# MingruiYuan/SpoofSV

Measured on AMD Instinct MI355X. Metric: mel-frames/sec (Text2Mel+SSRN train), higher is better.
Workload: dtype f32 (conv GEMMs: fp32 operands scaled by a power of two and split into fp16 hi+lo = 22 significand bits, three exact fp16 MFMAs per product, fp32 accumulate: ~2^-22 per product, gradients within 3e-6 of float64 = the exact-fp32 path's level); 1 GPU; train_text2mel + train_ssrn (train/ordinary.py step: fwd, l1+bin-div+guided-att losses, bwd, Adam), batch 32 utterances/GPU, N=186, T=325, 80 mel -> 513x1300 linear, hidden 256, random-init; global_batch=32, parallelism=dp1, launch=hipGraph replay, ddp=none

## Files before the change

include/ssv_hip.h:

```cpp
#ifndef SSV_HIP_H
#define SSV_HIP_H
#include <stddef.h>
#include <stdint.h>
#ifdef __cplusplus
extern "C" {
#endif

typedef void* ssv_stream_t;

int ssv_version(void);
const char* ssv_arch(void);
const char* ssv_last_error(void);
int ssv_set_precision(int mode);
int ssv_get_precision(void);
int ssv_amax_rows(int L);
int ssv_absmax(const float* x, long x_bs, int B, long n, float* amax, int namax, ssv_stream_t stream);
int ssv_shift_right_amax(const float* x, long x_bs, float* y, int B, int C, int T, float* amax, int namax, ssv_stream_t stream);
int ssv_deinterleave2_amax(const float* x, long x_bs, float* out, int B, long n, float* amax, int namax, ssv_stream_t stream);
int ssv_deinterleave2_rows_amax(const float* x, long x_bs, float* out, int B, int rows, int L, float* amax, int namax, ssv_stream_t stream);

size_t ssv_conv1d_fwd_workspace(int Cin, int Cout, int k);
int ssv_conv1d_fwd(const float* x, long x_bs, const float* x_amax, int x_namax, const float* w, const void* w_packed, const float* bias,
                   const float* bias_b, float* y, long y_bs, float* y_colstats,
                   int B, int Cin, int Cout, int L, int k, int dilation, int causal,
                   void* ws, size_t ws_bytes, ssv_stream_t stream);
size_t ssv_conv1d_bwd_data_workspace(int Cin, int Cout, int k);
int ssv_conv1d_bwd_data(const float* dy, long dy_bs, const float* dy_amax, int dy_namax, const float* w, const void* w_packed,
                        const float* dx_add, float* dx, long dx_bs,
                        int B, int Cin, int Cout, int L, int k, int dilation, int causal,
                        void* ws, size_t ws_bytes, ssv_stream_t stream);
size_t ssv_conv1d_bwd_weight_workspace(int B, int Cin, int Cout, int L, int k);
int ssv_conv1d_bwd_weight(const float* dy, long dy_bs, const float* dy_amax, int dy_namax, const float* x, long x_bs, const float* x_amax, int x_namax,
                          float* dw, int B, int Cin, int Cout, int L, int k, int dilation, int causal,
                          void* ws, size_t ws_bytes, ssv_stream_t stream);
int ssv_rowsum(const float* x, long x_bs, float* out, int B, int C, int L, ssv_stream_t stream);
int ssv_bias_grad(const float* x, long x_bs, float* out, int B, int C, int L, ssv_stream_t stream);
int ssv_sum_slabs(const float* slabs, float* out, long n, int Z, long stride, ssv_stream_t stream);
int ssv_copy_rows(const float* src, long src_bs, float* dst, long dst_bs, int B, long n, ssv_stream_t stream);

size_t ssv_channel_ln_act_fwd_workspace(int B, int C, int L);
int ssv_channel_ln_act_fwd(const float* x, long x_bs, const float* gamma, const float* beta,
                           float* y, long y_bs, float* y_amax, float* stats, int B, int C, int L, int act,
                           void* ws, size_t ws_bytes, ssv_stream_t stream);
size_t ssv_pointwise_conv_ln_act_fwd_workspace(int Cin, int Cout);
int ssv_pointwise_conv_ln_act_fwd(const float* x, long x_bs, const float* x_amax, int x_namax, const float* w, const void* w_packed, const float* bias,
                                  const float* s, const float* gamma, const float* beta, float* pre, float* stats, float* y, long y_bs, float* y_amax,
                                  int B, int Cin, int Cout, int L, int act, void* ws, size_t ws_bytes, ssv_stream_t stream);
size_t ssv_channel_ln_act_bwd_workspace(int B, int C, int L);
int ssv_channel_ln_act_bwd(const float* dy, long dy_bs, const float* x, long x_bs, const float* stats,
                           const float* gamma, const float* beta, float* dx, long dx_bs, float* pgrads,
                           int B, int C, int L, int act, void* ws, size_t ws_bytes, ssv_stream_t stream);

size_t ssv_pointwise_conv_ln_act_bwd_workspace(int B, int Cin, int Cout, int L);
int ssv_pointwise_conv_ln_act_bwd(const float* dy, long dy_bs, const float* x, long x_bs, const float* x_amax, int x_namax,
                                  const float* w, const void* w_packed,
                                  const float* gamma, const float* beta, const float* pre, const float* stats,
                                  float* dx, long dx_bs, float* dw, float* pgrads, float* ds,
                                  int B, int Cin, int Cout, int L, int act, void* ws, size_t ws_bytes, ssv_stream_t stream);

typedef struct {
  const float* dy; const float* x; float* dw; const float* part; float* pgrads;
  int shift[3]; int pad_;
  const float* dy_amax; const float* x_amax;
  int dy_namax, x_namax;
} ssv_wgrad_job;
int ssv_conv_shifts(int k, int dilation, int causal, int* shift3);
int ssv_conv1d_bwd_weight_multi_ok(int B, int Cin, int Cout, int L, int k);
int ssv_conv1d_bwd_weight_multi_splits(int njobs, int B, int Cin, int Cout, int L, int k);
size_t ssv_conv1d_bwd_weight_multi_workspace(int njobs, int B, int Cin, int Cout, int L, int k);
int ssv_conv1d_bwd_weight_multi(const ssv_wgrad_job* jobs_dev, int njobs, long dy_bs, long x_bs, int B, int Cin, int Cout, int L, int k, int max_shift,
                                int n2, int nblk, void* ws, size_t ws_bytes, ssv_stream_t stream);
int ssv_ln_partial_rows(int B, int L);
int ssv_ln_bwd_partial_rows(int gate, int B, int C, int L, int with_amax);
size_t ssv_highway_conv1d_bwd_data_workspace(int B, int C, int L, int k);
int ssv_highway_conv1d_bwd_data(const float* dy, long dy_bs, const float* x, long x_bs, const float* w, const void* w_packed,
                                const float* g1, const float* b1, const float* g2, const float* b2, const float* h, const float* stats,
                                float* dx, long dx_bs, float* dh, float* dh_amax, float* part, int B, int C, int L, int k, int dilation, int causal,
                                void* ws, size_t ws_bytes, ssv_stream_t stream);
size_t ssv_pointwise_conv_ln_act_bwd_data_workspace(int B, int Cin, int Cout, int L);
int ssv_pointwise_conv_ln_act_bwd_data(const float* dy, long dy_bs, const float* w, const void* w_packed, const float* gamma, const float* beta,
                                       const float* pre, const float* stats, float* dx, long dx_bs, float* ds, float* dpre, float* dpre_amax,
                                       float* part, int B, int Cin, int Cout, int L, int act, void* ws, size_t ws_bytes, ssv_stream_t stream);

size_t ssv_highway_conv1d_fwd_workspace(int B, int C, int L, int k);
int ssv_highway_conv1d_fwd(const float* x, long x_bs, const float* x_amax, int x_namax, const float* w, const void* w_packed, const float* bias,
                           const float* g1, const float* b1, const float* g2, const float* b2,
                           float* h, float* stats, float* y, long y_bs, float* y_amax,
                           int B, int C, int L, int k, int dilation, int causal,
                           void* ws, size_t ws_bytes, ssv_stream_t stream);
size_t ssv_highway_conv1d_bwd_workspace(int B, int C, int L, int k);
int ssv_highway_conv1d_bwd(const float* dy, long dy_bs, const float* x, long x_bs, const float* x_amax, int x_namax, const float* w, const void* w_packed,
                           const float* g1, const float* b1, const float* g2, const float* b2,
                           const float* h, const float* stats, float* dx, long dx_bs, float* dw, float* pgrads,
                           int B, int C, int L, int k, int dilation, int causal,
                           void* ws, size_t ws_bytes, ssv_stream_t stream);

size_t ssv_highway_gate_bwd_workspace(int B, int C, int L);
int ssv_highway_gate_bwd(const float* dy, long dy_bs, const float* x, long x_bs,
                         const float* g1, const float* b1, const float* g2, const float* b2,
                         const float* h, const float* stats, float* dh, float* dxres, long dx_bs, float* pgrads,
                         int B, int C, int L, void* ws, size_t ws_bytes, ssv_stream_t stream);

int ssv_text_embed_fwd(const int64_t* ids, const float* w, const float* bias, float* y,
                       int B, int N, int E, int vocab, ssv_stream_t stream);
int ssv_text_embed_bwd(const int64_t* ids, const float* dy, float* dw, float* dbias,
                       int B, int N, int E, int vocab, ssv_stream_t stream);

int ssv_attention_train_fwd(const float* k, const float* v, long kv_bs, const float* q, long q_bs,
                            float* a, float* r, long r_bs, int B, int d, int N, int T, ssv_stream_t stream);
int ssv_attention_train_fwd_rq(const float* k, const float* v, long kv_bs, const float* q, long q_bs, float* a, float* rq, long rq_bs,
                               int B, int d, int N, int T, ssv_stream_t stream);
size_t ssv_attention_train_bwd_workspace(int B, int d, int N, int T);
int ssv_attention_train_bwd(const float* dr, long dr_bs, const float* da_ext, const float* dq_add, long dq_add_bs,
                            const float* k, const float* v, long kv_bs, const float* q, long q_bs, const float* a,
                            float* dk, float* dv, long dkv_bs, float* dq, long dq_bs,
                            int B, int d, int N, int T, void* ws, size_t ws_bytes, ssv_stream_t stream);

int ssv_attention_step(const float* k, long kv_bs, const float* q_last, long q_bs, long q_cs,
                       const int64_t* pma_in, float* a, int a_T, int col, const int* col_dev, int64_t* pma_out,
                       int B, int d, int N, ssv_stream_t stream);
int ssv_synth_advance(const float* y, float* mel_in, int* col_dev, int B, int F, int T, ssv_stream_t stream);
int ssv_attention_apply(const float* v, long kv_bs, const float* a, int a_T, float* r, long r_bs,
                        int B, int d, int N, int T, ssv_stream_t stream);

size_t ssv_deconv1d_k2s2_fwd_workspace(int Cin, int Cout);
int ssv_deconv1d_k2s2_fwd(const float* x, long x_bs, const float* x_amax, int x_namax, const float* w, const void* w_packed, const float* bias,
                          float* y, long y_bs, float* y_amax, int y_namax, int B, int Cin, int Cout, int L, void* ws, size_t ws_bytes, ssv_stream_t stream);
size_t ssv_deconv1d_k2s2_bwd_workspace(int B, int Cin, int Cout);
int ssv_deconv1d_k2s2_bwd(const float* dy, long dy_bs, const float* dy_amax, int dy_namax, const float* x, long x_bs, const float* w,
                          float* dx, long dx_bs, float* dw, float* dbias,
                          int B, int Cin, int Cout, int L, void* ws, size_t ws_bytes, ssv_stream_t stream);

size_t ssv_spec_losses_workspace(long n);
int ssv_spec_losses_fwd(const float* y, const float* gt, long n, float* out, void* ws, size_t ws_bytes, ssv_stream_t stream);
int ssv_spec_losses_bwd(const float* y, const float* gt, long n, const float* gscale, float* dy, ssv_stream_t stream);
int ssv_spec_losses_fwd_bwd(const float* y, const float* gt, long n, const float* gscale, float* out, float* dy, void* ws, size_t ws_bytes,
                            ssv_stream_t stream);
size_t ssv_guided_att_loss_workspace(int B, int N, int T);
int ssv_guided_att_loss_fwd(const float* a, const float* gaw, int gaw_T, float* out, int B, int N, int T,
                            void* ws, size_t ws_bytes, ssv_stream_t stream);
int ssv_guided_att_loss_bwd(const float* gaw, int gaw_T, const float* gscale, float* da, int B, int N, int T,
                            ssv_stream_t stream);

int ssv_mask_cols(float* x, long x_bs, int B, int C, int L, const int* live, int mult, ssv_stream_t stream);
int ssv_attention_train_fwd_rq_len(const float* k, const float* v, long kv_bs, const float* q, long q_bs, float* a, float* rq, long rq_bs,
                                   int B, int d, int N, int T, const int* live, ssv_stream_t stream);
int ssv_spec_losses_len(const float* y, const float* gt, int B, int C, int L, const int* live, int mult, const float* gscale,
                        float* out, float* dy, void* ws, size_t ws_bytes, ssv_stream_t stream);
int ssv_guided_att_loss_fwd_len(const float* a, const float* gaw, int gaw_T, float* out, int B, int N, int T, const int* live,
                                void* ws, size_t ws_bytes, ssv_stream_t stream);
int ssv_guided_att_loss_bwd_len(const float* gaw, int gaw_T, const float* gscale, float* da, int B, int N, int T, const int* live,
                                ssv_stream_t stream);

typedef struct { const float* w; void* planes; int M, K, Kpad, KT; long sm, sk; int first_block, pad_; float* inv_out; } ssv_pack_job;
size_t ssv_conv_pack_bytes(int Cout, int Cin, int k);
int ssv_conv_pack_plan(int n, const float* const* w, void* const* planes, const int* Cout, const int* Cin, const int* k,
                       ssv_pack_job* jobs_host);
size_t ssv_conv_pack_multi_workspace(int njobs);
int ssv_conv_pack_multi(const ssv_pack_job* jobs_dev, int njobs, int nblocks, void* ws, size_t ws_bytes, ssv_stream_t stream);

typedef struct { float* p; const float* g; float* m; float* v; long n; } ssv_adam_chunk;
int ssv_adam_multi(const ssv_adam_chunk* chunks, int nchunks, float lr, float beta1, float beta2, float eps,
                   int step, int* step_dev, ssv_stream_t stream);

size_t ssv_lstm_fwd_workspace(int Bn, int T, int F, int H, int layers);
int ssv_lstm_fwd(const float* x, const float* const* w_ih, const float* const* w_hh,
                 const float* const* b_ih, const float* const* b_hh, float* h_last,
                 int Bn, int T, int F, int H, int layers, void* ws, size_t ws_bytes, ssv_stream_t stream);
int ssv_lstm_fwd_cached(const float* x, const float* const* w_ih, const float* const* w_hh,
                        const float* const* b_ih, const float* const* b_hh, float* h_last,
                        int Bn, int T, int F, int H, int layers, void* ws, size_t ws_bytes, int weights_packed, ssv_stream_t stream);
size_t ssv_proj_l2norm_fwd_workspace(int Bn, int P);
int ssv_proj_l2norm_fwd(const float* h, const float* w, const float* bias, float* e, float* norms, int Bn, int H, int P,
                        void* ws, size_t ws_bytes, ssv_stream_t stream);
size_t ssv_proj_l2norm_bwd_workspace(int Bn, int P);
int ssv_proj_l2norm_bwd(const float* de, const float* e, const float* norms, const float* h, const float* w,
                        float* dh, float* dw, float* dbias, int Bn, int H, int P, void* ws, size_t ws_bytes, ssv_stream_t stream);
size_t ssv_lstm_saved_bytes(int Bn, int T, int F, int H, int layers);
size_t ssv_lstm_train_fwd_workspace(int Bn, int T, int F, int H, int layers);
int ssv_lstm_train_fwd(const float* x, const float* const* w_ih, const float* const* w_hh,
                       const float* const* b_ih, const float* const* b_hh, float* h_last, void* saved,
                       int Bn, int T, int F, int H, int layers, void* ws, size_t ws_bytes, ssv_stream_t stream);
size_t ssv_lstm_bwd_workspace(int Bn, int T, int F, int H, int layers);
int ssv_lstm_bwd(const float* dh_last, const void* saved, const float* const* w_ih, const float* const* w_hh,
                 float* const* dw_ih, float* const* dw_hh, float* const* db_ih, float* const* db_hh,
                 int Bn, int T, int F, int H, int layers, void* ws, size_t ws_bytes, ssv_stream_t stream);
size_t ssv_ge2e_loss_fwd_workspace(int N, int M, int D);
int ssv_ge2e_loss_fwd(const float* emb, const float* w, const float* b, float* loss, float* per,
                      int N, int M, int D, void* ws, size_t ws_bytes, ssv_stream_t stream);

size_t ssv_ge2e_loss_bwd_workspace(int N, int M, int D);
int ssv_ge2e_loss_bwd(const float* emb, const float* w, const float* b, const float* dloss, float* demb, float* dw, float* db,
                      int N, int M, int D, void* ws, size_t ws_bytes, ssv_stream_t stream);

int ssv_tisv_batch_gather(const float* corpus, long U_total, const int* rows, float* out, int Bn, int nmels, int frames, ssv_stream_t stream);
#define SSV_CLIP_SGD_MAX_GROUPS 8
typedef struct { float* p; const float* g; long n; int group; int pad_; } ssv_clip_sgd_chunk;
long ssv_clip_sgd_workspace(int nchunks);
int ssv_clip_sgd_multi(const ssv_clip_sgd_chunk* chunks, int nchunks, const float* max_norm, int ngroups, float lr, float* norms,
                       const float* loss, float* loss_hist, int hist_len, int* step_dev, void* ws, size_t ws_bytes, ssv_stream_t stream);

int ssv_sv_trial_scores(const float* enr, const float* ver, float* sim, float* cent, int N, int E, int V, int ver_stride, int D, ssv_stream_t stream);
int ssv_sv_eer_sweep(const float* sim, int N, int V, const float* thr, int nthr, int head, int tail, double den, double pos, double hden,
                     double hpos, int* counts, double* hist, int hist_len, int* step_dev, ssv_stream_t stream);
int ssv_sv_accept_rate(const float* sim_stack, int nmat, int N, int V, int tail, float thres, float* rates, ssv_stream_t stream);
int ssv_sv_score_curve(const float* sim_stack, int nmat, int N, int V, int head, int tail, const float* thr, int nthr, int* counts, ssv_stream_t stream);
int ssv_score_list_curve_f32(const float* scores, const unsigned char* cls, long n, int nclass, const float* thr, int nthr, int* counts, ssv_stream_t stream);
int ssv_score_list_curve_f64(const double* scores, const unsigned char* cls, long n, int nclass, const double* thr, int nthr, int* counts, ssv_stream_t stream);
int ssv_sv_curve_tile(void);

long ssv_ivec_features_workspace(long G, int Cc, int delta_order);
int ssv_ivec_features(const float* mel, const long* utt_off, const float* dct, float* out, long G, int M, int U, int Cc, int delta_window,
                      int delta_order, int cmn_window, void* ws, size_t ws_bytes, ssv_stream_t stream);
int ssv_gmm_frame_tile(int D, int C);
int ssv_gmm_diag_gselect(const float* X, const float* A, const float* B, const float* g, int* idx, float* post, float* loglik, long F, int D, int C,
                         int nsel, float min_post, ssv_stream_t stream);
int ssv_gmm_diag_stats(const float* X, const int* idx, const float* post, const long* seg_off, const long* seg_off_host, float* slab, long F, int D,
                       int C, int nsel, int S, int order, ssv_stream_t stream);
int ssv_gmm_stats_reduce(const float* slab, double* out, int S, long n, ssv_stream_t stream);
int ssv_gmm_diag_update(const double* stats, double* w, double* mu, double* var, float* A, float* B, float* g, int C, int D, double var_floor,
                        double min_count, double min_weight, ssv_stream_t stream);
int ssv_gmm_diag_planes(const double* w, const double* mu, const double* var, float* A, float* B, float* g, int C, int D, ssv_stream_t stream);

int ssv_gl_project(const float* mag, const float* reb, const float* tprev, float alpha, float* proj,
                   int B, int F, int T, ssv_stream_t stream);
int ssv_complex_abs(const float* spec, float* mag, int B, int F, int T, ssv_stream_t stream);
int ssv_ola_frames(const float* fr, const float* inv_env, float* out, int B, int N, int T, int hop, ssv_stream_t stream);
int ssv_ola_signal(const float* fr, const float* inv_env, float* y, int B, int N, int T, int hop, ssv_stream_t stream);
int ssv_frame_signal(const float* y, float* fr, int B, int n, int N, int T, int hop, ssv_stream_t stream);
int ssv_rowmax(const float* x, float* out, int B, long n, ssv_stream_t stream);
int ssv_scale_pow(const float* x, const float* rowmax, float* y, float p, float s, int B, long n, ssv_stream_t stream);
int ssv_deemphasis(const float* x, float* y, double a, int B, int n, ssv_stream_t stream);
int ssv_preemphasis(const float* x, float* y, float a, int B, int n, ssv_stream_t stream);
int ssv_exp_affine(const float* x, float* y, float a, float b, long n, ssv_stream_t stream);
int ssv_log_norm(const float* x, float* y, float ref_db, float max_db, long n, ssv_stream_t stream);

size_t ssv_fft_tables_floats(int n_fft);
int ssv_fft_tables_host(float* out, int n_fft);
int ssv_fft_frame_tile(int n_fft);
int ssv_stft_fft(const float* y, const float* tab, float* spec, int B, int n, int n_fft, int hop, int T, ssv_stream_t stream);
int ssv_istft_frames_fft(const float* spec, const float* tab, float* fr, int B, int n_fft, int T, ssv_stream_t stream);
int ssv_ola_signal_fm(const float* fr, const float* inv_env, float* y, int B, int N, int T, int hop, ssv_stream_t stream);
int ssv_gl_step_fft(const float* fr, const float* inv_env, const float* tab, const float* mag, const float* tprev, float alpha,
                    float* reb, float* proj, int B, int n_fft, int T, int hop, ssv_stream_t stream);

int ssv_resample_sinc(const float* x, const int* n_in, const float* bank, float* y, int* n_out, int B, int n_max, int m_max,
// ... 92 lines not shown
```

spoofsv_amd/_lib.py:

```python
import ctypes
import os
import re

_PKG = os.path.dirname(os.path.abspath(__file__))
_ROOT = os.path.dirname(_PKG)
HEADER = os.path.join(_ROOT, "include", "ssv_hip.h")
LIBPATH = os.environ.get("SSV_HIP_LIB") or os.path.join(_PKG, "libssv_hip.so")


class AdamChunk(ctypes.Structure):
    _fields_ = [("p", ctypes.c_void_p), ("g", ctypes.c_void_p), ("m", ctypes.c_void_p),
                ("v", ctypes.c_void_p), ("n", ctypes.c_long)]


class AdamExChunk(ctypes.Structure):
    _fields_ = [("p", ctypes.c_void_p), ("g", ctypes.c_void_p), ("m", ctypes.c_void_p), ("v", ctypes.c_void_p),
                ("vmax", ctypes.c_void_p), ("n", ctypes.c_long)]


class ClipSgdChunk(ctypes.Structure):
    _fields_ = [("p", ctypes.c_void_p), ("g", ctypes.c_void_p), ("n", ctypes.c_long), ("group", ctypes.c_int), ("pad_", ctypes.c_int)]


class PackJob(ctypes.Structure):
    _fields_ = [("w", ctypes.c_void_p), ("planes", ctypes.c_void_p), ("M", ctypes.c_int), ("K", ctypes.c_int),
                ("Kpad", ctypes.c_int), ("KT", ctypes.c_int), ("sm", ctypes.c_long), ("sk", ctypes.c_long),
                ("first_block", ctypes.c_int), ("pad_", ctypes.c_int), ("inv_out", ctypes.c_void_p)]


class WgradJob(ctypes.Structure):
    _fields_ = [("dy", ctypes.c_void_p), ("x", ctypes.c_void_p), ("dw", ctypes.c_void_p), ("part", ctypes.c_void_p),
                ("pgrads", ctypes.c_void_p), ("shift", ctypes.c_int * 3), ("pad_", ctypes.c_int),
                ("dy_amax", ctypes.c_void_p), ("x_amax", ctypes.c_void_p), ("dy_namax", ctypes.c_int), ("x_namax", ctypes.c_int)]


def _ctype(decl):
    d = decl.strip()
    if "*" in d:
        return ctypes.c_char_p if d.replace(" ", "") == "constchar*" else ctypes.c_void_p
    base = d.split()[0] if d.split() else d
    if base == "unsigned":
        return ctypes.c_uint
    return {"int": ctypes.c_int, "long": ctypes.c_long, "float": ctypes.c_float, "double": ctypes.c_double, "size_t": ctypes.c_size_t,
            "ssv_stream_t": ctypes.c_void_p, "void": None}[base]


def parse_header(path=HEADER):
    src = open(path).read()
    src = re.sub(r"/\*.*?\*/", "", src, flags=re.S)
    src = re.sub(r"typedef\s+struct\s*\{.*?\}\s*\w+\s*;", "", src, flags=re.S)
    protos = {}
    for m in re.finditer(r"(?:^|\n)\s*((?:const\s+)?[\w]+\s*\*?)\s*(ssv_\w+)\s*\(([^;{]*?)\)\s*;", src, flags=re.S):
        ret, name, args = m.group(1), m.group(2), m.group(3)
        argtypes, argnames = [], []
        if args.strip() not in ("", "void"):
            for a in args.split(","):
                a = " ".join(a.split())
                mm = re.match(r"(.*?)(\w+)$", a)
                argtypes.append(_ctype(mm.group(1)))
                argnames.append(mm.group(2))
        protos[name] = (_ctype(ret), argtypes, argnames)
    return protos


_lib = None
_protos = None


def lib():
    global _lib, _protos
    if _lib is not None:
        return _lib
    if not os.path.exists(LIBPATH):
        raise RuntimeError(
            "libssv_hip.so not found at %s -- build it with `python -c 'import __graft_entry__ as g; g.build()'` "
            "(or `make -C spoofsv_amd/csrc`).  There is no CPU/torch fallback for the HIP hot path." % LIBPATH)
    import torch
    e = os.environ.get("SSV_PRECISION")
    if e and e not in ("fp32", "0", "bf16x3", "1", "f16x2", "2"):
        raise RuntimeError("SSV_PRECISION=%r is not one of fp32|0, bf16x3|1, f16x2|2" % e)
    L = ctypes.CDLL(LIBPATH)
    _protos = parse_header()
    missing = [n for n in _protos if not hasattr(L, n)]
    if missing:
        raise RuntimeError("libssv_hip.so lacks symbols declared in include/ssv_hip.h: %s" % ", ".join(missing))
    for name, (ret, argtypes, _) in _protos.items():
        fn = getattr(L, name)
        fn.restype = ret
        fn.argtypes = argtypes
    _lib = L
    return L


def precision():
    return lib().ssv_get_precision()


def call(name, *args):
    rc = getattr(lib(), name)(*args)
    if rc != 0:
        raise RuntimeError("%s failed (%d): %s" % (name, rc, lib().ssv_last_error().decode()))


def query(name, *args):
    return int(getattr(lib(), name)(*args))
```

spoofsv_amd/csrc/api.hip:

```cpp
#include <stdarg.h>
#include <stdio.h>
#include <stdlib.h>
#include <string.h>
#include "ssv_common.h"

static thread_local char g_err[512] = "";
int ssv_fail(int code, const char* fmt, ...) {
  va_list ap;
  va_start(ap, fmt);
  vsnprintf(g_err, sizeof(g_err), fmt, ap);
  va_end(ap);
  return code;
}
int ssv_check_launch(const char* what) {
  hipError_t e = hipGetLastError();
  if (e == hipSuccess) return 0;
  ssv_fail(0, "%s: launch failed: %s", what, hipGetErrorString(e));
  return -(int)e;
}
static int g_precision = -1;
static int precision_from_env() {
  const char* e = getenv("SSV_PRECISION");
  if (!e || !*e || !strcmp(e, "f16x2") || !strcmp(e, "2")) return 2;
  if (!strcmp(e, "fp32") || !strcmp(e, "0")) return 0;
  if (!strcmp(e, "bf16x3") || !strcmp(e, "1")) return 1;
  return -1;
}
int ssv_precision() {
  if (g_precision < 0) {
    g_precision = precision_from_env();
    if (g_precision < 0) {
      fprintf(stderr, "libssv_hip: SSV_PRECISION=%s is not one of fp32|0, bf16x3|1, f16x2|2 (call ssv_set_precision to choose a mode)\n", getenv("SSV_PRECISION"));
      abort();
    }
  }
  return g_precision;
}
static const char* const g_knob_names[SSV_T_COUNT] = {"SSV_NT_FORCE", "SSV_NNB_FORCE", "SSV_LN_GROUPS", "SSV_LN_PERSIST", "SSV_LSTM_MERGE", "SSV_PWLN_BWD"};
static char g_knob_val[SSV_T_COUNT][512];
static const char* g_knob[SSV_T_COUNT];
static int g_knobs_loaded = 0;
static void load_knobs() {
  for (int i = 0; i < SSV_T_COUNT; ++i) {
    const char* e = getenv(g_knob_names[i]);
    if (e) { strncpy(g_knob_val[i], e, sizeof g_knob_val[i] - 1); g_knob_val[i][sizeof g_knob_val[i] - 1] = 0; g_knob[i] = g_knob_val[i]; }
    else g_knob[i] = nullptr;
  }
  __atomic_store_n(&g_knobs_loaded, 1, __ATOMIC_RELEASE);
}
const char* ssv_tuning(int knob) {
  if (!__atomic_load_n(&g_knobs_loaded, __ATOMIC_ACQUIRE)) load_knobs();
  return g_knob[knob];
}
extern "C" void ssv_reload_tuning(void) { load_knobs(); }
#include <mutex>
#include <string>
#include <map>
static int g_shape_log = -1;
static std::string g_shape_path;
static std::mutex g_shape_mu;
static std::map<std::string, long>* g_shape_seen = nullptr;
static void shape_log_flush() {
  std::lock_guard<std::mutex> lk(g_shape_mu);
  if (!g_shape_seen) return;
  if (g_shape_path.empty()) return;
  if (FILE* f = fopen(g_shape_path.c_str(), "w")) {
    for (const auto& kv : *g_shape_seen) fprintf(f, "%s\t%ld\n", kv.first.c_str(), kv.second);
    fclose(f);
  }
}
bool ssv_shape_log_on() {
  if (g_shape_log < 0) { const char* e = getenv("SSV_SHAPE_LOG"); g_shape_log = (e && *e) ? 1 : 0; if (g_shape_log) { g_shape_path = e; atexit(shape_log_flush); } }
  return g_shape_log == 1;
}
void ssv_shape_log(const char* kernel, dim3 grid, dim3 block, double flops, double bytes, const char* note) {
  if (!ssv_shape_log_on()) return;
  char line[768];
  snprintf(line, sizeof line, "%s\t%ux%ux%u\t%.6g\t%.6g\t%s", kernel, grid.x * block.x, grid.y * block.y, grid.z * block.z, flops, bytes, note ? note : "");
  std::lock_guard<std::mutex> lk(g_shape_mu);
  if (!g_shape_seen) g_shape_seen = new std::map<std::string, long>();
  ++(*g_shape_seen)[line];
}
extern "C" int ssv_set_precision(int mode) {
  int prev = g_precision >= 0 ? g_precision : precision_from_env();
  if (prev < 0) prev = ssv_fail(SSV_UNSUPPORTED, "SSV_PRECISION=%s is not one of fp32|0, bf16x3|1, f16x2|2; mode %d set explicitly", getenv("SSV_PRECISION"), mode);
  g_precision = mode <= 0 ? 0 : (mode == 1 ? 1 : 2);
  return prev;
}
extern "C" int ssv_get_precision(void) {
  if (g_precision < 0 && precision_from_env() < 0)
    return ssv_fail(SSV_UNSUPPORTED, "SSV_PRECISION=%s is not one of fp32|0, bf16x3|1, f16x2|2", getenv("SSV_PRECISION"));
  return ssv_precision();
}
extern "C" int ssv_version(void) { return 7; }
extern "C" const char* ssv_arch(void) { return "gfx950"; }
extern "C" const char* ssv_last_error(void) { return g_err; }
```

spoofsv_amd/csrc/api_conv.hip:

```cpp
#include "ssv_host.h"

int conv_shifts(int k, int dilation, int causal, int* shift) {
  SSV_CHECK(k == 1 || k == 3, SSV_UNSUPPORTED, "conv1d: kernel_size %d not supported (1 or 3)", k);
  SSV_CHECK(dilation >= 1 && dilation * (k - 1) <= 54, SSV_UNSUPPORTED, "conv1d: dilation %d not supported (k=%d)", dilation, k);
  const int j0 = causal ? k - 1 : (k - 1) / 2;
  for (int j = 0; j < 3; ++j) shift[j] = j < k ? (j - j0) * dilation : 0;
  return 0;
}
extern "C" int ssv_conv_shifts(int k, int dilation, int causal, int* shift3) { return conv_shifts(k, dilation, causal, shift3); }

int amax_of(const float* x, long x_bs, int B, long n_item, const float* given, int ngiven, float* fb, AmaxList* out, hipStream_t st) {
  if (given) {
    SSV_CHECK(ngiven > 0, SSV_BAD_SHAPE, "operand scale list given with %d entries per item", ngiven);
    out->p = given; out->n = ngiven;
    return 0;
  }
  SSV_CHECK(fb, SSV_BAD_SHAPE, "split-fp16: no operand scales given and no workspace to compute them in");
  SSV_CHECK(B <= SSV_AMAX_FB_FLOATS, SSV_UNSUPPORTED, "split-fp16: batch %d needs caller-provided operand scales (ssv_absmax)", B);
  int npb = SSV_AMAX_FB_FLOATS / B;
  if (npb > 64) npb = 64;
  const long pieces = (n_item + 4095) / 4096;
  if (npb > pieces) npb = (int)(pieces > 0 ? pieces : 1);
  SSV_TRY(ssv_launch_absmax(x, x_bs, B, n_item, fb, npb, st));
  out->p = fb; out->n = npb;
// ... 51 lines not shown
    return ssv_launch_linear_len1_fwd(x, x_bs, w, bias, bias_b, M, y, y_bs, B, K, M, st);
  GemmNN g;
  for (int j = 0; j < 3; ++j) g.shift[j] = shift[j];
  const float* a = w;
  if (w_sk != k) {
    SSV_TRY(ssv_launch_pack_wt(w, ws_f32(ws, l.main), K, M, k, st));
    a = ws_f32(ws, l.main);
  }
  g.A = a; g.sam = (long)K * k; g.sac = k; g.saj = 1;
  g.X = x; g.sxb = x_bs; g.sxc = L; g.Lx = L;
  g.C = y; g.scb = y_bs; g.scm = L;
  g.bias = bias; g.bias_b = bias_b; g.sbb = M;
  if (r) { g.R = r; g.srb = r_bs; g.srm = L; }
  g.M = M; g.N = L; g.Kc = K; g.KT = k; g.B = B;
  return ssv_launch_gemm_nn(g, st);
}

extern "C" size_t ssv_conv1d_fwd_workspace(int Cin, int Cout, int k) { return conv_fwd_ws(Cin, Cout, k).total; }
extern "C" int ssv_conv1d_fwd(const float* x, long x_bs, const float* x_amax, int x_namax, const float* w, const void* w_packed, const float* bias,
                              const float* bias_b, float* y, long y_bs, float* y_colstats,
                              int B, int Cin, int Cout, int L, int k, int dilation, int causal, void* ws, size_t ws_bytes,
                              ssv_stream_t stream) {
  SSV_CHECK(x && w && y && B > 0 && Cin > 0 && Cout > 0 && L > 0, SSV_BAD_SHAPE, "conv1d_fwd: bad argument B=%d Cin=%d Cout=%d L=%d", B, Cin, Cout, L);
  SSV_CHECK(x_bs >= (long)Cin * L && y_bs >= (long)Cout * L, SSV_BAD_SHAPE, "conv1d_fwd: batch stride smaller than C*L");
  int shift[3];
  SSV_TRY(conv_shifts(k, dilation, causal, shift));
  const bool bf3 = use_bf3(B, L, Cin, Cout);
  const ConvWs l = conv_fwd_ws(Cin, Cout, k);
  if (bf3 && (!w_packed || (use_f16() && !x_amax)))
    SSV_CHECK(ws && ws_bytes >= l.total, SSV_BAD_SHAPE, "conv1d_fwd: workspace too small");
  SSV_CHECK(!y_colstats || (bf3 && Cout % 64 == 0 && y_bs == (long)Cout * L), SSV_UNSUPPORTED,
            "conv1d_fwd: column statistics need a split-MFMA mode, Cout %% 64 == 0 and a dense output (Cout=%d)", Cout);
  return conv_nn(x, x_bs, w, packed_planes(w_packed, Cout, Cin, k).fwd, (long)Cin * k, k, bias, bias_b, nullptr, 0, y, y_bs, B, Cin, Cout, L, k, shift, bf3,
                 ws, l, (hipStream_t)stream, x_amax, x_namax, y_colstats);
}

extern "C" size_t ssv_conv1d_bwd_data_workspace(int Cin, int Cout, int k) { return conv_bwd_data_ws(Cin, Cout, k).total; }
extern "C" int ssv_conv1d_bwd_data(const float* dy, long dy_bs, const float* dy_amax, int dy_namax, const float* w, const void* w_packed,
                                   const float* dx_add, float* dx, long dx_bs,
                                   int B, int Cin, int Cout, int L, int k, int dilation, int causal,
                                   void* ws, size_t ws_bytes, ssv_stream_t stream) {
  SSV_CHECK(dy && w && dx && B > 0 && Cin > 0 && Cout > 0 && L > 0, SSV_BAD_SHAPE, "conv1d_bwd_data: bad argument");
  const ConvWs l = conv_bwd_data_ws(Cin, Cout, k);
  SSV_CHECK((w_packed && !(use_f16() && !dy_amax)) || (ws && ws_bytes >= l.total), SSV_BAD_SHAPE, "conv1d_bwd_data: workspace too small");
  int shift[3];
  SSV_TRY(conv_shifts(k, dilation, causal, shift));
  for (int j = 0; j < 3; ++j) shift[j] = -shift[j];
  return conv_nn(dy, dy_bs, w, packed_planes(w_packed, Cout, Cin, k).tr, k, (long)Cin * k, nullptr, nullptr, dx_add, dx_bs, dx, dx_bs, B, Cout, Cin, L, k, shift,
                 use_bf3(B, L, Cout, Cin), ws, l, (hipStream_t)stream, dy_amax, dy_namax);
}

extern "C" size_t ssv_conv_pack_bytes(int Cout, int Cin, int k) { return packed_planes(nullptr, Cout, Cin, k).bytes; }
extern "C" int ssv_conv_pack_plan(int n, const float* const* w, void* const* planes, const int* Cout, const int* Cin, const int* k,
                                  ssv_pack_job* jobs) {
  SSV_CHECK(n > 0 && w && planes && Cout && Cin && k && jobs, SSV_BAD_SHAPE, "conv_pack_plan: bad argument");
  long blocks = 0;
  for (int i = 0; i < n; ++i) {
    SSV_CHECK(w[i] && planes[i] && Cout[i] > 0 && Cin[i] > 0 && (k[i] == 1 || k[i] == 3), SSV_BAD_SHAPE, "conv_pack_plan: weight %d: bad shape", i);
    const PackedPlanes pp = packed_planes(planes[i], Cout[i], Cin[i], k[i]);
    for (int tr = 0; tr < 2; ++tr) {
      ssv_pack_job& j = jobs[2 * i + tr];
      const SplitPlanes& pl = tr ? pp.tr : pp.fwd;
      const int M = tr ? Cin[i] : Cout[i], K = tr ? Cout[i] : Cin[i];
      j.w = w[i];
      j.planes = pl.hi;
      j.M = M; j.K = K; j.Kpad = pad32(K); j.KT = k[i];
      j.sm = tr ? k[i] : (long)Cin[i] * k[i];
      j.sk = tr ? (long)Cin[i] * k[i] : k[i];
      j.first_block = (int)blocks; j.pad_ = 0;
      j.inv_out = pl.inv;
      blocks += ssv_pack_job_blocks(j);
      SSV_CHECK(blocks < (1L << 30), SSV_UNSUPPORTED, "conv_pack_plan: too many elements");
    }
  }
  return (int)blocks;
}
extern "C" size_t ssv_conv_pack_multi_workspace(int njobs) { return align256((size_t)(njobs / 2) * SSV_PACK_AMAX_PER_WEIGHT * sizeof(float)); }
extern "C" int ssv_conv_pack_multi(const ssv_pack_job* jobs_dev, int njobs, int nblocks, void* ws, size_t ws_bytes, ssv_stream_t stream) {
  SSV_CHECK(jobs_dev && njobs > 0 && njobs % 2 == 0 && nblocks > 0, SSV_BAD_SHAPE, "conv_pack_multi: bad argument");
  const bool f16 = use_f16();
  SSV_CHECK(!f16 || (ws && ws_bytes >= ssv_conv_pack_multi_workspace(njobs)), SSV_BAD_SHAPE, "conv_pack_multi: workspace too small");
  return ssv_launch_pack_multi(jobs_dev, njobs, nblocks, f16 ? (float*)ws : nullptr, (hipStream_t)stream);
}

static int nt_slabs(long tiles_all, int njobs, int B, int L, int kt, int M, int Nc) {
  int wm, ntc;
  ssv_nt_bf3_tile(kt, M, Nc, &wm, &ntc);
  const int per_cu = ssv_nt_bf3_wg_per_cu(kt, wm, ntc);
  const long slots = 256L * per_cu;
  const double t_item = 2.0 * 64 * wm * 16 * ntc * kt * L / (0.55e12 * 2.0 / per_cu);
  const double t_slab = 8.0 * (double)M * Nc * kt / 4e12 * njobs;
  int best = 1;
  double best_t = 1e30;
  for (int z = 1; z <= B && z <= 64; ++z) {
    const long rounds = (tiles_all * z + slots - 1) / slots;
    const double t = (double)rounds * ssv_cdiv(B, z) * t_item + (z > 1 ? z * t_slab : 0.0);
    if (t < best_t * 0.98) { best_t = t; best = z; }
  }
  return best;
}
static int xrow_slabs(long tiles_all, int B, int L) {
  const long chunks = (long)B * ssv_cdiv(L, 64);
  long z = 512 / (tiles_all > 0 ? tiles_all : 1);
  if (z > chunks) z = chunks;
  if (z > 64) z = 64;
  return (int)(z < 1 ? 1 : z);
}
static bool wgrad_bf3_runs(int B, int M, int Nc, int L, long dy_bs, long x_bs) {
  if (ssv_precision() < 1 || (long)B * L < 256 || Nc < SSV_MIN_SPLIT_CHANNELS || M < SSV_MIN_SPLIT_CHANNELS) return false;
  GemmNT g;
  g.sab = dy_bs; g.sam = L; g.La = L; g.sxb = x_bs; g.sxc = L; g.Lx = L;
  g.M = M; g.Nc = Nc; g.B = B;
  return ssv_nt_bf3_fits(g);
}
static bool wgrad_bf3_runs_dense(int B, int M, int Nc, int L) { return wgrad_bf3_runs(B, M, Nc, L, (long)M * L, (long)Nc * L); }
static int nt_force(int z, int M, int Nc, int k) {
  if (const char* e = ssv_tuning(SSV_T_NT_FORCE)) {
    char key[48];
    snprintf(key, sizeof key, "%d:%d:%d=", M, Nc, k);
    const char* hit = strstr(e, key);
    if (hit && (hit == e || hit[-1] == ';')) { const int v = atoi(hit + strlen(key)); if (v > 0) z = v; }
  }
  return z;
}
int dw_splits(int B, int M, int Nc, int k, int L) {
  const int tiles = ssv_nt_bf3_tiles(k == 3 ? 3 : 1, M, Nc);
  if (k != 3 && ssv_nt_bf3_xrow(1, M, Nc) && wgrad_bf3_runs_dense(B, M, Nc, L)) {
    int z = nt_force(xrow_slabs(tiles, B, L), M, Nc, k);
    const long chunks = (long)B * ssv_cdiv(L, 64);
    if (z > chunks) z = (int)chunks;
    return z < 1 ? 1 : z;
  }
  int z = nt_force(nt_slabs(tiles, 1, B, L, k == 3 ? 3 : 1, M, Nc), M, Nc, k);
  if (z > B) z = B;
  if (z < 1) z = 1;
  return z;
}
struct WgradWs { int Z; size_t slabs, fb_dy, fb_x, total; };
static WgradWs wgrad_ws(int B, int Cin, int Cout, int L, int k) {
  WsTake t;
  WgradWs l;
  l.Z = dw_splits(B, Cout, Cin, k, L);
  l.slabs = t.take((size_t)l.Z * Cout * Cin * k * sizeof(float));
  l.fb_dy = t.take(AMAX_FB_BYTES);
  l.fb_x = t.take(AMAX_FB_BYTES);
  l.total = t.off;
  return l;
}
extern "C" size_t ssv_conv1d_bwd_weight_workspace(int B, int Cin, int Cout, int L, int k) { return wgrad_ws(B, Cin, Cout, L, k).total; }
int conv1d_bwd_weight_impl(const float* dy, long dy_bs, const float* x, long x_bs, float* dw, int B, int Cin, int Cout, int L, int k, int dilation,
                           int causal, void* ws, size_t ws_bytes, ssv_stream_t stream, const float* part, float* pgrads, int n2, int nblk,
                           const float* dy_amax, int dy_namax, const float* x_amax, int x_namax) {
  SSV_CHECK(dy && x && dw && B > 0 && Cin > 0 && Cout > 0 && L > 0, SSV_BAD_SHAPE, "conv1d_bwd_weight: bad argument");
  const WgradWs l = wgrad_ws(B, Cin, Cout, L, k);
  SSV_CHECK(ws && ws_bytes >= l.total, SSV_BAD_SHAPE, "conv1d_bwd_weight: workspace too small");
  hipStream_t st = (hipStream_t)stream;
  GemmNT g;
  SSV_TRY(conv_shifts(k, dilation, causal, g.shift));
  int Z = l.Z;
  const float* slabs = ws_f32(ws, l.slabs);
  const long n = (long)Cout * Cin * k;
  g.A = dy; g.sab = dy_bs; g.sam = L; g.La = L;
  g.X = x; g.sxb = x_bs; g.sxc = L; g.Lx = L;
  g.M = Cout; g.Nc = Cin; g.KT = k; g.B = B;
  const bool bf3 = wgrad_bf3_runs(B, Cout, Cin, L, dy_bs, x_bs);
  if (!bf3 && Z > B) Z = B;
  if (Z == 1) { g.C = dw; g.scz = n; g.scm = (long)Cin * k; g.scc = k; g.scj = 1; }
  else { g.C = ws_f32(ws, l.slabs); g.scz = n; g.scm = (long)Cin * k; g.scc = 1; g.scj = Cin; }
  g.Z = Z; g.bstep = Z;
  if (bf3) {
    if (k != 3 && ssv_nt_bf3_xrow(1, Cout, Cin)) g.bstep = 0;
    if (use_f16()) {
      AmaxList la, lx;
      SSV_TRY(amax_of(dy, dy_bs, B, (long)Cout * L, dy_amax, dy_namax, ws_f32(ws, l.fb_dy), &la, st));
      SSV_TRY(amax_of(x, x_bs, B, (long)Cin * L, x_amax, x_namax, ws_f32(ws, l.fb_x), &lx, st));
      g.f16 = 1; g.a_amax = la.p; g.a_namax = la.n * B; g.x_amax = lx.p; g.x_namax = lx.n * B;
    }
    SSV_TRY(ssv_launch_gemm_nt_bf3(g, st));
  } else if (L == 1 && k == 1) {
    SSV_TRY(ssv_launch_linear_len1_wgrad(dy, dy_bs, x, x_bs, dw, B, Cin, Cout, st));
    if (part) SSV_TRY(ssv_reduce_partial_rows(part, pgrads, n2, nblk, st));
    return 0;
  } else SSV_TRY(ssv_launch_gemm_nt(g, st));
  if (part) {
    if (Z > 1 && nblk <= 768) return ssv_launch_reduce_pair(slabs, dw, Cout, Cin, k, Z, part, pgrads, n2, nblk, st);
    SSV_TRY(ssv_reduce_partial_rows(part, pgrads, n2, nblk, st));
  }
  if (Z > 1) SSV_TRY(ssv_launch_reduce_slabs_perm(slabs, dw, Cout, Cin, k, Z, st));
  return 0;
}
extern "C" int ssv_conv1d_bwd_weight(const float* dy, long dy_bs, const float* dy_amax, int dy_namax, const float* x, long x_bs, const float* x_amax, int x_namax,
                                     float* dw, int B, int Cin, int Cout, int L, int k, int dilation, int causal,
                                     void* ws, size_t ws_bytes, ssv_stream_t stream) {
  return conv1d_bwd_weight_impl(dy, dy_bs, x, x_bs, dw, B, Cin, Cout, L, k, dilation, causal, ws, ws_bytes, stream, nullptr, nullptr, 0, 0,
                                dy_amax, dy_namax, x_amax, x_namax);
}

extern "C" int ssv_conv1d_bwd_weight_multi_ok(int B, int Cin, int Cout, int L, int k) {
  return (k == 1 || k == 3) && L >= 8 && wgrad_bf3_runs_dense(B, Cout, Cin, L) ? 1 : 0;
}
extern "C" int ssv_conv1d_bwd_weight_multi_splits(int njobs, int B, int Cin, int Cout, int L, int k) {
  const int kt = k == 3 ? 3 : 1;
  if (njobs < 1) njobs = 1;
  const long tiles = (long)ssv_nt_bf3_tiles(kt, Cout, Cin) * njobs;
  if (kt == 1 && ssv_nt_bf3_xrow(1, Cout, Cin)) return xrow_slabs(tiles, B, L);
  int z = nt_slabs(tiles, njobs, B, L, kt, Cout, Cin);
  if (z > B) z = B;
  if (z < 1) z = 1;
  return z;
}
extern "C" size_t ssv_conv1d_bwd_weight_multi_workspace(int njobs, int B, int Cin, int Cout, int L, int k) {
  return align256((size_t)njobs * ssv_conv1d_bwd_weight_multi_splits(njobs, B, Cin, Cout, L, k) * Cout * Cin * k * sizeof(float));
}
extern "C" int ssv_conv1d_bwd_weight_multi(const ssv_wgrad_job* jobs_dev, int njobs, long dy_bs, long x_bs, int B, int Cin, int Cout, int L, int k, int max_shift,
                                           int n2, int nblk, void* ws, size_t ws_bytes, ssv_stream_t stream) {
  SSV_CHECK(jobs_dev && njobs > 0 && B > 0 && Cin > 0 && Cout > 0 && L > 0, SSV_BAD_SHAPE, "conv1d_bwd_weight_multi: bad argument");
  SSV_CHECK(ssv_conv1d_bwd_weight_multi_ok(B, Cin, Cout, L, k), SSV_UNSUPPORTED, "conv1d_bwd_weight_multi: shape or arithmetic mode not supported");
  SSV_CHECK(n2 == 0 || nblk <= 768, SSV_UNSUPPORTED, "conv1d_bwd_weight_multi: %d partial rows (max 768)", nblk);
  SSV_CHECK(ws && ws_bytes >= ssv_conv1d_bwd_weight_multi_workspace(njobs, B, Cin, Cout, L, k), SSV_BAD_SHAPE, "conv1d_bwd_weight_multi: workspace too small");
  hipStream_t st = (hipStream_t)stream;
  const int Z = ssv_conv1d_bwd_weight_multi_splits(njobs, B, Cin, Cout, L, k);
  const long n = (long)Cout * Cin * k;
  GemmNT g;
  g.sab = dy_bs; g.sam = L; g.La = L;
  g.sxb = x_bs; g.sxc = L; g.Lx = L;
  g.C = (float*)ws; g.scz = n; g.scm = (long)Cin * k; g.scc = 1; g.scj = Cin;
  g.M = Cout; g.Nc = Cin; g.KT = k; g.B = B; g.Z = Z; g.bstep = (k != 3 && ssv_nt_bf3_xrow(1, Cout, Cin)) ? 0 : Z;
  g.jobs = jobs_dev; g.njobs = njobs; g.max_shift = max_shift;
  g.f16 = use_f16() ? 1 : 0;
  SSV_TRY(ssv_launch_gemm_nt_bf3(g, st));
  return ssv_launch_reduce_pair_multi(jobs_dev, njobs, (const float*)ws, Cout, Cin, k, Z, n2, nblk, st);
}

static ConvWs deconv_fwd_ws(int Cin, int Cout) { return conv_ws(2 * split_bytes(Cout, Cin, 2)); }
extern "C" size_t ssv_deconv1d_k2s2_fwd_workspace(int Cin, int Cout) { return deconv_fwd_ws(Cin, Cout).total; }
extern "C" int ssv_deconv1d_k2s2_fwd(const float* x, long x_bs, const float* x_amax, int x_namax, const float* w, const void* w_packed, const float* bias,
                                     float* y, long y_bs, float* y_amax, int y_namax, int B, int Cin, int Cout, int L, void* ws, size_t ws_bytes, ssv_stream_t stream) {
  SSV_CHECK(x && w && y && B > 0 && Cin > 0 && Cout > 0 && L > 0, SSV_BAD_SHAPE, "deconv1d_k2s2_fwd: bad argument");
  SSV_CHECK(!y_amax || y_namax > 0, SSV_BAD_SHAPE, "deconv1d_k2s2_fwd: scale list of %d entries", y_namax);
  hipStream_t st = (hipStream_t)stream;
  if (use_bf3(B, L, Cin, Cout)) {
    const ConvWs l = deconv_fwd_ws(Cin, Cout);
    SSV_CHECK(ws && ws_bytes >= l.total, SSV_BAD_SHAPE, "deconv1d_k2s2_fwd: workspace too small");
    const int M2 = 2 * Cout, Kpad = pad32(Cin);
    const bool f16 = use_f16();
    float* aux = ws_f32(ws, l.aux);
    SplitPlanes pl = packed_planes(w_packed, Cin, M2, 1).tr;
    if (!pl.hi) {
      pl.hi = ws_u16(ws, l.main); pl.lo = ws_u16(ws, l.main + split_bytes(M2, Cin, 1));
      if (f16) { SSV_TRY(ssv_launch_pack_split_f16(w, (long)Cin * M2, pl.hi, pl.lo, M2, Cin, Kpad, 1, 1, (long)M2, 1, aux, st)); pl.inv = aux + 64; }
      else SSV_TRY(ssv_launch_pack_split(w, pl.hi, pl.lo, M2, Cin, Kpad, 1, 1, (long)M2, 1, 0, st));
    }
    GemmNNB g;
    if (f16) {
      AmaxList xa = {nullptr, 0};
      SSV_TRY(amax_of(x, x_bs, B, (long)Cin * L, x_amax, x_namax, ws_f32(ws, l.fb), &xa, st));
      g.f16 = 1; g.a_inv = pl.inv; g.x_amax = xa.p; g.x_namax = xa.n; g.x_amax_bs = xa.n;
    }
    g.Ahi = pl.hi; g.Alo = pl.lo; g.Kpad = Kpad;
    g.X = x; g.sxb = x_bs; g.sxc = L; g.Lx = L;
    g.C = y; g.scb = y_bs; g.scm = (long)2 * L; g.row_pair = 1;
    g.bias = bias;
    g.M = M2; g.N = L; g.Kc = Cin; g.B = B;
    if (y_amax && f16) { g.c_amax = y_amax; g.c_namax = y_namax; }
    const int rc = ssv_launch_gemm_nn_bf3(g, st);
    if (rc == SSV_UNSUPPORTED && g.c_amax) {
      g.c_amax = nullptr; g.c_namax = 0;
      SSV_TRY(ssv_launch_gemm_nn_bf3(g, st));
      return ssv_launch_absmax(y, y_bs, B, (long)Cout * 2 * L, y_amax, y_namax, st);
    }
    return rc;
  }
  for (int j = 0; j < 2; ++j) {
    GemmNN g;
    g.A = w + j; g.sam = 2; g.sac = (long)2 * Cout;
    g.X = x; g.sxb = x_bs; g.sxc = L; g.Lx = L;
    g.C = y + j; g.scb = y_bs; g.scm = (long)2 * L; g.scn = 2;
    g.bias = bias;
    g.M = Cout; g.N = L; g.Kc = Cin; g.B = B;
    SSV_TRY(ssv_launch_gemm_nn(g, st));
  }
  if (y_amax && use_f16()) return ssv_launch_absmax(y, y_bs, B, (long)Cout * 2 * L, y_amax, y_namax, st);
  return 0;
}
struct DeconvBwdWs { int Z; size_t slabs, rs, hi, lo, aux, fb, total; };
static DeconvBwdWs deconv_bwd_ws(int B, int Cin, int Cout) {
  WsTake t;
  DeconvBwdWs l;
  l.Z = dw_splits(B, Cin, Cout, 1, SSV_NOMINAL_L);
  l.slabs = t.take((size_t)l.Z * Cin * Cout * 2 * sizeof(float));
  l.rs = t.take((size_t)B * Cout * sizeof(float));
  l.hi = t.take(split_bytes(Cin, Cout, 2));
  l.lo = t.take(split_bytes(Cin, Cout, 2));
  l.aux = t.take(SSV_F16_AUX_BYTES);
  l.fb = t.take(AMAX_FB_BYTES);
  l.total = t.off;
  return l;
}
extern "C" size_t ssv_deconv1d_k2s2_bwd_workspace(int B, int Cin, int Cout) { return deconv_bwd_ws(B, Cin, Cout).total; }
extern "C" int ssv_deconv1d_k2s2_bwd(const float* dy, long dy_bs, const float* dy_amax, int dy_namax, const float* x, long x_bs, const float* w, float* dx, long dx_bs,
                                     float* dw, float* dbias, int B, int Cin, int Cout, int L, void* ws, size_t ws_bytes, ssv_stream_t stream) {
  SSV_CHECK(dy && x && w && dx && B > 0 && Cin > 0 && Cout > 0 && L > 0, SSV_BAD_SHAPE, "deconv1d_k2s2_bwd: bad argument");
  const DeconvBwdWs l = deconv_bwd_ws(B, Cin, Cout);
  SSV_CHECK(ws && ws_bytes >= l.total, SSV_BAD_SHAPE, "deconv1d_k2s2_bwd: workspace too small");
  hipStream_t st = (hipStream_t)stream;
  const int Z = l.Z;
  const long n = (long)Cin * Cout * 2;
  float* slabs = ws_f32(ws, l.slabs);
  float* rs = ws_f32(ws, l.rs);
  const bool bf3 = use_bf3(B, L, Cout, Cin);
  unsigned short* hi = ws_u16(ws, l.hi);
  unsigned short* lo = ws_u16(ws, l.lo);
  const int Kpad = pad32(Cout);
  const size_t tap = (size_t)((Cin + 15) / 16 * 16) * Kpad;
// ... 42 lines not shown
```

spoofsv_amd/csrc/misc.hip:

```cpp
#include "ssv_common.h"
#include "../../include/ssv_hip.h"

__global__ __launch_bounds__(256) void reduce_slabs_kernel(const float* __restrict__ s, float* __restrict__ out, long n, int Z, long stride) {
  const long i = (long)blockIdx.x * 256 + threadIdx.x;
  if (i >= n) return;
  float a[4] = {0.f, 0.f, 0.f, 0.f};
  int z = 0;
  for (; z + 3 < Z; z += 4) {
#pragma unroll
    for (int u = 0; u < 4; ++u) a[u] += s[(long)(z + u) * stride + i];
  }
  for (; z < Z; ++z) a[0] += s[(long)z * stride + i];
  out[i] = (a[0] + a[1]) + (a[2] + a[3]);
}
int ssv_launch_reduce_slabs(const float* slabs, float* out, long n, int Z, long stride, hipStream_t st) {
  hipLaunchKernelGGL(reduce_slabs_kernel, dim3(ssv_cdiv(n, 256)), dim3(256), 0, st, slabs, out, n, Z, stride);
  return ssv_check_launch("reduce_slabs");
}

__device__ __forceinline__ void reduce_perm_block(const float* __restrict__ s, float* __restrict__ out, int Nc, int KT, long n, int Z, int block,
                                                  float* __restrict__ stage ) {
  const long P = n / KT;
  const long q = (long)block * 256 + threadIdx.x;
  if (KT == 1) {
    if (q >= P) return;
    float a[8];
#pragma unroll
    for (int u = 0; u < 8; ++u) a[u] = 0.f;
    int z = 0;
    for (; z + 7 < Z; z += 8) {
#pragma unroll
      for (int u = 0; u < 8; ++u) a[u] += s[(long)(z + u) * n + q];
    }
    for (; z < Z; ++z) a[0] += s[(long)z * n + q];
    out[q] = ((a[0] + a[1]) + (a[2] + a[3])) + ((a[4] + a[5]) + (a[6] + a[7]));
    return;
  }
  if (q < P) {
    const long m = q / Nc;
    const int c = (int)(q % Nc);
    if (KT == 3) {
      const long i0 = (m * 3) * Nc + c, i1 = i0 + Nc, i2 = i1 + Nc;
      float a0 = 0.f, a1 = 0.f, b0 = 0.f, b1 = 0.f, c0 = 0.f, c1 = 0.f;
      int z = 0;
#pragma unroll 2
      for (; z + 1 < Z; z += 2) {
        const float* __restrict__ s0 = s + (long)z * n;
        const float* __restrict__ s1 = s0 + n;
        a0 += s0[i0]; a1 += s1[i0]; b0 += s0[i1]; b1 += s1[i1]; c0 += s0[i2]; c1 += s1[i2];
      }
      if (z < Z) { const float* __restrict__ s0 = s + (long)z * n; a0 += s0[i0]; b0 += s0[i1]; c0 += s0[i2]; }
      stage[threadIdx.x * 3] = a0 + a1; stage[threadIdx.x * 3 + 1] = b0 + b1; stage[threadIdx.x * 3 + 2] = c0 + c1;
    } else {
      for (int j = 0; j < KT; ++j) {
        const long i = (m * KT + j) * Nc + c;
        float a0 = 0.f, a1 = 0.f;
        int z = 0;
        for (; z + 1 < Z; z += 2) { a0 += s[(long)z * n + i]; a1 += s[(long)(z + 1) * n + i]; }
        if (z < Z) a0 += s[(long)z * n + i];
        stage[threadIdx.x * KT + j] = a0 + a1;
      }
    }
  }
  __syncthreads();
  const long o0 = (long)block * 256 * KT;
  const long cnt = (P - (long)block * 256 < 256 ? P - (long)block * 256 : 256) * KT;
  float* __restrict__ dst = out + o0;
  if ((reinterpret_cast<size_t>(dst) & 15) == 0) {
    for (long f = threadIdx.x * 4; f + 3 < cnt; f += 1024) *reinterpret_cast<float4*>(dst + f) = *reinterpret_cast<const float4*>(stage + f);
    for (long f = (cnt & ~3L) + threadIdx.x; f < cnt; f += 256) dst[f] = stage[f];
  } else {
    for (long f = threadIdx.x; f < cnt; f += 256) dst[f] = stage[f];
  }
}
__global__ __launch_bounds__(256) void reduce_slabs_perm_kernel(const float* __restrict__ s, float* __restrict__ out, int Nc, int KT, long n, int Z) {
  __shared__ __attribute__((aligned(16))) float stage[256 * 3];
  reduce_perm_block(s, out, Nc, KT, n, Z, (int)blockIdx.x, stage);
}
int ssv_launch_reduce_slabs_perm(const float* slabs, float* out, int M, int Nc, int KT, int Z, hipStream_t st) {
  const long n = (long)M * Nc * KT;
  hipLaunchKernelGGL(reduce_slabs_perm_kernel, dim3(ssv_cdiv((long)M * Nc, 256)), dim3(256), 0, st, slabs, out, Nc, KT, n, Z);
  return ssv_check_launch("reduce_slabs_perm");
}

template <typename P>
__device__ __forceinline__ float ssv_fold_rows(P part, int n2, int nblk, int i, int rg) {
  float a[16];
#pragma unroll
  for (int u = 0; u < 16; ++u) a[u] = 0.f;
  int k = rg;
  for (; k + 120 < nblk; k += 128) {
#pragma unroll
    for (int u = 0; u < 16; ++u) a[u] += part[(long)(k + 8 * u) * n2 + i];
  }
  for (; k < nblk; k += 8) a[0] += part[(long)k * n2 + i];
  return (((a[0] + a[1]) + (a[2] + a[3])) + ((a[4] + a[5]) + (a[6] + a[7]))) + (((a[8] + a[9]) + (a[10] + a[11])) + ((a[12] + a[13]) + (a[14] + a[15])));
}
__global__ __launch_bounds__(256) void reduce_pair_kernel(const float* __restrict__ s, float* __restrict__ out, int Nc, int KT, long n, int Z, int nA,
                                                          const float* __restrict__ part, float* __restrict__ pout, int n2, int nblk) {
  __shared__ float red[8][32];
  __shared__ __attribute__((aligned(16))) float stage[256 * 3];
  if ((int)blockIdx.x < nA) {
    reduce_perm_block(s, out, Nc, KT, n, Z, (int)blockIdx.x, stage);
    return;
  }
  const int li = threadIdx.x & 31, rg = threadIdx.x >> 5;
  const int i = ((int)blockIdx.x - nA) * 32 + li;
  red[rg][li] = i < n2 ? ssv_fold_rows(part, n2, nblk, i, rg) : 0.f;
  __syncthreads();
  if (rg == 0 && i < n2) {
    float t = 0.f;
#pragma unroll
    for (int r = 0; r < 8; ++r) t += red[r][li];
    pout[i] = t;
  }
}
int ssv_launch_reduce_pair(const float* slabs, float* out, int M, int Nc, int KT, int Z, const float* part, float* pout, int n2, int nblk, hipStream_t st) {
  const long n = (long)M * Nc * KT;
  const int nA = ssv_cdiv((long)M * Nc, 256), nB = ssv_cdiv(n2, 32);
  hipLaunchKernelGGL(reduce_pair_kernel, dim3(nA + nB), dim3(256), 0, st, slabs, out, Nc, KT, n, Z, nA, part, pout, n2, nblk);
  return ssv_check_launch("reduce_pair");
}

__global__ __launch_bounds__(256) void reduce_pair_multi_kernel(const ssv_wgrad_job* __restrict__ jobs, const float* __restrict__ slabs, int Nc, int KT, long n,
                                                                int Z, int nA, int n2, int nblk) {
  __shared__ float red[8][32];
  const ssv_wgrad_job jb = jobs[blockIdx.y];
  const float* __restrict__ s = slabs + (long)blockIdx.y * Z * n;
  __shared__ __attribute__((aligned(16))) float stage[256 * 3];
  if ((int)blockIdx.x < nA) {
    reduce_perm_block(s, jb.dw, Nc, KT, n, Z, (int)blockIdx.x, stage);
    return;
  }
  if (!jb.part) return;
  const __attribute__((address_space(1))) float* __restrict__ part = (const __attribute__((address_space(1))) float*)jb.part;
  const int li = threadIdx.x & 31, rg = threadIdx.x >> 5;
  const int i = ((int)blockIdx.x - nA) * 32 + li;
  red[rg][li] = i < n2 ? ssv_fold_rows(part, n2, nblk, i, rg) : 0.f;
  __syncthreads();
  if (rg == 0 && i < n2) {
    float t = 0.f;
#pragma unroll
    for (int r = 0; r < 8; ++r) t += red[r][li];
    jb.pgrads[i] = t;
  }
}
int ssv_launch_reduce_pair_multi(const ssv_wgrad_job* jobs, int njobs, const float* slabs, int M, int Nc, int KT, int Z, int n2, int nblk, hipStream_t st) {
  const long n = (long)M * Nc * KT;
  const int nA = ssv_cdiv((long)M * Nc, 256), nB = n2 > 0 ? ssv_cdiv(n2, 32) : 0;
  hipLaunchKernelGGL(reduce_pair_multi_kernel, dim3(nA + nB, njobs), dim3(256), 0, st, jobs, slabs, Nc, KT, n, Z, nA, n2, nblk);
  return ssv_check_launch("reduce_pair_multi");
}

__global__ __launch_bounds__(256) void pack_wt_kernel(const float* __restrict__ w, float* __restrict__ wt, int Cout, int Cin, int KT) {
  const long i = (long)blockIdx.x * 256 + threadIdx.x;
  const long n = (long)Cout * Cin * KT;
  if (i >= n) return;
  const int j = (int)(i % KT);
  const long r = i / KT;
  const int o = (int)(r % Cout), c = (int)(r / Cout);
  wt[i] = w[((long)o * Cin + c) * KT + j];
}
int ssv_launch_pack_wt(const float* w, float* wt, int Cout, int Cin, int KT, hipStream_t st) {
  const long n = (long)Cout * Cin * KT;
  hipLaunchKernelGGL(pack_wt_kernel, dim3(ssv_cdiv(n, 256)), dim3(256), 0, st, w, wt, Cout, Cin, KT);
  return ssv_check_launch("pack_wt");
}

__global__ __launch_bounds__(256) void linear_len1_fwd_kernel(const float* __restrict__ x, long x_bs, const float* __restrict__ w, const float* __restrict__ bias,
                                                              const float* __restrict__ bias_b, long sbb, float* __restrict__ y, long y_bs, int B, int K, int M) {
  const long t = ((long)blockIdx.x * 256 + threadIdx.x) >> 3;
  const int j = threadIdx.x & 7;
  if (t >= (long)B * M) return;
  const int m = (int)(t % M), b = (int)(t / M);
  const float* __restrict__ wr = w + (long)m * K;
  const float* __restrict__ xr = x + (long)b * x_bs;
  float a0 = 0.f, a1 = 0.f, a2 = 0.f, a3 = 0.f;
  int kdone = 0;
  if ((K & 3) == 0 && (((size_t)w | (size_t)x) & 15) == 0 && (x_bs & 3) == 0) {
    for (int k = 4 * j; k + 3 < K; k += 32) {
      const f32x4 wv = *reinterpret_cast<const f32x4*>(wr + k), xv = *reinterpret_cast<const f32x4*>(xr + k);
      a0 = __builtin_fmaf(wv[0], xv[0], a0); a1 = __builtin_fmaf(wv[1], xv[1], a1); a2 = __builtin_fmaf(wv[2], xv[2], a2); a3 = __builtin_fmaf(wv[3], xv[3], a3);
    }
    kdone = K;
  }
  for (int k = kdone + j; k < K; k += 8) a0 = __builtin_fmaf(wr[k], xr[k], a0);
  float acc = (a0 + a1) + (a2 + a3);
  acc += __shfl_xor(acc, 1);
  acc += __shfl_xor(acc, 2);
  acc += __shfl_xor(acc, 4);
  if (j == 0) {
    if (bias) acc += bias[m];
    if (bias_b) acc += bias_b[(long)b * sbb + m];
    y[(long)b * y_bs + m] = acc;
  }
}
int ssv_launch_linear_len1_fwd(const float* x, long x_bs, const float* w, const float* bias, const float* bias_b, long sbb, float* y, long y_bs,
                               int B, int K, int M, hipStream_t st) {
  hipLaunchKernelGGL(linear_len1_fwd_kernel, dim3(ssv_cdiv((long)B * M * 8, 256)), dim3(256), 0, st, x, x_bs, w, bias, bias_b, sbb, y, y_bs, B, K, M);
  return ssv_check_launch("linear_len1_fwd");
}
__global__ __launch_bounds__(256) void linear_len1_wgrad_kernel(const float* __restrict__ dy, long dy_bs, const float* __restrict__ x, long x_bs,
                                                                float* __restrict__ dw, int B, int K, int M) {
  const long i = (long)blockIdx.x * 256 + threadIdx.x;
  if (i >= (long)M * K) return;
  const int m = (int)(i / K), c = (int)(i % K);
  float acc = 0.f;
  int b = 0;
  for (; b + 3 < B; b += 4) {
    const float d0 = dy[(long)b * dy_bs + m], d1 = dy[(long)(b + 1) * dy_bs + m], d2 = dy[(long)(b + 2) * dy_bs + m], d3 = dy[(long)(b + 3) * dy_bs + m];
    const float x0 = x[(long)b * x_bs + c], x1 = x[(long)(b + 1) * x_bs + c], x2 = x[(long)(b + 2) * x_bs + c], x3 = x[(long)(b + 3) * x_bs + c];
    acc = __builtin_fmaf(d0, x0, acc); acc = __builtin_fmaf(d1, x1, acc); acc = __builtin_fmaf(d2, x2, acc); acc = __builtin_fmaf(d3, x3, acc);
  }
  for (; b < B; ++b) acc = __builtin_fmaf(dy[(long)b * dy_bs + m], x[(long)b * x_bs + c], acc);
  dw[i] = acc;
}
int ssv_launch_linear_len1_wgrad(const float* dy, long dy_bs, const float* x, long x_bs, float* dw, int B, int K, int M, hipStream_t st) {
  hipLaunchKernelGGL(linear_len1_wgrad_kernel, dim3(ssv_cdiv((long)M * K, 256)), dim3(256), 0, st, dy, dy_bs, x, x_bs, dw, B, K, M);
  return ssv_check_launch("linear_len1_wgrad");
}

__global__ __launch_bounds__(256) void fill_kernel(float* p, float v, long n) {
  const long i = (long)blockIdx.x * 256 + threadIdx.x;
  if (i < n) p[i] = v;
}
int ssv_launch_fill(float* p, float v, long n, hipStream_t st) {
  hipLaunchKernelGGL(fill_kernel, dim3(ssv_cdiv(n, 256)), dim3(256), 0, st, p, v, n);
  return ssv_check_launch("fill");
}

__global__ __launch_bounds__(256) void rowsum_kernel(const float* __restrict__ x, long x_bs, float* __restrict__ out, int B, int C, int L) {
  const int row = blockIdx.x * 4 + (threadIdx.x >> 6), lane = threadIdx.x & 63;
  if (row >= B * C) return;
  const int b = row / C, c = row % C;
// ... 372 lines not shown
  const float w1 = dy ? gscale[0] * inv : 0.f, w2 = dy ? gscale[1] * inv : 0.f;
  float s1 = 0.f, s2 = 0.f;
  for (long i = (long)blockIdx.x * 256 + threadIdx.x; i < n; i += (long)gridDim.x * 256) {
    const int t = (int)(i % L);
    float d = 0.f;
    if (t < lv) {
      const float a = y[i], g = gt[i];
      s1 += fabsf(g - a);
      s2 += -g * logf(a + 1e-8f) - (1.f - g) * logf(1.f - a + 1e-8f);
      const float df = a - g;
      const float sgn = df > 0.f ? 1.f : (df < 0.f ? -1.f : 0.f);
      d = w1 * sgn + w2 * (-g / (a + 1e-8f) + (1.f - g) / (1.f - a + 1e-8f));
    }
    if (dy) dy[i] = d;
  }
  s1 = block_sum256(s1, red);
  s2 = block_sum256(s2, red);
  if (threadIdx.x == 0) { part[blockIdx.x] = s1; part[gridDim.x + blockIdx.x] = s2; }
}
__global__ __launch_bounds__(256) void finish_sums_len_kernel(const float* __restrict__ part, int nblk, int nout, long rows, const int* __restrict__ live0,
                                                              int mult, int cap0, const int* __restrict__ live1, int cap1, float* __restrict__ out) {
  __shared__ float red[4];
  const float den = (float)rows * (float)live_cols(live0, mult, cap0) * (live1 ? (float)live_cols(live1, 1, cap1) : 1.f);
  for (int k = 0; k < nout; ++k) {
    float s = 0.f;
    for (int i = threadIdx.x; i < nblk; i += 256) s += part[(long)k * nblk + i];
    s = block_sum256(s, red);
    if (threadIdx.x == 0) out[k] = den > 0.f ? s / den : 0.f;
  }
}
extern "C" int ssv_spec_losses_len(const float* y, const float* gt, int B, int C, int L, const int* live, int mult, const float* gscale,
                                   float* out, float* dy, void* ws, size_t ws_bytes, ssv_stream_t stream) {
  SSV_CHECK(y && gt && out && live && B > 0 && C > 0 && L > 0 && mult > 0 && (!dy || gscale), SSV_BAD_SHAPE,
            "spec_losses_len: bad argument (B=%d C=%d L=%d mult=%d)", B, C, L, mult);
  const long n = (long)B * C * L;
  SSV_CHECK(ws && ws_bytes >= ssv_spec_losses_workspace(n), SSV_BAD_SHAPE, "spec_losses_len: workspace too small");
  const int nblk = (int)((n + 255) / 256 < LOSS_BLOCKS ? (n + 255) / 256 : LOSS_BLOCKS);
  hipLaunchKernelGGL(spec_loss_len_kernel, dim3(nblk), dim3(256), 0, (hipStream_t)stream, y, gt, C, L, n, live, mult, gscale, dy, (float*)ws);
  SSV_TRY(ssv_check_launch("spec_loss_len"));
  hipLaunchKernelGGL(finish_sums_len_kernel, dim3(1), dim3(256), 0, (hipStream_t)stream, (const float*)ws, nblk, 2, (long)B * C, live, mult, L,
                     (const int*)nullptr, 1, out);
  return ssv_check_launch("finish_sums_len");
}
__global__ __launch_bounds__(256) void gatt_part_len_kernel(const float* __restrict__ a, const float* __restrict__ gaw, int gaw_T,
                                                            long tot, int N, int T, const int* __restrict__ live, float* __restrict__ part) {
  __shared__ float red[4];
  const int nl = live_cols(live, 1, N), tl = live_cols(live + 1, 1, T);
  float s = 0.f;
  for (long i = (long)blockIdx.x * 256 + threadIdx.x; i < tot; i += (long)gridDim.x * 256) {
    const int t = (int)(i % T), n = (int)((i / T) % N);
    if (n < nl && t < tl) s += a[i] * gaw[(long)n * gaw_T + t];
  }
  s = block_sum256(s, red);
  if (threadIdx.x == 0) part[blockIdx.x] = s;
}
__global__ __launch_bounds__(256) void gatt_bwd_len_kernel(const float* __restrict__ gaw, int gaw_T, const float* __restrict__ gscale,
                                                           float* __restrict__ da, long tot, int B, int N, int T, const int* __restrict__ live) {
  const long i = (long)blockIdx.x * 256 + threadIdx.x;
  if (i >= tot) return;
  const int nl = live_cols(live, 1, N), tl = live_cols(live + 1, 1, T);
  const int t = (int)(i % T), n = (int)((i / T) % N);
  da[i] = (n < nl && t < tl) ? gscale[0] * gaw[(long)n * gaw_T + t] / ((float)B * (float)nl * (float)tl) : 0.f;
}
extern "C" int ssv_guided_att_loss_fwd_len(const float* a, const float* gaw, int gaw_T, float* out, int B, int N, int T, const int* live,
                                           void* ws, size_t ws_bytes, ssv_stream_t stream) {
  SSV_CHECK(a && gaw && out && live && B > 0 && N > 0 && T > 0 && gaw_T >= T, SSV_BAD_SHAPE, "guided_att_loss_fwd_len: bad shape B=%d N=%d T=%d gaw_T=%d",
            B, N, T, gaw_T);
  SSV_CHECK(ws && ws_bytes >= LOSS_BLOCKS * sizeof(float), SSV_BAD_SHAPE, "guided_att_loss_fwd_len: workspace too small");
  const long tot = (long)B * N * T;
  const int nblk = (int)((tot + 255) / 256 < LOSS_BLOCKS ? (tot + 255) / 256 : LOSS_BLOCKS);
  hipLaunchKernelGGL(gatt_part_len_kernel, dim3(nblk), dim3(256), 0, (hipStream_t)stream, a, gaw, gaw_T, tot, N, T, live, (float*)ws);
  SSV_TRY(ssv_check_launch("gatt_part_len"));
  hipLaunchKernelGGL(finish_sums_len_kernel, dim3(1), dim3(256), 0, (hipStream_t)stream, (const float*)ws, nblk, 1, (long)B, live, 1, N, live + 1, T, out);
  return ssv_check_launch("finish_sums_len");
}
extern "C" int ssv_guided_att_loss_bwd_len(const float* gaw, int gaw_T, const float* gscale, float* da, int B, int N, int T, const int* live,
                                           ssv_stream_t stream) {
  SSV_CHECK(gaw && gscale && da && live && B > 0 && N > 0 && T > 0 && gaw_T >= T, SSV_BAD_SHAPE, "guided_att_loss_bwd_len: bad shape");
  const long tot = (long)B * N * T;
  hipLaunchKernelGGL(gatt_bwd_len_kernel, dim3(ssv_cdiv(tot, 256)), dim3(256), 0, (hipStream_t)stream, gaw, gaw_T, gscale, da, tot, B, N, T, live);
  return ssv_check_launch("gatt_bwd_len");
}

__global__ __launch_bounds__(256) void adam_multi_kernel(const ssv_adam_chunk* __restrict__ chunks, float lr, float b1, float b2, float eps,
                                                         int step_host, const int* __restrict__ step_dev) {
  const int step = step_dev ? step_dev[0] + 1 : step_host;
  const double bc1 = 1.0 - pow((double)b1, (double)step), bc2 = 1.0 - pow((double)b2, (double)step);
  const float step_size = (float)((double)lr / bc1), inv_sqrt_bc2 = (float)(1.0 / sqrt(bc2));
  const ssv_adam_chunk ch = chunks[blockIdx.x];
  auto upd = [&](float& p, float g, float& m, float& v) {
    m = b1 * m + (1.f - b1) * g;
    v = b2 * v + (1.f - b2) * g * g;
    p -= step_size * (m / (sqrtf(v) * inv_sqrt_bc2 + eps));
  };
  long i0 = 0;
  if ((((uintptr_t)ch.p | (uintptr_t)ch.g | (uintptr_t)ch.m | (uintptr_t)ch.v) & 15) == 0) {
    const long n4 = ch.n >> 2;
    typedef float vf4 __attribute__((ext_vector_type(4)));
    auto upd4 = [&](vf4& p, const vf4 g, vf4& m, vf4& v) {
#pragma unroll
      for (int k = 0; k < 4; ++k) {
        float pp = p[k], mm = m[k], vv = v[k];
        upd(pp, g[k], mm, vv);
        p[k] = pp; m[k] = mm; v[k] = vv;
      }
    };
    typedef __attribute__((address_space(1))) vf4 gf4;
    gf4* __restrict__ p4 = (gf4*)ch.p; const gf4* __restrict__ g4 = (const gf4*)ch.g;
    gf4* __restrict__ m4 = (gf4*)ch.m; gf4* __restrict__ v4 = (gf4*)ch.v;
    long i = threadIdx.x;
    for (; i + 256 < n4; i += 512) {
      vf4 p = p4[i], m = m4[i], v = v4[i], q = p4[i + 256], n = m4[i + 256], w = v4[i + 256];
      const vf4 g = g4[i], h = g4[i + 256];
      upd4(p, g, m, v);
      upd4(q, h, n, w);
      p4[i] = p; m4[i] = m; v4[i] = v;
      p4[i + 256] = q; m4[i + 256] = n; v4[i + 256] = w;
    }
    for (; i < n4; i += 256) {
      vf4 p = p4[i], m = m4[i], v = v4[i];
      const vf4 g = g4[i];
      upd4(p, g, m, v);
      p4[i] = p; m4[i] = m; v4[i] = v;
    }
    i0 = n4 << 2;
  }
  for (long i = i0 + threadIdx.x; i < ch.n; i += 256) {
    float p = ch.p[i], m = ch.m[i], v = ch.v[i];
    upd(p, ch.g[i], m, v);
    ch.p[i] = p; ch.m[i] = m; ch.v[i] = v;
  }
}
__global__ void step_inc_kernel(int* step_dev) { step_dev[0] += 1; }
extern "C" int ssv_adam_multi(const ssv_adam_chunk* chunks, int nchunks, float lr, float beta1, float beta2, float eps,
                              int step, int* step_dev, ssv_stream_t stream) {
  SSV_CHECK(nchunks > 0 && (step_dev || step > 0), SSV_BAD_SHAPE, "adam_multi: nchunks=%d step=%d", nchunks, step);
  hipLaunchKernelGGL(adam_multi_kernel, dim3(nchunks), dim3(256), 0, (hipStream_t)stream, chunks, lr, beta1, beta2, eps, step, (const int*)step_dev);
  SSV_TRY(ssv_check_launch("adam_multi"));
  if (step_dev) {
    hipLaunchKernelGGL(step_inc_kernel, dim3(1), dim3(1), 0, (hipStream_t)stream, step_dev);
    return ssv_check_launch("step_inc");
  }
  return 0;
}
```

spoofsv_amd/csrc/pack.hip:

```cpp
#include "bf3_common.h"

__device__ __forceinline__ float ssv_absmax4(const f32x4 q) { return fmaxf(fmaxf(fabsf(q[0]), fabsf(q[1])), fmaxf(fabsf(q[2]), fabsf(q[3]))); }
__device__ __forceinline__ float ssv_absmax_scan(const float* __restrict__ xb, const long lo, const long hi) {
  float v = 0.f;
  if ((((size_t)xb) & 15) == 0) {
    long i = lo + 4L * threadIdx.x;
    for (; i + 3 * 1024 + 3 < hi; i += 4096) {
      const f32x4 q0 = *reinterpret_cast<const f32x4*>(xb + i), q1 = *reinterpret_cast<const f32x4*>(xb + i + 1024);
      const f32x4 q2 = *reinterpret_cast<const f32x4*>(xb + i + 2048), q3 = *reinterpret_cast<const f32x4*>(xb + i + 3072);
      v = fmaxf(v, fmaxf(fmaxf(ssv_absmax4(q0), ssv_absmax4(q1)), fmaxf(ssv_absmax4(q2), ssv_absmax4(q3))));
    }
    for (; i + 3 < hi; i += 1024) v = fmaxf(v, ssv_absmax4(*reinterpret_cast<const f32x4*>(xb + i)));
    for (; i < hi; ++i) v = fmaxf(v, fabsf(xb[i]));
  } else {
    for (long i = lo + threadIdx.x; i < hi; i += 256) v = fmaxf(v, fabsf(xb[i]));
  }
  return v;
}
__global__ __launch_bounds__(256) void absmax_kernel(const float* __restrict__ x, long x_bs, long n, float* __restrict__ out, int npb) {
  __shared__ float sm[4];
  const float* __restrict__ xb = x + (long)blockIdx.y * x_bs;
  const long piece = (((n + npb - 1) / npb) + 3) & ~3L;
  const long lo = (long)blockIdx.x * piece, hi = min(lo + piece, n);
  float v = ssv_absmax_scan(xb, lo, hi);
// ... 61 lines not shown
int ssv_launch_pack_split(const float* w, void* hi, void* lo, int M, int K, int Kpad, int KT, long sm, long sk, long sj, int perm_h, hipStream_t st,
                          int nch_total, int ch_off) {
  const long n = (long)KT * ((M + 15) / 16 * 16) * Kpad;
  if (nch_total <= 0) { nch_total = Kpad / 32; ch_off = 0; }
  hipLaunchKernelGGL(pack_split_kernel, dim3(ssv_cdiv(n, 256)), dim3(256), 0, st, w, (__bf16*)hi, (__bf16*)lo, M, K, Kpad, KT, sm, sk, sj, perm_h,
                     nch_total, ch_off);
  return ssv_check_launch("pack_split");
}

#define PACK_PER_BLOCK 256
__global__ __launch_bounds__(256) void pack_amax_multi_kernel(const ssv_pack_job* __restrict__ jobs, float* __restrict__ amax) {
  __shared__ float sm[4];
  const ssv_pack_job j = jobs[2 * blockIdx.y];
  const long n = (long)j.M * j.K * j.KT;
  const long piece = (((n + gridDim.x - 1) / gridDim.x) + 3) & ~3L;
  const long lo = (long)blockIdx.x * piece, hi = min(lo + piece, n);
  float v = ssv_absmax_scan(j.w, lo, hi);
  v = ssv_wg_max<4>(v, sm);
  if (threadIdx.x == 0) amax[(long)blockIdx.y * gridDim.x + blockIdx.x] = v;
}
template <int F16, int KT>
__device__ __forceinline__ void pack_slot(const ssv_pack_job& j, const long slot, const float sc) {
  typedef __attribute__((address_space(1))) const float gfloat;
  typedef unsigned vu4 __attribute__((ext_vector_type(4)));
  typedef __attribute__((address_space(1))) vu4 guint4;
  const int MB = (j.M + 15) >> 4, NCH = j.Kpad >> 5;
  const int r16 = (int)(slot & 15), kg = (int)((slot >> 4) & 3);
  const long blk = slot >> 6;
  const int ch = (int)(blk % NCH), mb = (int)(blk / NCH);
  const int m = mb * 16 + r16, k0 = ch * 32 + kg * 8;
  const long n = (long)KT * MB * NCH * 512;
  guint4* hip = (guint4*)j.planes;
  guint4* lop = (guint4*)((char*)j.planes + (((size_t)n * 2 + 255) & ~(size_t)255));
  gfloat* w = (gfloat*)j.w + (long)m * j.sm + (long)k0 * j.sk;
  float v[8][KT];
  if (m < j.M && k0 + 8 <= j.K) {
    if (j.sk == KT) {
      float flat[8 * KT];
#pragma unroll
      for (int q = 0; q < 8 * KT; ++q) flat[q] = w[q];
#pragma unroll
      for (int e = 0; e < 8; ++e)
#pragma unroll
        for (int t = 0; t < KT; ++t) v[e][t] = flat[e * KT + t];
    } else {
#pragma unroll
      for (int e = 0; e < 8; ++e)
#pragma unroll
        for (int t = 0; t < KT; ++t) v[e][t] = w[(long)e * j.sk + t];
    }
  } else {
#pragma unroll
    for (int e = 0; e < 8; ++e)
#pragma unroll
      for (int t = 0; t < KT; ++t) v[e][t] = (m < j.M && k0 + e < j.K) ? w[(long)e * j.sk + t] : 0.f;
  }
#pragma unroll
  for (int t = 0; t < KT; ++t) {
    unsigned hw[4], lw[4];
#pragma unroll
    for (int q = 0; q < 4; ++q) {
      unsigned short hb[2], lb[2];
#pragma unroll
      for (int u = 0; u < 2; ++u) {
        const float x = v[2 * q + u][t];
        if constexpr (F16) {
          const _Float16 h = (_Float16)(x * sc);
          const _Float16 l = (_Float16)__builtin_fmaf(x, sc, -(float)h);
          hb[u] = __builtin_bit_cast(unsigned short, h); lb[u] = __builtin_bit_cast(unsigned short, l);
        } else {
          const __bf16 h = (__bf16)x;
          const __bf16 l = (__bf16)(x - (float)h);
          hb[u] = __builtin_bit_cast(unsigned short, h); lb[u] = __builtin_bit_cast(unsigned short, l);
        }
      }
      hw[q] = hb[0] | ((unsigned)hb[1] << 16); lw[q] = lb[0] | ((unsigned)lb[1] << 16);
    }
    const long o = (((long)t * MB + mb) * NCH + ch) * 64 + kg * 16 + r16;
    hip[o] = vu4{hw[0], hw[1], hw[2], hw[3]};
    lop[o] = vu4{lw[0], lw[1], lw[2], lw[3]};
  }
}
template <int F16>
__global__ __launch_bounds__(256) void pack_multi_kernel(const ssv_pack_job* __restrict__ jobs, int njobs, const float* __restrict__ amax) {
  __shared__ float smx[4];
  int lo = 0, hi = njobs - 1;
  while (lo < hi) {
    const int mid = (lo + hi + 1) >> 1;
    if (jobs[mid].first_block <= (int)blockIdx.x) lo = mid; else hi = mid - 1;
  }
  const ssv_pack_job j = jobs[lo];
  float sc = 1.f, inv = 1.f;
  if constexpr (F16) {
    ssv_pow2_scale(ssv_list_max<4>(amax + (long)(lo >> 1) * SSV_PACK_AMAX_PER_WEIGHT, SSV_PACK_AMAX_PER_WEIGHT, smx), sc, inv);
    if ((int)blockIdx.x == j.first_block && threadIdx.x == 0 && j.inv_out) *j.inv_out = inv;
  }
  const long slots = (long)((j.M + 15) >> 4) * (j.Kpad >> 5) * 64;
  const long slot = (long)((int)blockIdx.x - j.first_block) * PACK_PER_BLOCK + threadIdx.x;
  if (slot >= slots) return;
  if (j.KT == 3) pack_slot<F16, 3>(j, slot, sc);
  else if (j.KT == 1) pack_slot<F16, 1>(j, slot, sc);
  else if (j.KT == 2) pack_slot<F16, 2>(j, slot, sc);
}
int ssv_pack_job_blocks(const ssv_pack_job& j) {
  const long slots = (long)((j.M + 15) / 16) * (j.Kpad / 32) * 64;
  return (int)((slots + PACK_PER_BLOCK - 1) / PACK_PER_BLOCK);
}
int ssv_launch_pack_multi(const ssv_pack_job* jobs_dev, int njobs, int nblocks, float* amax_ws, hipStream_t st) {
  if (amax_ws) {
    hipLaunchKernelGGL(pack_amax_multi_kernel, dim3(SSV_PACK_AMAX_PER_WEIGHT, njobs / 2), dim3(256), 0, st, jobs_dev, amax_ws);
    SSV_TRY(ssv_check_launch("pack_amax_multi"));
    hipLaunchKernelGGL(pack_multi_kernel<1>, dim3(nblocks), dim3(256), 0, st, jobs_dev, njobs, (const float*)amax_ws);
  } else {
    hipLaunchKernelGGL(pack_multi_kernel<0>, dim3(nblocks), dim3(256), 0, st, jobs_dev, njobs, (const float*)nullptr);
  }
  return ssv_check_launch("pack_multi");
}
```

spoofsv_amd/csrc/ssv_common.h:

```cpp
#pragma once
#include <hip/hip_runtime.h>
#include <stdint.h>
#include <stddef.h>
#include "../../include/ssv_hip.h"

int ssv_fail(int code, const char* fmt, ...);
#define SSV_BAD_SHAPE (-1)
#define SSV_UNSUPPORTED (-2)
#define SSV_CHECK(cond, code, ...) do { if (!(cond)) return ssv_fail((code), __VA_ARGS__); } while (0)
#define SSV_TRY(expr) do { int _e = (expr); if (_e) return _e; } while (0)
int ssv_check_launch(const char* what);

typedef __attribute__((ext_vector_type(4))) float f32x4;

struct GemmNN {
  const float* A = nullptr; long sab = 0, sam = 0, sac = 0, saj = 0;
  const float* X = nullptr; long sxb = 0, sxc = 0, sxn = 1; int Lx = 0;
  float* C = nullptr; long scb = 0, scm = 0, scn = 1;
  const float* bias = nullptr;
  const float* bias_b = nullptr; long sbb = 0;
  const float* R = nullptr; long srb = 0, srm = 0, srn = 1;
  int M = 0, N = 0, Kc = 0, KT = 1, B = 1;
  int shift[3] = {0, 0, 0};
  float alpha = 1.f;
};
int ssv_launch_gemm_nn(const GemmNN& g, hipStream_t st);

struct GemmNT {
  const float* A = nullptr; long sab = 0, sam = 0, sat = 1; int La = 0;
  const float* X = nullptr; long sxb = 0, sxc = 0, sxn = 1; int Lx = 0;
  float* C = nullptr; long scz = 0, scm = 0, scc = 1, scj = 0;
  int M = 0, Nc = 0, KT = 1, B = 1, Z = 1, bstep = 1;
  int shift[3] = {0, 0, 0};
  const ssv_wgrad_job* jobs = nullptr; int njobs = 0;
  int max_shift = -1;
  int f16 = 0; const float* a_amax = nullptr; int a_namax = 0; const float* x_amax = nullptr; int x_namax = 0;
};
int ssv_launch_gemm_nt(const GemmNT& g, hipStream_t st);

struct GemmNNB {
  const unsigned short* Ahi = nullptr; const unsigned short* Alo = nullptr; int Kpad = 0;
  const float* X = nullptr; long sxb = 0, sxc = 0; int Lx = 0;
  float* C = nullptr; long scb = 0, scm = 0;
  const float* bias = nullptr;
  const float* bias_b = nullptr; long sbb = 0;
  const float* R = nullptr; long srb = 0, srm = 0;
  int M = 0, N = 0, Kc = 0, KT = 1, B = 1;
  int shift[3] = {0, 0, 0};
  int sxn = 1, scn = 1;
  int row_pair = 0; float* c_amax = nullptr; int c_namax = 0;
  unsigned short* hs_planes = nullptr; long hs_plane_bytes = 0; int hs_npad = 0;
  int hs_keep_h = 1;
  int ksplit = 1; long scz = 0; int skip_rows = 0;
  const unsigned short* x0_planes = nullptr; const float* x0_amax = nullptr; int xsplit0 = 0;
  int perm_h = 0, epi = 0, first = 0;
  float* cstate = nullptr;
  float* lstm_out = nullptr; int lstm_s = 0, lstm_lo = 0, lstm_D = 0, xsplit = 0; long sab = 0;
  const unsigned short* A0hi = nullptr; const unsigned short* A0lo = nullptr;
  float* gates_out = nullptr;
  int f16 = 0; const float* a_inv = nullptr; const float* x_amax = nullptr; int x_namax = 0; long x_amax_bs = 0;
  float* colstats = nullptr;
  const float* xrow_w = nullptr; long xrow_sk = 0;
};
int ssv_launch_gemm_nn_bf3(const GemmNNB& g, hipStream_t st);
int ssv_launch_gemm_pwln(const GemmNNB& g, const float* gamma, const float* beta, float* y, long ybs, float* stats, float* y_amax, int namax, int act,
                         hipStream_t st);
int ssv_launch_gemm_nt_bf3(const GemmNT& g, hipStream_t st);
int ssv_launch_gemm_nt3r(const GemmNT& g, dim3 grid, int mtiles, int tchunks, int ring_ms, hipStream_t st);
struct PwLnBw {
  const float* dy; long dy_bs; const float* pre; const float* stats; const float* gamma; const float* beta;
  float* dpre; float* part; int part_rows; int part_q; float* amax; int namax;
  const unsigned short* Ahi; const unsigned short* Alo; const float* a_inv;
  float* dx; long dx_bs; const float* xrow_w; long xrow_sk;
  int M, Cin, L, act;
};
bool ssv_pwln_bwd_fused_ok(int B, int Cin, int Cout, int L);
int ssv_launch_pwln_bwd(const PwLnBw& q, int B, int f16, hipStream_t st);
bool ssv_nt_bf3_xrow(int KT, int M, int Nc);
bool ssv_nt_bf3_fits(const GemmNT& g);
int ssv_launch_pack_split(const float* w, void* hi, void* lo, int M, int K, int Kpad, int KT, long sm, long sk, long sj, int perm_h, hipStream_t st,
                          int nch_total = 0, int ch_off = 0);
int ssv_launch_pack_split_f16(const float* w, long w_elems, void* hi, void* lo, int M, int K, int Kpad, int KT, long sm, long sk, long sj, float* aux, hipStream_t st);
int ssv_launch_pack_split_f16_list(const float* w, void* hi, void* lo, int M, int K, int Kpad, int KT, long sm, long sk, long sj, int perm_h,
                                   const float* list, int nlist, float* inv_out, hipStream_t st, int nch_total = 0, int ch_off = 0);
#define SSV_F16_AUX_FLOATS 128
#define SSV_AMAX_FALLBACK 64
int ssv_launch_absmax(const float* x, long x_bs, int B, long n, float* out, int npb, hipStream_t st);
int ssv_nt_bf3_tiles(int KT, int M, int Nc);
void ssv_nt_bf3_tile(int KT, int M, int Nc, int* wm, int* ntc);
int ssv_nt_bf3_wg_per_cu(int KT, int wm, int ntc);
int ssv_precision();
enum { SSV_T_NT_FORCE, SSV_T_NNB_FORCE, SSV_T_LN_GROUPS, SSV_T_LN_PERSIST, SSV_T_LSTM_MERGE, SSV_T_PWLN_BWD, SSV_T_COUNT };
const char* ssv_tuning(int knob);
int ssv_pack_job_blocks(const ssv_pack_job& j);
int ssv_launch_pack_multi(const ssv_pack_job* jobs_dev, int njobs, int nblocks, float* amax_ws, hipStream_t st);
#define SSV_PACK_AMAX_PER_WEIGHT 32

int ssv_launch_reduce_slabs(const float* slabs, float* out, long n, int Z, long slab_stride, hipStream_t st);
int ssv_launch_reduce_slabs_perm(const float* slabs, float* out, int M, int Nc, int KT, int Z, hipStream_t st);
int ssv_launch_reduce_pair(const float* slabs, float* out, int M, int Nc, int KT, int Z, const float* part, float* pout, int n2, int nblk, hipStream_t st);
int ssv_launch_reduce_pair_multi(const ssv_wgrad_job* jobs, int njobs, const float* slabs, int M, int Nc, int KT, int Z, int n2, int nblk, hipStream_t st);
int ssv_launch_pack_wt(const float* w, float* wt, int Cout, int Cin, int KT, hipStream_t st);
int ssv_launch_fill(float* p, float v, long n, hipStream_t st);
int ssv_launch_linear_len1_fwd(const float* x, long x_bs, const float* w, const float* bias, const float* bias_b, long sbb, float* y, long y_bs,
                               int B, int K, int M, hipStream_t st);
int ssv_launch_linear_len1_wgrad(const float* dy, long dy_bs, const float* x, long x_bs, float* dw, int B, int K, int M, hipStream_t st);

static inline int ssv_cdiv(long a, long b) { return (int)((a + b - 1) / b); }
bool ssv_shape_log_on();
void ssv_shape_log(const char* kernel, dim3 grid, dim3 block, double flops, double bytes, const char* note);
__host__ __device__ static inline int ssv_amax_rows_(int L) { return 4 * ((L + 63) / 64); }

__device__ __forceinline__ unsigned ssv_xcd_order(unsigned lin, unsigned total) {
  const unsigned xcd = lin & 7u, idx = lin >> 3, q = total >> 3, r = total & 7u;
  return xcd * q + (xcd < r ? xcd : r) + idx;
}

__device__ __forceinline__ void ssv_pow2_scale(float amax, float& scale, float& inv) {
  int E = (int)((__float_as_uint(amax) >> 23) & 0xffu);
  E = min(max(E, 15), 254);
  scale = __uint_as_float((unsigned)(268 - E) << 23);
  inv = __uint_as_float((unsigned)(E - 14) << 23);
}
typedef unsigned ssv_u32x4g __attribute__((vector_size(16)));
__device__ __forceinline__ __amdgpu_buffer_rsrc_t ssv_buf(const void* base) {
  return __builtin_amdgcn_make_buffer_rsrc(const_cast<void*>(base), 0, -1, 0x00020000);
}
__device__ __forceinline__ float ssv_buf_f32(__amdgpu_buffer_rsrc_t r, unsigned voff, unsigned soff) {
  return __builtin_bit_cast(float, __builtin_amdgcn_raw_buffer_load_b32(r, (int)voff, (int)soff, 0));
}
__device__ __forceinline__ uint4 ssv_buf_u4(__amdgpu_buffer_rsrc_t r, unsigned voff, unsigned soff) {
  return __builtin_bit_cast(uint4, __builtin_amdgcn_raw_buffer_load_b128(r, (int)voff, (int)soff, 0));
}
template <class T> __device__ __forceinline__ T* ssv_global(T* p) {
  return (T*)(__attribute__((address_space(1))) T*)p;
}
__device__ __forceinline__ float ssv_uniform(float v) { return __builtin_bit_cast(float, __builtin_amdgcn_readfirstlane(__builtin_bit_cast(int, v))); }
template <int NW>
__device__ __forceinline__ float ssv_wg_max(float v, float* sm) {
#pragma unroll
  for (int o = 1; o < 64; o <<= 1) v = fmaxf(v, __shfl_xor(v, o));
  if ((threadIdx.x & 63) == 0) sm[threadIdx.x >> 6] = v;
  __syncthreads();
  float r = sm[0];
#pragma unroll
  for (int i = 1; i < NW; ++i) r = fmaxf(r, sm[i]);
  return r;
}
template <int CTRL> __device__ __forceinline__ float ssv_dpp_mov(float v);
template <int CTRL>
__device__ __forceinline__ float ssv_dpp_max(float v) { return fmaxf(v, ssv_dpp_mov<CTRL>(v)); }
__device__ __forceinline__ float ssv_wave_list_max(const float* __restrict__ p, int n) {
  float v = 0.f;
  for (int i = threadIdx.x & 63; i < n; i += 64) v = fmaxf(v, p[i]);
  v = ssv_dpp_max<0xB1>(v);
  v = ssv_dpp_max<0x4E>(v);
  v = ssv_dpp_max<0x141>(v);
  v = ssv_dpp_max<0x140>(v);
  const int b = __builtin_bit_cast(int, v);
  const float r0 = __builtin_bit_cast(float, __builtin_amdgcn_readlane(b, 0)), r1 = __builtin_bit_cast(float, __builtin_amdgcn_readlane(b, 16));
  const float r2 = __builtin_bit_cast(float, __builtin_amdgcn_readlane(b, 32)), r3 = __builtin_bit_cast(float, __builtin_amdgcn_readlane(b, 48));
  return fmaxf(fmaxf(r0, r1), fmaxf(r2, r3));
}
template <int NW>
__device__ __forceinline__ float ssv_list_max(const float* __restrict__ p, int n, float* sm) {
  float v = 0.f;
  for (int i = threadIdx.x; i < n; i += 64 * NW) v = fmaxf(v, p[i]);
  return ssv_wg_max<NW>(v, sm);
}

template <int CTRL>
__device__ __forceinline__ float ssv_dpp_mov(float v) {
  return __builtin_bit_cast(float, __builtin_amdgcn_update_dpp(0, __builtin_bit_cast(int, v), CTRL, 0xf, 0xf, true));
}
__device__ __forceinline__ float ssv_row16_sum(float v) {
  v += ssv_dpp_mov<0xB1>(v);
  v += ssv_dpp_mov<0x4E>(v);
  v += ssv_dpp_mov<0x141>(v);
  v += ssv_dpp_mov<0x140>(v);
  return v;
}
__device__ __forceinline__ float ssv_wave_sum(float v) {
  v = ssv_row16_sum(v);
  v += __shfl_xor(v, 16);
// ... 4 lines not shown
```

spoofsv_amd/csrc/ssv_host.h:

```cpp
#pragma once
#include <math.h>
#include <stdio.h>
#include <stdlib.h>
#include <string.h>
#include "ssv_common.h"
#include <type_traits>
static_assert(std::is_trivially_copyable<GemmNN>::value && std::is_trivially_copyable<GemmNT>::value && std::is_trivially_copyable<GemmNNB>::value,
              "the GEMM argument structs are kernel arguments");
#define SSV_HIP(expr) do { hipError_t _he = (expr); if (_he != hipSuccess) { ssv_fail(0, "%s: %s", #expr, hipGetErrorString(_he)); return -(int)_he; } } while (0)

static inline size_t align256(size_t n) { return (n + 255) & ~(size_t)255; }
static inline size_t zmax(size_t a, size_t b) { return a > b ? a : b; }
static inline int pad32(int n) { return (n + 31) & ~31; }

struct WsTake {
  size_t off = 0;
  size_t take(size_t bytes) { const size_t at = off; off += align256(bytes); return at; }
};
static inline float* ws_f32(void* ws, size_t off) { return (float*)((char*)ws + off); }
static inline const float* ws_f32(const void* ws, size_t off) { return (const float*)((const char*)ws + off); }
static inline unsigned short* ws_u16(void* ws, size_t off) { return (unsigned short*)((char*)ws + off); }

#define SSV_MIN_SPLIT_CHANNELS 32
static inline bool use_bf3(int B, int L, int Cin, int Cout) {
  return ssv_precision() >= 1 && (long)B * L >= 128 && Cin >= SSV_MIN_SPLIT_CHANNELS && Cout >= SSV_MIN_SPLIT_CHANNELS;
}
static inline bool use_f16() { return ssv_precision() == 2; }

static inline size_t split_bytes(int rows, int K, int k) { return align256((size_t)k * ((rows + 15) / 16 * 16) * pad32(K) * sizeof(unsigned short)); }
struct SplitPlanes { unsigned short* hi; unsigned short* lo; float* inv; };
struct PackedPlanes { SplitPlanes fwd, tr; size_t bytes; };
static inline PackedPlanes packed_planes(const void* w_packed, int Cout, int Cin, int k) {
  const size_t f = split_bytes(Cout, Cin, k), t = split_bytes(Cin, Cout, k);
  PackedPlanes p = {{nullptr, nullptr, nullptr}, {nullptr, nullptr, nullptr}, 2 * f + 2 * t + 256};
  if (char* b = (char*)w_packed) {
    p.fwd = {(unsigned short*)b, (unsigned short*)(b + f), (float*)(b + 2 * f + 2 * t)};
    p.tr = {(unsigned short*)(b + 2 * f), (unsigned short*)(b + 2 * f + t), (float*)(b + 2 * f + 2 * t + 128)};
  }
  return p;
}

#pragma GCC visibility push(hidden)
#define SSV_AMAX_FB_FLOATS 4096
#define SSV_F16_AUX_BYTES (SSV_F16_AUX_FLOATS * sizeof(float))
static const size_t AMAX_FB_BYTES = SSV_AMAX_FB_FLOATS * sizeof(float);
struct AmaxList { const float* p; int n; };
int amax_of(const float* x, long x_bs, int B, long n_item, const float* given, int ngiven, float* fb, AmaxList* out, hipStream_t st);

int conv_shifts(int k, int dilation, int causal, int* shift);
struct ConvWs { size_t main, aux, fb, total; };
ConvWs conv_ws(size_t main_bytes);
ConvWs conv_fwd_ws(int Cin, int Cout, int k);
ConvWs conv_bwd_data_ws(int Cin, int Cout, int k);
struct PwLnArgs { const float* gamma; const float* beta; float* y; long ybs; float* stats; float* y_amax; int namax; int act; };
int conv_nn(const float* x, long x_bs, const float* w, SplitPlanes packed, long w_sm, long w_sk, const float* bias, const float* bias_b,
            const float* r, long r_bs, float* y, long y_bs, int B, int K, int M, int L, int k, const int* shift,
            bool bf3, void* ws, const ConvWs& l, hipStream_t st, const float* xa_given = nullptr, int xa_n = 0,
            float* colstats = nullptr, const PwLnArgs* pw = nullptr);
#define SSV_NOMINAL_L 325
int dw_splits(int B, int M, int Nc, int k, int L);
int conv1d_bwd_weight_impl(const float* dy, long dy_bs, const float* x, long x_bs, float* dw, int B, int Cin, int Cout, int L, int k, int dilation,
                           int causal, void* ws, size_t ws_bytes, ssv_stream_t stream, const float* part, float* pgrads, int n2, int nblk,
                           const float* dy_amax, int dy_namax, const float* x_amax, int x_namax);

struct LstmWave { size_t xt, xp, out, c, bias, ih0, hh0, comb, comb_stride, aux, hp, hp_plane, l0c, x0p, total; int npad, xsplit0; };
LstmWave lstm_wave_ws(int Bn, int T, int F, int H, int layers);
int lstm_fwd_wave(const float* x, const float* const* w_ih, const float* const* w_hh, const float* const* b_ih,
                  const float* const* b_hh, float* h_last, int Bn, int T, int F, int H, int layers, char* base, hipStream_t st,
                  float* keep_xt = nullptr, float* keep_hs = nullptr, float* keep_cs = nullptr, float* keep_gates = nullptr, bool packed = false);
int lstm_gemm_f32(const float* A, const float* X, long sxb, float* C, long scb, const float* bias, const float* bias_b,
                  const float* R, int M, int K, int Bn, int nb, hipStream_t st);

#pragma GCC visibility pop

int ssv_launch_ln_gate_fwd(const float* H, long h_bs, const float* X, long x_bs, const float* g1, const float* b1, const float* g2, const float* b2,
                           float* Y, long y_bs, float* stats, int B, int C, int L, hipStream_t st, float* amax = nullptr);
int ssv_launch_ln_gate_fwd_stream(const float* H, const float* X, long x_bs, const float* colstats, const float* g1, const float* b1, const float* g2, const float* b2,
                                  float* Y, long y_bs, float* stats, float* amax, int B, int C, int L, hipStream_t st);
int ssv_launch_ln_gate_bwd(const float* dY, long dy_bs, const float* H, const float* X, long x_bs, const float* stats, const float* g1, const float* b1,
                           const float* g2, const float* b2, float* dH, float* dXres, long dx_bs, float* part, float* pgrads ,
                           int B, int C, int L, hipStream_t st, float* amax = nullptr);
int ssv_launch_ln_act_fwd(const float* X, long x_bs, const float* gam, const float* bet, float* Y, long y_bs, float* stats,
                          int B, int C, int L, int act, hipStream_t st, float* amax = nullptr);
int ssv_launch_ln_act_bwd(const float* dY, long dy_bs, const float* X, long x_bs, const float* stats, const float* gam, const float* bet,
                          float* dX, long dx_bs, float* part, float* pgrads , int B, int C, int L, int act, hipStream_t st, float* amax = nullptr);
int ssv_launch_ln_bwd2(const float* V, long v_bs, const float* GN, long gn_bs, const float* X, long x_bs, const float* stats, const float* gam,
                       float* dGN, long dgn_bs, float* dX, long dx_bs, float* part, float* dgamma, int B, int C, int L, hipStream_t st);
int ssv_launch_ln_gate_bwd2(const float* VH, const float* VX, long vx_bs, const float* GY, long gy_bs, const float* H, const float* X, long x_bs,
                            const float* stats, const float* g1, const float* b1, const float* g2, const float* b2, float* dGY, long dgy_bs,
                            float* dH, float* dX, long dx_bs, float* part, float* pgrads , int B, int C, int L, hipStream_t st);
int ssv_ln_gate_bwd_nblk(int B, int L);
int ssv_ln_gate_bwd_rows(int B, int C, int L, bool has_amax);
int ssv_ln_act_bwd_rows(int B, int C, int L, bool has_amax);
int ssv_ln_act_bwd_vec(int C, int L, bool has_amax);
int ssv_reduce_partial_rows(const float* part, float* out, int n, int nblk, hipStream_t st);

int ssv_launch_softmax_cols(float* s, int B, int N, int T, hipStream_t st);
int ssv_launch_softmax_cols_bwd(const float* a, float* da, const float* da_ext, float scale, int B, int N, int T, hipStream_t st);
int ssv_launch_softmax_cols_len(float* s, int B, int N, int T, const int* live, hipStream_t st);
bool ssv_attn_fused_ok(int B, int d, int N, int T);
int ssv_launch_attn_fwd_fused(const float* k, const float* v, long kv_bs, const float* q, long q_bs, float* a, float* rq, long rq_bs, int copy_q,
                              int B, int d, int N, int T, hipStream_t st);
int ssv_launch_attn_bwd_fused(const float* dr, long dr_bs, const float* da_ext, const float* dq_add, long dq_add_bs, const float* k, const float* v, long kv_bs,
                              const float* a, float* ds, float* dq, long dq_bs, int B, int d, int N, int T, hipStream_t st);

int ssv_launch_lstm_in_transpose(const float* x, float* xt, int Bn, int T, int F, hipStream_t st);
int ssv_launch_lstm_x_planes(const float* x, const float* amax, void* planes, long plane_bytes, int Bn, int T, int F, int kgroups, int npad, hipStream_t st);
int ssv_launch_lstm_cell(const float* g, float* c, float* h, int H, int Bn, int first, hipStream_t st);
int ssv_launch_lstm_cell_train(const float* pre, float* act, const float* cprev, float* c, float* h, int H, int Bn, hipStream_t st);
int ssv_launch_lstm_cell_bwd(const float* gates, const float* cs, const float* dxa, long zstride, int nz, const float* dh_top, float* dgates, float* dcarry,
                             float* dbp, float* amax, int H, int Bn, int T, int layers, int s, int lo, int nl, hipStream_t st);
int ssv_launch_transpose_out(const float* src, float* dst, int R, int Bn, hipStream_t st);
int ssv_launch_l2norm_rows(const float* y, float* e, float* norms, int P, int Bn, hipStream_t st);
int ssv_launch_l2norm_bwd(const float* de, const float* e, const float* norms, float* dy, int P, int Bn, hipStream_t st);
int ssv_launch_colsum(const float* x, float* out, int P, int Bn, hipStream_t st);
```

spoofsv_amd/ops.py:

```python
import collections
import contextlib
import ctypes

import torch

from . import _lib, gradarena, resident

_F32 = torch.float32


def _stream():
    return ctypes.c_void_p(torch.cuda.current_stream().cuda_stream)


def _p(t):
    return None if t is None else ctypes.c_void_p(t.data_ptr())


def _dev(t, what="tensor"):
    if not t.is_cuda:
        raise RuntimeError("spoofsv_amd: %s is on %s; the HIP hot path needs a ROCm device tensor "
                           "(no CPU fallback exists)" % (what, t.device))
    return t

# ... 35 lines not shown

class Live:
    __slots__ = ("lens", "index", "mult")

    def __init__(self, lens, index=0, mult=1):
        if lens.dtype != torch.int32 or not lens.is_cuda or lens.dim() != 1 or not 0 <= index < lens.numel():
            raise RuntimeError("Live: lens must be a 1-D int32 device tensor with an entry %d" % index)
        self.lens, self.index, self.mult = lens, int(index), int(mult)

    def ptr(self):
        return ctypes.c_void_p(self.lens.data_ptr() + 4 * self.index)


def _mask_cols(t, bs, live):
    if live is None:
        return
    B, C, L = t.shape
    _lib.call("ssv_mask_cols", _p(t), bs, B, C, L, live.ptr(), live.mult, _stream())


_AMAX_PIECES = 8


def _f16():
    return _lib.precision() == 2


_AMAX_ROWS = {}


def _amax_out(B, L, device):
    n = _AMAX_ROWS.get(L)
    if n is None:
        n = _AMAX_ROWS[L] = int(_lib.lib().ssv_amax_rows(L))
    return torch.empty((B, n), dtype=_F32, device=device)


def _tag(y, amax):
    y._ssv_amax = (amax, y._version)
    return y


def amax_of(x):
    h = getattr(x, "_ssv_amax", None)
    if h is not None and h[1] == x._version and h[0].shape[0] == x.shape[0] and h[0].device == x.device:
        return h[0]
    xd, xbs = _act3(x.detach(), "operand")
    B, C, L = xd.shape
    out = torch.empty((B, _AMAX_PIECES), dtype=_F32, device=xd.device)
    _lib.call("ssv_absmax", _p(xd), xbs, B, C * L, _p(out), _AMAX_PIECES, _stream())
    return out


def shift_right(mel):
    x, xbs = _act3(mel.detach(), "shift_right input")
    B, C, T = x.shape
    y = torch.empty((B, C, T), dtype=_F32, device=x.device)
    npb = min(C, 40)
    amax = torch.empty((B, npb), dtype=_F32, device=x.device)
    _lib.call("ssv_shift_right_amax", _p(x), xbs, _p(y), B, C, T, _p(amax), npb, _stream())
    return _tag(y, amax)


def _an(a):
    return (None, 0) if a is None else (_p(a), a.shape[1])


def _needs_grad(ctx):
    return any(ctx.needs_input_grad)


class _WgradSlot:
    __slots__ = ("pinned", "eager", "copied", "upload_pending", "captured", "captured_in_use")

    def __init__(self, cap, dev):
        self.pinned = torch.empty(cap, dtype=torch.uint8).pin_memory()
        self.eager = torch.empty(cap, dtype=torch.uint8, device=dev)
        self.copied = None
        self.upload_pending = False
        self.captured = torch.empty(cap, dtype=torch.uint8, device=dev)
        self.captured_in_use = False


_WgradJob = collections.namedtuple("_WgradJob", "dy x part dw_ptr pg_ptr storages shift dy_amax x_amax")


class DeferredWgrad:

    def __init__(self):
        self.jobs = {}
        self.slots = []
        self.cursor = 0
        self.pending = set()
        self._side = None

    def __enter__(self):
        global _DEFER
        self._prev, _DEFER = _DEFER, self
        return self

    def __exit__(self, *exc):
        global _DEFER
        _DEFER = self._prev
        return False

    def begin_step(self):
        self.cursor = 0

    def finish_uploads(self):
        if self._side is not None:
            self._side.synchronize()
        for slot in self.slots:
            slot.upload_pending = False

    def release_capture(self):
        if self._side is not None:
            self._side.synchronize()
        for slot in self.slots:
            slot.upload_pending = False
            slot.captured_in_use = False
        self.jobs = {}
        self.pending.clear()

    @staticmethod
    def accepts(B, Cin, Cout, L, k, nblk, params=()):
        if torch.is_grad_enabled() or any(p is not None and p.grad is not None for p in params):
            return False
        ok = nblk <= 768 and bool(_lib.lib().ssv_conv1d_bwd_weight_multi_ok(B, Cin, Cout, L, k))
        if _DEFER is not None:
            owners = [resident.param_of(p) for p in params if p is not None]
            if any(q in _DEFER.pending for q in owners):
                raise RuntimeError("DeferredWgrad: a parameter is used by two operators of one backward pass; deferred (batched) "
                                   "weight gradients cannot be summed by autograd -- build the step with defer_wgrad=False")
            if ok:
                _DEFER.pending.update(owners)
        return ok

    def add(self, dy, dy_bs, x, x_bs, dw, part, pg, k, dilation, causal, n2, nblk, dy_amax=None, x_amax=None):
        B, Cin, L = x.shape
        key = (B, Cin, dy.shape[1], L, k, dy_bs, x_bs, n2, nblk, x.device)
        sh = (ctypes.c_int * 3)()
        _lib.call("ssv_conv_shifts", k, dilation, int(causal), sh)
        self.jobs.setdefault(key, []).append(_WgradJob(dy, x, part, dw.data_ptr(), pg.data_ptr(), (dw.untyped_storage(), pg.untyped_storage()),
                                                       tuple(sh), dy_amax, x_amax))

    def _slot(self, nbytes, dev):
        capturing = torch.cuda.is_current_stream_capturing()
        if self.cursor == len(self.slots):
            if capturing:
                raise RuntimeError("DeferredWgrad: run one eager iteration before capturing (job tables are pinned buffers, "
                                   "which cannot be allocated during a hipGraph capture)")
            cap = max(4096, nbytes)
            self.slots.append(_WgradSlot(cap, dev))
        slot = self.slots[self.cursor]
        if slot.pinned.numel() < nbytes or slot.eager.device != dev:
            raise RuntimeError("DeferredWgrad: the sequence of weight-gradient launches changed between iterations")
        if capturing:
            if slot.upload_pending:
                raise RuntimeError("DeferredWgrad: call finish_uploads() after a capture before capturing again")
            slot.upload_pending = True
        elif slot.copied is not None:
            slot.copied.synchronize()
        self.cursor += 1
        return slot

    def flush(self):
        for key, jobs in self.jobs.items():
            B, Cin, Cout, L, k, dy_bs, x_bs, n2, nblk, dev = key
            n = len(jobs)
            table = (_lib.WgradJob * n)()
            f16 = _f16()
            for t, j in zip(table, jobs):
                t.dy, t.x, t.dw, t.part, t.pgrads = j.dy.data_ptr(), j.x.data_ptr(), j.dw_ptr, j.part.data_ptr(), j.pg_ptr
                t.shift[0], t.shift[1], t.shift[2] = j.shift
                if f16:
                    if j.dy_amax is None or j.x_amax is None:
                        raise RuntimeError("DeferredWgrad: a job was queued without operand scales in the split-fp16 mode")
                    t.dy_amax, t.x_amax, t.dy_namax, t.x_namax = j.dy_amax.data_ptr(), j.x_amax.data_ptr(), j.dy_amax.numel(), j.x_amax.numel()
            raw = bytes(table)
            slot = self._slot(len(raw), dev)
            slot.pinned[:len(raw)].copy_(torch.frombuffer(bytearray(raw), dtype=torch.uint8))
            if torch.cuda.is_current_stream_capturing():
                if slot.captured_in_use:
                    raise RuntimeError("DeferredWgrad: this instance already serves a captured step (its frozen job tables are in use); "
                                       "build a new step object for another capture")
                slot.captured_in_use = True
                dtable = slot.captured
                if self._side is None:
                    self._side = torch.cuda.Stream(device=dev)
                with torch.cuda.stream(self._side):
                    dtable.copy_(slot.pinned, non_blocking=True)
                    slot.copied = torch.cuda.Event()
                    slot.copied.record()
            else:
                dtable = slot.eager
                dtable.copy_(slot.pinned, non_blocking=True)
                slot.copied = torch.cuda.Event()
                slot.copied.record()
            nb = _lib.query("ssv_conv1d_bwd_weight_multi_workspace", n, B, Cin, Cout, L, k)
            ws = _ws(nb, dev)
            max_shift = max(abs(v) for j in jobs for v in j.shift)
            _lib.call("ssv_conv1d_bwd_weight_multi", _p(dtable), n, dy_bs, x_bs, B, Cin, Cout, L, k, max_shift, n2, nblk, _p(ws), nb, _stream())
        self.jobs = {}
        self.pending.clear()


_DEFER = None


class HighwayConvFn(torch.autograd.Function):

    @staticmethod
    def forward(ctx, x, w, bias, g1, b1, g2, b2, k, dilation, causal, x_amax=None, y_amax=None, live=None):
        x, xbs = _act3(x, "highwayConv input")
        B, C, L = x.shape
        w, bias, g1, b1, g2, b2 = map(_c, (w, bias, g1, b1, g2, b2))
        if tuple(w.shape) != (2 * C, C, k):
            raise RuntimeError("highwayConv: weight %s does not match input channels %d" % (tuple(w.shape), C))
        train = _needs_grad(ctx)
        y = torch.empty((B, C, L), dtype=_F32, device=x.device)
        h = torch.empty((B, 2 * C, L), dtype=_F32, device=x.device)
        stats = torch.empty((B, 4, L), dtype=_F32, device=x.device) if train else None
        nb = _lib.query("ssv_highway_conv1d_fwd_workspace", B, C, L, k)
        ws = _ws(nb, x.device)
        _lib.call("ssv_highway_conv1d_fwd", _p(x), xbs, *_an(x_amax), _p(w), resident.lookup(w), _p(bias), _p(g1), _p(b1), _p(g2), _p(b2),
                  _p(h), _p(stats), _p(y), C * L, _p(y_amax), B, C, L, k, dilation, int(causal), _p(ws), nb, _stream())
        _mask_cols(y, C * L, live)
        if train:
            ctx.save_for_backward(x, w, g1, b1, g2, b2, h, stats)
            ctx.x_amax = x_amax
            ctx.live = live
            ctx.cfg = (k, dilation, int(causal))
            ctx.bias_ref = bias
        return y

    @staticmethod
    def backward(ctx, dy):
        x, w, g1, b1, g2, b2, h, stats = ctx.saved_tensors
        k, dilation, causal = ctx.cfg
        x, xbs = _act3(x)
        dy, dybs = _act3(dy, "highwayConv grad")
        _mask_cols(dy, dybs, ctx.live)
        B, C, L = x.shape
        dx = torch.empty((B, C, L), dtype=_F32, device=x.device)
        dw = gradarena.grad_like(w)
        bias = ctx.bias_ref
        pg = gradarena.grad_block((g1, b1, g2, b2, bias), 6, C, x.device) if bias is not None else torch.empty((6, C), dtype=_F32, device=x.device)
        nblk = _lib.query("ssv_ln_partial_rows", B, L)
        if _DEFER is not None and _DEFER.accepts(B, C, 2 * C, L, k, nblk, (w, g1, b1, g2, b2, bias)):
            dh = torch.empty((B, 2 * C, L), dtype=_F32, device=x.device)
            part = torch.empty((nblk, 6 * C), dtype=_F32, device=x.device)
            f16 = _f16()
            dh_amax = _amax_out(B, L, x.device) if f16 else None
            x_amax = (ctx.x_amax if ctx.x_amax is not None else amax_of(x)) if f16 else None
            rows = _lib.query("ssv_ln_bwd_partial_rows", 1, B, C, L, int(f16))
            nb = _lib.query("ssv_highway_conv1d_bwd_data_workspace", B, C, L, k)
            ws = _ws(nb, x.device)
            _lib.call("ssv_highway_conv1d_bwd_data", _p(dy), dybs, _p(x), xbs, _p(w), resident.lookup(w), _p(g1), _p(b1), _p(g2), _p(b2),
                      _p(h), _p(stats), _p(dx), C * L, _p(dh), _p(dh_amax), _p(part), B, C, L, k, dilation, causal, _p(ws), nb, _stream())
            _DEFER.add(dh, 2 * C * L, x, xbs, dw, part, pg, k, dilation, causal, 6 * C, rows, dh_amax, x_amax)
            return (dx, dw, pg[4:6].reshape(2 * C), pg[0], pg[1], pg[2], pg[3]) + (None,) * 6
        nb = _lib.query("ssv_highway_conv1d_bwd_workspace", B, C, L, k)
        ws = _ws(nb, x.device)
        _lib.call("ssv_highway_conv1d_bwd", _p(dy), dybs, _p(x), xbs, *_an(ctx.x_amax), _p(w), resident.lookup(w), _p(g1), _p(b1), _p(g2), _p(b2),
                  _p(h), _p(stats), _p(dx), C * L, _p(dw), _p(pg), B, C, L, k, dilation, causal,
                  _p(ws), nb, _stream())
        return (dx, dw, pg[4:6].reshape(2 * C), pg[0], pg[1], pg[2], pg[3]) + (None,) * 6


def _conv_fwd(x, xbs, w, bias, bias_b, y, ybs, k, dilation, causal, x_amax=None):
    B, Cin, L = x.shape
    nb = _lib.query("ssv_conv1d_fwd_workspace", Cin, w.shape[0], k)
    ws = _ws(nb, x.device)
    _lib.call("ssv_conv1d_fwd", _p(x), xbs, *_an(x_amax), _p(w), resident.lookup(w), _p(bias), _p(bias_b), _p(y), ybs, None, B, Cin, w.shape[0], L,
              k, dilation, int(causal), _p(ws), nb, _stream())


def _conv_bwd_data(dy, dybs, w, Cin, L, k=1, dilation=1, causal=0, dy_amax=None):
    B, Cout = dy.shape[0], w.shape[0]
    dx = torch.empty((B, Cin, L), dtype=_F32, device=dy.device)
    nb = _lib.query("ssv_conv1d_bwd_data_workspace", Cin, Cout, k)
    ws = _ws(nb, dy.device)
    _lib.call("ssv_conv1d_bwd_data", _p(dy), dybs, *_an(dy_amax), _p(w), resident.lookup(w), None, _p(dx), Cin * L, B, Cin, Cout, L, k, dilation,
              int(causal), _p(ws), nb, _stream())
    return dx


def _conv_bwd_weight(dy, dybs, x, xbs, wshape, k=1, dilation=1, causal=0, out=None, dy_amax=None, x_amax=None):
    B, Cin, L = x.shape
    Cout = wshape[0]
    dw = out if out is not None else torch.empty(wshape, dtype=_F32, device=x.device)
    nb = _lib.query("ssv_conv1d_bwd_weight_workspace", B, Cin, Cout, L, k)
    ws = _ws(nb, x.device)
    _lib.call("ssv_conv1d_bwd_weight", _p(dy), dybs, *_an(dy_amax), _p(x), xbs, *_an(x_amax), _p(dw), B, Cin, Cout, L, k, dilation, int(causal),
              _p(ws), nb, _stream())
    return dw


def _sum_over_batch(rows, B, n, out=None):
    if out is None:
        out = torch.empty((n,), dtype=_F32, device=rows.device)
    _lib.call("ssv_sum_slabs", _p(rows), _p(out), n, B, n, _stream())
    return out


class PointwiseConvLnActFn(torch.autograd.Function):

    @staticmethod
    def forward(ctx, x, w, bias, gamma, beta, s, act, x_amax=None, y_amax=None, live=None):
        x, xbs = _act3(x, "conv input")
        B, Cin, L = x.shape
        w, bias, gamma, beta = map(_c, (w, bias, gamma, beta))
        Cout = w.shape[0]
        if w.shape[1] != Cin or w.shape[2] != 1:
            raise RuntimeError("pointwise conv: weight %s does not match input channels %d" % (tuple(w.shape), Cin))
        sb = None
        if s is not None:
            sb = _c(s.reshape(B, Cout))
        train = _needs_grad(ctx)
        pre = torch.empty((B, Cout, L), dtype=_F32, device=x.device)
        y = torch.empty((B, Cout, L), dtype=_F32, device=x.device)
        stats = torch.empty((B, 2, L), dtype=_F32, device=x.device) if train else None
        nb = _lib.query("ssv_pointwise_conv_ln_act_fwd_workspace", Cin, Cout)
        ws = _ws(nb, x.device)
        _lib.call("ssv_pointwise_conv_ln_act_fwd", _p(x), xbs, *_an(x_amax), _p(w), resident.lookup(w), _p(bias), _p(sb), _p(gamma), _p(beta),
                  _p(pre), _p(stats), _p(y), Cout * L, _p(y_amax), B, Cin, Cout, L, act, _p(ws), nb, _stream())
        _mask_cols(y, Cout * L, live)
        if train:
            ctx.save_for_backward(x, w, gamma, beta, pre, stats)
            ctx.x_amax = x_amax
            ctx.live = live
            ctx.act = act
            ctx.bias_ref = bias
            ctx.has_s = s is not None
            ctx.need_dx = ctx.needs_input_grad[0]
        return y

    @staticmethod
    def backward(ctx, dy):
        x, w, gamma, beta, pre, stats = ctx.saved_tensors
        x, xbs = _act3(x)
        dy, dybs = _act3(dy, "grad")
        _mask_cols(dy, dybs, ctx.live)
        B, Cin, L = x.shape
        Cout = w.shape[0]
        pg = gradarena.grad_block((gamma, beta, ctx.bias_ref), 3, Cout, x.device)
        dx = torch.empty((B, Cin, L), dtype=_F32, device=x.device) if ctx.need_dx else None
        dw = gradarena.grad_like(w)
        ds = torch.empty((B, Cout, 1), dtype=_F32, device=x.device) if ctx.has_s else None
        nblk = _lib.query("ssv_ln_partial_rows", B, L)
        if _DEFER is not None and _DEFER.accepts(B, Cin, Cout, L, 1, nblk, (w, gamma, beta, ctx.bias_ref)):
            dpre = torch.empty((B, Cout, L), dtype=_F32, device=x.device)
            part = torch.empty((nblk, 3 * Cout), dtype=_F32, device=x.device)
            f16 = _f16()
            dpre_amax = _amax_out(B, L, x.device) if f16 else None
            x_amax = (ctx.x_amax if ctx.x_amax is not None else amax_of(x)) if f16 else None
            rows = _lib.query("ssv_ln_bwd_partial_rows", 0, B, Cout, L, int(f16))
            nb = _lib.query("ssv_pointwise_conv_ln_act_bwd_data_workspace", B, Cin, Cout, L)
            ws = _ws(nb, x.device)
            _lib.call("ssv_pointwise_conv_ln_act_bwd_data", _p(dy), dybs, _p(w), resident.lookup(w), _p(gamma), _p(beta), _p(pre), _p(stats),
                      _p(dx), Cin * L, _p(ds), _p(dpre), _p(dpre_amax), _p(part), B, Cin, Cout, L, ctx.act, _p(ws), nb, _stream())
            _DEFER.add(dpre, Cout * L, x, xbs, dw, part, pg, 1, 1, 0, 3 * Cout, rows, dpre_amax, x_amax)
            return dx, dw, pg[2], pg[0], pg[1], ds, None, None, None, None
        nb = _lib.query("ssv_pointwise_conv_ln_act_bwd_workspace", B, Cin, Cout, L)
        ws = _ws(nb, x.device)
        _lib.call("ssv_pointwise_conv_ln_act_bwd", _p(dy), dybs, _p(x), xbs, *_an(ctx.x_amax), _p(w), resident.lookup(w), _p(gamma), _p(beta), _p(pre), _p(stats),
                  _p(dx), Cin * L, _p(dw), _p(pg), _p(ds), B, Cin, Cout, L, ctx.act, _p(ws), nb, _stream())
        return dx, dw, pg[2], pg[0], pg[1], ds, None, None, None, None


class Conv1dFn(torch.autograd.Function):

    @staticmethod
    def forward(ctx, x, w, bias, k, dilation, causal, x_amax=None):
        x, xbs = _act3(x, "conv input")
        B, Cin, L = x.shape
        w = _c(w)
        bias = _c(bias) if bias is not None else None
        Cout = w.shape[0]
        y = torch.empty((B, Cout, L), dtype=_F32, device=x.device)
        _conv_fwd(x, xbs, w, bias, None, y, Cout * L, k, dilation, causal, x_amax)
        if _needs_grad(ctx):
            ctx.save_for_backward(x, w)
            ctx.x_amax = x_amax
            ctx.cfg = (k, dilation, int(causal), ctx.needs_input_grad[0], bias is not None)
            ctx.bias_ref = bias
        return y

    @staticmethod
    def backward(ctx, dy):
        x, w = ctx.saved_tensors
        k, dilation, causal, need_dx, has_bias = ctx.cfg
        x, xbs = _act3(x)
        dy, dybs = _act3(dy, "grad")
        B, Cin, L = x.shape
        Cout = w.shape[0]
        dy_amax = amax_of(dy) if (_f16() and _bf3_shape(dy)) else None
        dx = _conv_bwd_data(dy, dybs, w, Cin, L, k, dilation, causal, dy_amax) if need_dx else None
        dw = _conv_bwd_weight(dy, dybs, x, xbs, tuple(w.shape), k, dilation, causal, out=gradarena.view(w), dy_amax=dy_amax, x_amax=ctx.x_amax)
        db = None
        if has_bias:
            db = gradarena.view(ctx.bias_ref)
            if db is None:
                db = torch.empty((Cout,), dtype=_F32, device=x.device)
            _lib.call("ssv_bias_grad", _p(dy), dybs, _p(db), B, Cout, L, _stream())
        return dx, dw, db, None, None, None, None


def _tiny_conv(cin, cout):
    return min(int(cin), int(cout)) < 32


def _dd_amax(t, cin=None, cout=None):
    if t is None or not (_f16() and _bf3_shape(t)) or (cin is not None and _tiny_conv(cin, cout)):
        return None
    return amax_of(t)


_INPUT_ONLY = None


def _skip_param_grads(*params):
    if _INPUT_ONLY is None:
        return False
    return all(p is not None and resident.param_of(p) in _INPUT_ONLY for p in params)


@contextlib.contextmanager
def input_grads_only(module):
    global _INPUT_ONLY
    prev, _INPUT_ONLY = _INPUT_ONLY, frozenset(module.parameters())
    try:
        yield
    finally:
        _INPUT_ONLY = prev


class ConvFwdDD(torch.autograd.Function):

    @staticmethod
    def forward(ctx, x, w, bias, k, dilation, causal, x_amax=None):
        x, xbs = _act3(x, "conv input")
        w = _c(w)
        bias = _c(bias) if bias is not None else None
        B, Cin, L = x.shape
        y = torch.empty((B, w.shape[0], L), dtype=_F32, device=x.device)
        _conv_fwd(x, xbs, w, bias, None, y, w.shape[0] * L, k, dilation, causal, x_amax)
        ctx.save_for_backward(x, w)
        ctx.x_amax = x_amax
        ctx.cfg = (k, dilation, causal, bias is not None)
        return y

    @staticmethod
    def backward(ctx, dy):
        x, w = ctx.saved_tensors
        k, dilation, causal, has_bias = ctx.cfg
        dya = _dd_amax(dy, x.shape[1], w.shape[0])
        dx = ConvBwdDataDD.apply(dy, w, x.shape[1], k, dilation, causal, dya) if ctx.needs_input_grad[0] else None
        if _skip_param_grads(w):
            return dx, None, None, None, None, None, None
        dw = ConvBwdWeightDD.apply(dy, x, k, dilation, causal, dya, ctx.x_amax) if ctx.needs_input_grad[1] else None
        db = BiasGradFn.apply(dy) if (has_bias and ctx.needs_input_grad[2]) else None
        return dx, dw, db, None, None, None, None


class BiasGradFn(torch.autograd.Function):

    @staticmethod
    def forward(ctx, dy):
        dy, dybs = _act3(dy, "grad")
        B, C, L = dy.shape
        rows = torch.empty((B, C), dtype=_F32, device=dy.device)
        _lib.call("ssv_rowsum", _p(dy), dybs, _p(rows), B, C, L, _stream())
        ctx.dims = (B, C, L)
        return _sum_over_batch(rows, B, C)

    @staticmethod
    def backward(ctx, g):
        B, C, L = ctx.dims
        return g.view(1, C, 1).expand(B, C, L)


# ... 462 lines not shown
    kv, kvbs = _act3(kv, "K|V")
    q, qbs = _act3(q, "Q")
    B, d2, N = kv.shape
    d, T = q.shape[1], q.shape[2]
    pma = pma.long().contiguous()
    out = torch.empty((B,), dtype=torch.int64, device=q.device)
    q_last = ctypes.c_void_p(q.data_ptr() + 4 * (T - 1))
    _lib.call("ssv_attention_step", ctypes.c_void_p(kv.data_ptr()), kvbs, q_last, qbs, T, _p(pma), _p(a_buf),
              a_buf.shape[2], col, None, _p(out), B, d, N, _stream())
    return out


def attention_step_dev(kv, q, pma, a_buf, col_dev):
    kv, kvbs = _act3(kv, "K|V")
    q, qbs = _act3(q, "Q")
    B, d2, N = kv.shape
    d, T = q.shape[1], q.shape[2]
    _lib.call("ssv_attention_step", ctypes.c_void_p(kv.data_ptr()), kvbs, _p(q), qbs, T, _p(pma), _p(a_buf),
              a_buf.shape[2], 0, _p(col_dev), _p(pma), B, d, N, _stream())


def synth_advance(y, mel_in, col_dev):
    B, F, T = y.shape
    _lib.call("ssv_synth_advance", _p(y), _p(mel_in), _p(col_dev), B, F, T, _stream())


def attention_apply(kv, a_buf, q, T):
    kv, kvbs = _act3(kv, "K|V")
    q, qbs = _act3(q, "Q")
    B, d2, N = kv.shape
    d = q.shape[1]
    rq = torch.empty((B, 2 * d, T), dtype=_F32, device=q.device)
    _lib.call("ssv_attention_apply", ctypes.c_void_p(kv.data_ptr() + 4 * d * N), kvbs, _p(a_buf), a_buf.shape[2],
              _p(rq), 2 * d * T, B, d, N, T, _stream())
    _lib.call("ssv_copy_rows", _p(q), qbs, ctypes.c_void_p(rq.data_ptr() + 4 * d * T), 2 * d * T, B, d * T, _stream())
    return rq


class DeconvK2S2Fn(torch.autograd.Function):

    @staticmethod
    def forward(ctx, x, w, bias, x_amax=None, y_amax=None, live=None):
        x, xbs = _act3(x, "deconv input")
        B, Cin, L = x.shape
        w, bias = _c(w), _c(bias)
        Cout = w.shape[1]
        if w.shape[0] != Cin or w.shape[2] != 2:
            raise RuntimeError("deconv: weight %s does not match input channels %d / kernel 2" % (tuple(w.shape), Cin))
        y = torch.empty((B, Cout, 2 * L), dtype=_F32, device=x.device)
        nb = _lib.query("ssv_deconv1d_k2s2_fwd_workspace", Cin, Cout)
        ws = _ws(nb, x.device)
        _lib.call("ssv_deconv1d_k2s2_fwd", _p(x), xbs, *_an(x_amax), _p(w), resident.lookup(w.view(Cin, 2 * Cout, 1)), _p(bias), _p(y), Cout * 2 * L,
                  _p(y_amax), 64, B, Cin, Cout, L, _p(ws), nb, _stream())
        _mask_cols(y, Cout * 2 * L, live)
        if _needs_grad(ctx):
            ctx.live = live
            ctx.save_for_backward(x, w)
            ctx.bias_ref = bias
            ctx.x_amax = x_amax
        return y

    @staticmethod
    def backward(ctx, dy):
        x, w = ctx.saved_tensors
        x, xbs = _act3(x)
        dy, dybs = _act3(dy, "grad")
        _mask_cols(dy, dybs, ctx.live)
        B, Cin, L = x.shape
        Cout = w.shape[1]
        dx = torch.empty((B, Cin, L), dtype=_F32, device=x.device)
        dw = gradarena.grad_like(w)
        db = gradarena.grad_like(ctx.bias_ref)
        nb = _lib.query("ssv_deconv1d_k2s2_bwd_workspace", B, Cin, Cout)
        ws = _ws(nb, x.device)
        split = _lib.precision() >= 1 and B * L >= 256 and L >= 8 and dybs == Cout * 2 * L
        if split:
            f16 = _f16()
            du = torch.empty((B, 2 * Cout, L), dtype=_F32, device=x.device)
            du_am = torch.empty((B, 64), dtype=_F32, device=x.device) if f16 else None
            _lib.call("ssv_deinterleave2_rows_amax", _p(dy), dybs, _p(du), B, Cout, L, _p(du_am), 64, _stream())
            w2 = w.view(Cin, 2 * Cout, 1)
            _conv_fwd(du, 2 * Cout * L, w2, None, None, dx, Cin * L, 1, 1, 0, du_am)
            x_am = (ctx.x_amax if ctx.x_amax is not None else amax_of(x)) if f16 else None
            _conv_bwd_weight(x, xbs, du, 2 * Cout * L, (Cin, 2 * Cout, 1), 1, 1, 0, dw.view(Cin, 2 * Cout, 1), x_am, du_am)
            _lib.call("ssv_bias_grad", _p(dy), dybs, _p(db), B, Cout, 2 * L, _stream())
            return dx, dw, db, None, None, None
        _lib.call("ssv_deconv1d_k2s2_bwd", _p(dy), dybs, None, 0, _p(x), xbs, _p(w), _p(dx), Cin * L, _p(dw), _p(db),
                  B, Cin, Cout, L, _p(ws), nb, _stream())
        return dx, dw, db, None, None, None


class SpecLossFn(torch.autograd.Function):

    @staticmethod
    def forward(ctx, y, gt, seed=None, live=None):
        y, gt = _c(y), _c(gt)
        if y.shape != gt.shape:
            raise RuntimeError("spec loss: prediction %s vs target %s" % (tuple(y.shape), tuple(gt.shape)))
        n = y.numel()
        out = torch.empty((2,), dtype=_F32, device=y.device)
        nb = _lib.query("ssv_spec_losses_workspace", n)
        ws = _ws(nb, y.device)
        ctx.fused = None
        ctx.live = live
        if live is not None and y.dim() != 3:
            raise RuntimeError("spec loss: a length-masked loss needs (B, C, L) tensors, got %s" % (tuple(y.shape),))
        if seed is not None and ctx.needs_input_grad[0]:
            if seed.dtype != _F32 or seed.numel() != 2 or seed.device != y.device or not seed.is_contiguous():
                raise RuntimeError("spec loss: the promised gradient seed must be a contiguous float32 2-vector on the prediction's device")
            dy = torch.empty_like(y)
            if live is None:
                _lib.call("ssv_spec_losses_fwd_bwd", _p(y), _p(gt), n, _p(seed), _p(out), _p(dy), _p(ws), nb, _stream())
            else:
                _lib.call("ssv_spec_losses_len", _p(y), _p(gt), *y.shape, live.ptr(), live.mult, _p(seed), _p(out), _p(dy), _p(ws), nb, _stream())
            ctx.fused = (dy, seed, seed._version)
        elif live is None:
            _lib.call("ssv_spec_losses_fwd", _p(y), _p(gt), n, _p(out), _p(ws), nb, _stream())
        else:
            _lib.call("ssv_spec_losses_len", _p(y), _p(gt), *y.shape, live.ptr(), live.mult, None, _p(out), None, _p(ws), nb, _stream())
        ctx.save_for_backward(y, gt)
        return out

    @staticmethod
    def backward(ctx, gout):
        y, gt = ctx.saved_tensors
        f = ctx.fused
        if f is not None and gout is f[1] and gout._version == f[2]:
            return f[0], None, None, None
        ctx.fused = None
        gout = _c(gout)
        dy = torch.empty_like(y)
        live = ctx.live
        if live is None:
            _lib.call("ssv_spec_losses_bwd", _p(y), _p(gt), y.numel(), _p(gout), _p(dy), _stream())
        else:
            nb = _lib.query("ssv_spec_losses_workspace", y.numel())
            scratch = torch.empty((2,), dtype=_F32, device=y.device)
            _lib.call("ssv_spec_losses_len", _p(y), _p(gt), *y.shape, live.ptr(), live.mult, _p(gout), _p(scratch), _p(dy),
                      _p(_ws(nb, y.device)), nb, _stream())
        return dy, None, None, None


class GuidedAttLossFn(torch.autograd.Function):

    @staticmethod
    def forward(ctx, a, gaw, live=None):
        a, gaw = _c(a), _c(gaw)
        B, N, T = a.shape
        if gaw.shape[0] < N or gaw.shape[1] < T:
            raise RuntimeError("guided attention: weight %s smaller than attention %s" % (tuple(gaw.shape), tuple(a.shape)))
        out = torch.empty((1,), dtype=_F32, device=a.device)
        nb = _lib.query("ssv_guided_att_loss_workspace", B, N, T)
        ws = _ws(nb, a.device)
        if live is None:
            _lib.call("ssv_guided_att_loss_fwd", _p(a), _p(gaw), gaw.shape[1], _p(out), B, N, T, _p(ws), nb, _stream())
        else:
            _lib.call("ssv_guided_att_loss_fwd_len", _p(a), _p(gaw), gaw.shape[1], _p(out), B, N, T, live.ptr(), _p(ws), nb, _stream())
        ctx.live = live
        ctx.save_for_backward(gaw)
        ctx.dims = (B, N, T)
        return out

    @staticmethod
    def backward(ctx, gout):
        (gaw,) = ctx.saved_tensors
        B, N, T = ctx.dims
        gout = _c(gout)
# ... 71 lines not shown
```

spoofsv_amd/resident.py:

```python
import ctypes
import weakref

import numpy as np
import torch

from . import _lib

_LIVE = weakref.WeakSet()
_INFER = weakref.WeakKeyDictionary()


class _Entry:
    __slots__ = ("planes", "shape", "version", "addr", "owner")

    def __reduce__(self):
        return type(None), ()


def param_of(t):
    return t if t._base is None else t._base


def lookup(w):
    p = param_of(w)
    e = getattr(p, "_ssv_planes", None)
    if (e is None or e.version != p._version or e.addr != p.data_ptr() or w.data_ptr() != e.addr or e.shape != tuple(w.shape)
            or e.owner() is None):
        return None
    return e.planes


def _owner(p):
    e = getattr(p, "_ssv_planes", None)
    return e.owner() if e is not None else None


def invalidate(params=None):
    for p in ([p for rw in _LIVE for p in rw.params] if params is None else params):
        e = getattr(p, "_ssv_planes", None)
        if e is not None:
            e.version = -1


def mark_transposed(p):
    p._ssv_transposed = True
    return p


def eligible(p):
    return (p.is_cuda and p.dtype == torch.float32 and p.dim() == 3 and p.is_contiguous()
            and p.shape[2] in ((2,) if getattr(p, "_ssv_transposed", False) else (1, 3)))


def pack_shape(p):
    return (p.shape[0], 2 * p.shape[1], 1) if getattr(p, "_ssv_transposed", False) else tuple(p.shape)


class ResidentWeights:

    def __init__(self, params):
        self.params = [p for p in params if eligible(p)]
        self._key = None
        self._jobs = None
        self._nblocks = 0
        _LIVE.add(self)

    def _build(self):
        key = tuple(p.data_ptr() for p in self.params)
        if key == self._key:
            return
        n = len(self.params)
        dev = self.params[0].device
        sizes = [int(_lib.query("ssv_conv_pack_bytes", *pack_shape(p))) for p in self.params]
        self._planes = [torch.empty(s, dtype=torch.uint8, device=dev) for s in sizes]
        vp = ctypes.c_void_p
        w = (vp * n)(*[p.data_ptr() for p in self.params])
        pl = (vp * n)(*[t.data_ptr() for t in self._planes])
        ci = lambda k: (ctypes.c_int * n)(*[pack_shape(p)[k] for p in self.params])
        jobs = (_lib.PackJob * (2 * n))()
        nblocks = _lib.lib().ssv_conv_pack_plan(n, w, pl, ci(0), ci(1), ci(2), jobs)
        if nblocks < 0:
            raise RuntimeError("ssv_conv_pack_plan: " + _lib.lib().ssv_last_error().decode())
        raw = np.frombuffer(bytes(jobs), dtype=np.uint8).copy()
        host = torch.from_numpy(raw).pin_memory()
        self._jobs = torch.empty(raw.size, dtype=torch.uint8, device=dev)
        self._jobs.copy_(host, non_blocking=False)
        self._nblocks, self._njobs = nblocks, 2 * n
        self._ws_bytes = int(_lib.query("ssv_conv_pack_multi_workspace", 2 * n))
        self._ws = torch.empty(max(self._ws_bytes, 256), dtype=torch.uint8, device=dev)
        me = weakref.ref(self)
        for p, t in zip(self.params, self._planes):
            e = p._ssv_planes = _Entry()
            e.planes, e.shape, e.version, e.addr, e.owner = ctypes.c_void_p(t.data_ptr()), pack_shape(p), -1, None, me
        self._key = key

    def refresh(self, stream):
        if not self.params:
            return
        self._build()
        _lib.call("ssv_conv_pack_multi", ctypes.c_void_p(self._jobs.data_ptr()), self._njobs, self._nblocks,
                  ctypes.c_void_p(self._ws.data_ptr()), self._ws_bytes, stream)
        for p in self.params:
            if _owner(p) is self:
                p._ssv_planes.version, p._ssv_planes.addr = p._version, p.data_ptr()


def ensure(module, stream):
    mine = [p for p in module.parameters() if eligible(p)]
    rw = _INFER.get(module)
    owners = {id(o): o for o in map(_owner, mine)}
    if owners and not any(o is None or o is rw for o in owners.values()):
        if any(lookup(p) is None for p in mine):
            for o in owners.values():
                o.refresh(stream)
        return next(iter(owners.values()))
    if rw is None or [id(p) for p in rw.params] != [id(p) for p in mine]:
        rw = _INFER[module] = ResidentWeights(mine)
    if any(lookup(p) is None for p in rw.params):
        rw.refresh(stream)
    return rw
```

spoofsv_amd/train.py:

```python
import ctypes
import os
import contextlib
import gc
import time
from types import SimpleNamespace

import numpy as np
import torch
import torch.distributed as dist

from . import _lib, ops, tts
from . import resident as _resident
from .ops import _p, _stream


def init_weights(layer):
    if hasattr(layer, "weight"):
        if len(layer.weight.shape) > 1:
            torch.nn.init.kaiming_normal_(layer.weight, nonlinearity="relu")


def guided_attention_mat(max_text_len, max_frame_num, device=None, g=0.2):
    n = torch.arange(max_text_len, dtype=torch.float64).unsqueeze(1) / max_text_len
    t = torch.arange(max_frame_num, dtype=torch.float64).unsqueeze(0) / max_frame_num
    W = (1 - torch.exp(-(t - n) ** 2 / (2 * g * g))).float()
    return W.to(device) if device is not None else W


_CHUNK = 32768



@contextlib.contextmanager
def _no_gc():
    gc.collect()
    was = gc.isenabled()
    gc.disable()
    try:
        yield
    finally:
        if was:
            gc.enable()

class FusedAdam(torch.optim.Optimizer):

    def __init__(self, params, lr=1e-3, betas=(0.9, 0.999), eps=1e-8, capturable=False, resident=True,
                 weight_decay=0, amsgrad=False, maximize=False):
        if weight_decay != 0 or amsgrad or maximize:
            raise ValueError("FusedAdam implements plain Adam as the reference uses it (train/ordinary.py:182): "
                             "weight_decay, amsgrad and maximize are not supported")
        super().__init__(params, dict(lr=lr, betas=betas, eps=eps, weight_decay=0, amsgrad=False, maximize=False,
                                      foreach=None, capturable=False, differentiable=False, fused=None,
                                      decoupled_weight_decay=False))
        self.capturable = capturable
        self._table = None
        self._upload = None
        self._key = None
        self._step_dev = None
        self._steps = 0
        self._resident = None
        self.resident = resident

    def refresh_resident_weights(self):
        if not self.resident:
            return
        if self._resident is None:
            self._resident = _resident.ResidentWeights([p for g in self.param_groups for p in g["params"]])
        self._resident.refresh(_stream())

    _CHUNK_STRUCT = _lib.AdamChunk
    _COLS = 5

    def _moments(self, p):
        st = self.state[p]
        if "exp_avg" not in st:
            st["step"] = torch.tensor(0.0)
            st["exp_avg"] = torch.zeros_like(p, memory_format=torch.contiguous_format)
            st["exp_avg_sq"] = torch.zeros_like(p, memory_format=torch.contiguous_format)
        return st["exp_avg"], st["exp_avg_sq"]

    def _check_rows(self, rows):
        pass

    def _launch(self, group, step_dev):
        b1, b2 = group["betas"]
        _lib.call("ssv_adam_multi", _p(self._table), self._nchunks, float(group["lr"]), float(b1), float(b2),
                  float(group["eps"]), self._steps, step_dev, _stream())

    def _build(self, plist):
        key = tuple((p.data_ptr(), p.grad.data_ptr()) for p in plist)
        if key == self._key:
            return
        rows = []
        for p in plist:
            moments = self._moments(p)
            if not (p.is_contiguous() and p.grad.is_contiguous() and p.dtype == torch.float32 and p.grad.dtype == torch.float32):
                raise RuntimeError("FusedAdam needs dense float32 parameters and gradients")
            n = p.numel()
            for off in range(0, n, _CHUNK):
                m = min(_CHUNK, n - off)
                rows.append((p.data_ptr() + 4 * off, p.grad.data_ptr() + 4 * off) + tuple(0 if t is None else t.data_ptr() + 4 * off for t in moments) + (m,))
        self._check_rows(rows)
        arr = np.array(rows, dtype=np.int64)
        cols = self._COLS
        assert ctypes.sizeof(self._CHUNK_STRUCT) == 8 * cols and arr.shape[1] == cols
        if self._upload is None:
            cap = sum((p.numel() + _CHUNK - 1) // _CHUNK for g in self.param_groups for p in g["params"])
            self._table = torch.empty((cap, cols), dtype=torch.int64, device=plist[0].device)
            self._upload = StagedUpload(self._table)
        self._upload.host()[:len(rows)].copy_(torch.from_numpy(arr))
        self._upload.send()
        self._nchunks = len(rows)
        self._key = key

    @torch.no_grad()
    def step(self, closure=None):
        loss = closure() if closure is not None else None
        if len(self.param_groups) != 1:
            raise RuntimeError("FusedAdam keeps one device-side step counter: use one parameter group")
        for group in self.param_groups:
            plist = [p for p in group["params"] if p.grad is not None]
            if not plist:
                continue
            ops._dev(plist[0], "parameter")
            self._build(plist)
            self._steps += 1
            step_dev = None
            if self.capturable:
                if self._step_dev is None:
                    self._step_dev = torch.full((1,), self._steps - 1, dtype=torch.int32, device=plist[0].device)
                step_dev = _p(self._step_dev)
            self._launch(group, step_dev)
        self.refresh_resident_weights()
        return loss

    def state_dict(self):
        if self._step_dev is not None:
            self._steps = int(self._step_dev.item())
        for st in self.state.values():
            if "exp_avg" in st:
                st["step"] = torch.tensor(float(self._steps))
        return super().state_dict()

    def load_state_dict(self, state_dict):
        super().load_state_dict(state_dict)
        steps = [int(st["step"]) for st in self.state.values() if "step" in st]
        self._steps = max(steps) if steps else 0
        if self._step_dev is not None:
            self._step_dev.fill_(self._steps)
        self._key = None


def check_adam_ex_rows(rows, amsgrad):
    for i, r in enumerate(rows):
        if len(r) != 6:
            raise ValueError("adam_ex chunk %d has %d fields, expected (p, g, m, v, vmax, n)" % (i, len(r)))
        if not (r[0] and r[1] and r[2] and r[3]) or int(r[5]) <= 0:
            raise ValueError("adam_ex chunk %d: null p, g, m or v, or n = %d" % (i, int(r[5])))
        if amsgrad and not r[4]:
            raise ValueError("adam_ex chunk %d: amsgrad needs max_exp_avg_sq, got a null vmax" % i)


class FusedAdamEx(FusedAdam):

    _CHUNK_STRUCT = _lib.AdamExChunk
    _COLS = 6

    def __init__(self, params, lr=1e-3, betas=(0.9, 0.999), eps=1e-8, weight_decay=0, amsgrad=False, capturable=False, resident=True):
        if weight_decay < 0:
            raise ValueError("Invalid weight_decay value: %r" % (weight_decay,))
        super().__init__(params, lr, betas, eps, capturable=capturable, resident=resident)
        self.defaults.update(weight_decay=weight_decay, amsgrad=bool(amsgrad))
        for g in self.param_groups:
            g.update(weight_decay=weight_decay, amsgrad=bool(amsgrad))

    def _moments(self, p):
        m, v = super()._moments(p)
        st = self.state[p]
        if not self.param_groups[0]["amsgrad"]:
            return m, v, None
        if "max_exp_avg_sq" not in st:
            st["max_exp_avg_sq"] = torch.zeros_like(p, memory_format=torch.contiguous_format)
        return m, v, st["max_exp_avg_sq"]

    def _check_rows(self, rows):
        check_adam_ex_rows(rows, self.param_groups[0]["amsgrad"])

    def _launch(self, group, step_dev):
        b1, b2 = group["betas"]
        _lib.call("ssv_adam_ex_multi", _p(self._table), self._nchunks, float(group["lr"]), float(b1), float(b2), float(group["eps"]),
                  float(group["weight_decay"]), int(bool(group["amsgrad"])), self._steps, step_dev, _stream())


class TrainingSnapshot:

    _MOMENTS = ("exp_avg", "exp_avg_sq", "max_exp_avg_sq")

    def __init__(self, modules, optimizers):
        self.modules, self.optimizers = list(modules), list(optimizers)

    def _tensors(self):
        return [t for m in self.modules for t in list(m.parameters()) + list(m.buffers())]

    def _sync(self):
        tensors = self._tensors()
        if tensors and tensors[0].is_cuda:
            torch.cuda.synchronize()

    def __enter__(self):
        return self.take()

    def __exit__(self, exc_type, exc, tb):
        if exc_type is None:
            self._sync()
            self.restore()

# ... 806 lines not shown
```

Baseline: 889,900 mel-frames/s.

## Batch deferred wgrad slab reductions and fuse Adam amax into resident weight repack

Weight-gradient GEMMs with split-K slabs can now skip their per-layer reduce step and queue it, so one multi-job reduce kernel folds the slabs and LN partial rows for many layers at once. The Adam kernel also gains a variant that records a per-chunk absolute max. The resident fp16 weight repack then reads these maxima, through a per-parameter chunk range table, instead of running its own amax pass, and it defers the step-counter increment. Together these aim to cut kernel launches and redundant passes over weights and gradients in the tail of the step. The cost is more bookkeeping and more paths that must stay consistent, with a legacy knob kept as a fallback.

```diff
diff --git a/include/ssv_hip.h b/include/ssv_hip.h
--- a/include/ssv_hip.h
+++ b/include/ssv_hip.h
@@ -70,6 +70,17 @@
 size_t ssv_conv1d_bwd_weight_multi_workspace(int njobs, int B, int Cin, int Cout, int L, int k);
 int ssv_conv1d_bwd_weight_multi(const ssv_wgrad_job* jobs_dev, int njobs, long dy_bs, long x_bs, int B, int Cin, int Cout, int L, int k, int max_shift,
                                 int n2, int nblk, void* ws, size_t ws_bytes, ssv_stream_t stream);
+int ssv_conv1d_bwd_weight_multi_gemm(const ssv_wgrad_job* jobs_dev, int njobs, long dy_bs, long x_bs, int B, int Cin, int Cout, int L, int k, int max_shift,
+                                     int n2, int nblk, void* ws, size_t ws_bytes, ssv_stream_t stream);
+int ssv_conv1d_bwd_weight_slabs(const float* dy, long dy_bs, const float* dy_amax, int dy_namax, const float* x, long x_bs, const float* x_amax, int x_namax,
+                                float* dw, const float* part, float* pgrads, int n2, int nblk, int B, int Cin, int Cout, int L, int k, int dilation, int causal,
+                                void* ws, size_t ws_bytes, ssv_stream_t stream);
+typedef struct {
+  const float* slabs; float* dw; const float* part; float* pgrads;
+  int M, Nc, KT, Z; int n2, nblk; int first_block, pad_;
+} ssv_reduce_job;
+int ssv_wgrad_reduce_plan(ssv_reduce_job* jobs_host, int njobs);
+int ssv_wgrad_reduce_jobs(const ssv_reduce_job* jobs_dev, int njobs, int nblocks, ssv_stream_t stream);
 int ssv_ln_partial_rows(int B, int L);
 int ssv_ln_bwd_partial_rows(int gate, int B, int C, int L, int with_amax);
 size_t ssv_highway_conv1d_bwd_data_workspace(int B, int C, int L, int k);
@@ -158,10 +169,15 @@
                        ssv_pack_job* jobs_host);
 size_t ssv_conv_pack_multi_workspace(int njobs);
 int ssv_conv_pack_multi(const ssv_pack_job* jobs_dev, int njobs, int nblocks, void* ws, size_t ws_bytes, ssv_stream_t stream);
+int ssv_conv_pack_multi_from(const ssv_pack_job* jobs_dev, int njobs, int nblocks, const float* chunk_amax, const int* ranges_dev, int* step_inc,
+                             ssv_stream_t stream);
 
 typedef struct { float* p; const float* g; float* m; float* v; long n; } ssv_adam_chunk;
 int ssv_adam_multi(const ssv_adam_chunk* chunks, int nchunks, float lr, float beta1, float beta2, float eps,
                    int step, int* step_dev, ssv_stream_t stream);
+int ssv_adam_multi_amax(const ssv_adam_chunk* chunks, int nchunks, float lr, float beta1, float beta2, float eps,
+                        int step, int* step_dev, float* chunk_amax, int defer_step_inc, ssv_stream_t stream);
+int ssv_tail_legacy(void);
 
 size_t ssv_lstm_fwd_workspace(int Bn, int T, int F, int H, int layers);
 int ssv_lstm_fwd(const float* x, const float* const* w_ih, const float* const* w_hh,
diff --git a/spoofsv_amd/_lib.py b/spoofsv_amd/_lib.py
--- a/spoofsv_amd/_lib.py
+++ b/spoofsv_amd/_lib.py
@@ -32,6 +32,16 @@
     _fields_ = [("dy", ctypes.c_void_p), ("x", ctypes.c_void_p), ("dw", ctypes.c_void_p), ("part", ctypes.c_void_p),
                 ("pgrads", ctypes.c_void_p), ("shift", ctypes.c_int * 3), ("pad_", ctypes.c_int),
                 ("dy_amax", ctypes.c_void_p), ("x_amax", ctypes.c_void_p), ("dy_namax", ctypes.c_int), ("x_namax", ctypes.c_int)]
+
+
+class ReduceJob(ctypes.Structure):
+    _fields_ = [("slabs", ctypes.c_void_p), ("dw", ctypes.c_void_p), ("part", ctypes.c_void_p), ("pgrads", ctypes.c_void_p),
+                ("M", ctypes.c_int), ("Nc", ctypes.c_int), ("KT", ctypes.c_int), ("Z", ctypes.c_int),
+                ("n2", ctypes.c_int), ("nblk", ctypes.c_int), ("first_block", ctypes.c_int), ("pad_", ctypes.c_int)]
+
+
+def tail_legacy():
+    return bool(lib().ssv_tail_legacy())
 
 
 def _ctype(decl):
diff --git a/spoofsv_amd/csrc/api.hip b/spoofsv_amd/csrc/api.hip
--- a/spoofsv_amd/csrc/api.hip
+++ b/spoofsv_amd/csrc/api.hip
@@ -36,7 +36,7 @@
   }
   return g_precision;
 }
-static const char* const g_knob_names[SSV_T_COUNT] = {"SSV_NT_FORCE", "SSV_NNB_FORCE", "SSV_LN_GROUPS", "SSV_LN_PERSIST", "SSV_LSTM_MERGE", "SSV_PWLN_BWD"};
+static const char* const g_knob_names[SSV_T_COUNT] = {"SSV_NT_FORCE", "SSV_NNB_FORCE", "SSV_LN_GROUPS", "SSV_LN_PERSIST", "SSV_LSTM_MERGE", "SSV_PWLN_BWD", "SSV_TAIL_LEGACY"};
 static char g_knob_val[SSV_T_COUNT][512];
 static const char* g_knob[SSV_T_COUNT];
 static int g_knobs_loaded = 0;
@@ -53,6 +53,7 @@
   return g_knob[knob];
 }
 extern "C" void ssv_reload_tuning(void) { load_knobs(); }
+extern "C" int ssv_tail_legacy(void) { const char* e = ssv_tuning(SSV_T_TAIL_LEGACY); return e && !strcmp(e, "1") ? 1 : 0; }
 #include <mutex>
 #include <string>
 #include <map>
diff --git a/spoofsv_amd/csrc/api_conv.hip b/spoofsv_amd/csrc/api_conv.hip
--- a/spoofsv_amd/csrc/api_conv.hip
+++ b/spoofsv_amd/csrc/api_conv.hip
@@ -157,6 +157,12 @@
   SSV_CHECK(!f16 || (ws && ws_bytes >= ssv_conv_pack_multi_workspace(njobs)), SSV_BAD_SHAPE, "conv_pack_multi: workspace too small");
   return ssv_launch_pack_multi(jobs_dev, njobs, nblocks, f16 ? (float*)ws : nullptr, (hipStream_t)stream);
 }
+extern "C" int ssv_conv_pack_multi_from(const ssv_pack_job* jobs_dev, int njobs, int nblocks, const float* chunk_amax, const int* ranges_dev, int* step_inc,
+                                        ssv_stream_t stream) {
+  SSV_CHECK(jobs_dev && njobs > 0 && njobs % 2 == 0 && nblocks > 0 && chunk_amax && ranges_dev, SSV_BAD_SHAPE, "conv_pack_multi_from: bad argument");
+  SSV_CHECK(use_f16(), SSV_UNSUPPORTED, "conv_pack_multi_from: only the split-fp16 planes take a scale (use ssv_conv_pack_multi)");
+  return ssv_launch_pack_multi_from(jobs_dev, njobs, nblocks, chunk_amax, ranges_dev, step_inc, (hipStream_t)stream);
+}
 
 static int nt_slabs(long tiles_all, int njobs, int B, int L, int kt, int M, int Nc) {
   int wm, ntc;
@@ -225,7 +231,8 @@
 extern "C" size_t ssv_conv1d_bwd_weight_workspace(int B, int Cin, int Cout, int L, int k) { return wgrad_ws(B, Cin, Cout, L, k).total; }
 int conv1d_bwd_weight_impl(const float* dy, long dy_bs, const float* x, long x_bs, float* dw, int B, int Cin, int Cout, int L, int k, int dilation,
                            int causal, void* ws, size_t ws_bytes, ssv_stream_t stream, const float* part, float* pgrads, int n2, int nblk,
-                           const float* dy_amax, int dy_namax, const float* x_amax, int x_namax) {
+                           const float* dy_amax, int dy_namax, const float* x_amax, int x_namax, int* left_z) {
+  if (left_z) *left_z = 0;
   SSV_CHECK(dy && x && dw && B > 0 && Cin > 0 && Cout > 0 && L > 0, SSV_BAD_SHAPE, "conv1d_bwd_weight: bad argument");
   const WgradWs l = wgrad_ws(B, Cin, Cout, L, k);
   SSV_CHECK(ws && ws_bytes >= l.total, SSV_BAD_SHAPE, "conv1d_bwd_weight: workspace too small");
@@ -252,6 +259,7 @@
       g.f16 = 1; g.a_amax = la.p; g.a_namax = la.n * B; g.x_amax = lx.p; g.x_namax = lx.n * B;
     }
     SSV_TRY(ssv_launch_gemm_nt_bf3(g, st));
+    if (left_z && Z > 1 && (!part || nblk <= 768)) { *left_z = Z; return 0; }
   } else if (L == 1 && k == 1) {
     SSV_TRY(ssv_launch_linear_len1_wgrad(dy, dy_bs, x, x_bs, dw, B, Cin, Cout, st));
     if (part) SSV_TRY(ssv_reduce_partial_rows(part, pgrads, n2, nblk, st));
@@ -269,6 +277,36 @@
                                      void* ws, size_t ws_bytes, ssv_stream_t stream) {
   return conv1d_bwd_weight_impl(dy, dy_bs, x, x_bs, dw, B, Cin, Cout, L, k, dilation, causal, ws, ws_bytes, stream, nullptr, nullptr, 0, 0,
                                 dy_amax, dy_namax, x_amax, x_namax);
+}
+extern "C" int ssv_conv1d_bwd_weight_slabs(const float* dy, long dy_bs, const float* dy_amax, int dy_namax, const float* x, long x_bs, const float* x_amax,
+                                           int x_namax, float* dw, const float* part, float* pgrads, int n2, int nblk, int B, int Cin, int Cout, int L, int k,
+                                           int dilation, int causal, void* ws, size_t ws_bytes, ssv_stream_t stream) {
+  SSV_CHECK(!part || (pgrads && n2 > 0 && nblk > 0), SSV_BAD_SHAPE, "conv1d_bwd_weight_slabs: partial rows without pgrads / n2 / nblk");
+  static_assert(sizeof(ssv_reduce_job) == 64, "ssv_reduce_job is mirrored by the callers");
+  int left = 0;
+  SSV_TRY(conv1d_bwd_weight_impl(dy, dy_bs, x, x_bs, dw, B, Cin, Cout, L, k, dilation, causal, ws, ws_bytes, stream, part, pgrads, part ? n2 : 0, part ? nblk : 0,
+                                 dy_amax, dy_namax, x_amax, x_namax, &left));
+  return left;
+}
+extern "C" int ssv_wgrad_reduce_plan(ssv_reduce_job* jobs, int njobs) {
+  SSV_CHECK(jobs && njobs > 0, SSV_BAD_SHAPE, "wgrad_reduce_plan: bad argument");
+  long blocks = 0;
+  for (int i = 0; i < njobs; ++i) {
+    ssv_reduce_job& j = jobs[i];
+    SSV_CHECK(j.slabs && j.dw && j.M > 0 && j.Nc > 0 && j.KT >= 1 && j.KT <= 3 && j.Z >= 1, SSV_BAD_SHAPE, "wgrad_reduce_plan: job %d: bad shape M=%d Nc=%d KT=%d Z=%d",
+              i, j.M, j.Nc, j.KT, j.Z);
+    if (j.part) SSV_CHECK(j.pgrads && j.n2 > 0 && j.nblk > 0, SSV_BAD_SHAPE, "wgrad_reduce_plan: job %d: partial rows without pgrads / n2 / nblk", i);
+    else { j.pgrads = nullptr; j.n2 = 0; j.nblk = 0; }
+    SSV_CHECK(j.nblk <= 768, SSV_UNSUPPORTED, "wgrad_reduce_plan: job %d: %d partial rows (max 768)", i, j.nblk);
+    j.first_block = (int)blocks; j.pad_ = 0;
+    blocks += ssv_reduce_job_blocks(j);
+    SSV_CHECK(blocks < (1L << 30), SSV_UNSUPPORTED, "wgrad_reduce_plan: too many elements");
+  }
+  return (int)blocks;
+}
+extern "C" int ssv_wgrad_reduce_jobs(const ssv_reduce_job* jobs_dev, int njobs, int nblocks, ssv_stream_t stream) {
+  SSV_CHECK(jobs_dev && njobs > 0 && nblocks > 0, SSV_BAD_SHAPE, "wgrad_reduce_jobs: bad argument");
+  return ssv_launch_reduce_jobs(jobs_dev, njobs, nblocks, (hipStream_t)stream);
 }
 
 extern "C" int ssv_conv1d_bwd_weight_multi_ok(int B, int Cin, int Cout, int L, int k) {
@@ -287,8 +325,8 @@
 extern "C" size_t ssv_conv1d_bwd_weight_multi_workspace(int njobs, int B, int Cin, int Cout, int L, int k) {
   return align256((size_t)njobs * ssv_conv1d_bwd_weight_multi_splits(njobs, B, Cin, Cout, L, k) * Cout * Cin * k * sizeof(float));
 }
-extern "C" int ssv_conv1d_bwd_weight_multi(const ssv_wgrad_job* jobs_dev, int njobs, long dy_bs, long x_bs, int B, int Cin, int Cout, int L, int k, int max_shift,
-                                           int n2, int nblk, void* ws, size_t ws_bytes, ssv_stream_t stream) {
+static int wgrad_multi_gemm(const ssv_wgrad_job* jobs_dev, int njobs, long dy_bs, long x_bs, int B, int Cin, int Cout, int L, int k, int max_shift,
+                            int n2, int nblk, void* ws, size_t ws_bytes, ssv_stream_t stream, int* z_out) {
   SSV_CHECK(jobs_dev && njobs > 0 && B > 0 && Cin > 0 && Cout > 0 && L > 0, SSV_BAD_SHAPE, "conv1d_bwd_weight_multi: bad argument");
   SSV_CHECK(ssv_conv1d_bwd_weight_multi_ok(B, Cin, Cout, L, k), SSV_UNSUPPORTED, "conv1d_bwd_weight_multi: shape or arithmetic mode not supported");
   SSV_CHECK(n2 == 0 || nblk <= 768, SSV_UNSUPPORTED, "conv1d_bwd_weight_multi: %d partial rows (max 768)", nblk);
@@ -303,8 +341,19 @@
   g.M = Cout; g.Nc = Cin; g.KT = k; g.B = B; g.Z = Z; g.bstep = (k != 3 && ssv_nt_bf3_xrow(1, Cout, Cin)) ? 0 : Z;
   g.jobs = jobs_dev; g.njobs = njobs; g.max_shift = max_shift;
   g.f16 = use_f16() ? 1 : 0;
-  SSV_TRY(ssv_launch_gemm_nt_bf3(g, st));
-  return ssv_launch_reduce_pair_multi(jobs_dev, njobs, (const float*)ws, Cout, Cin, k, Z, n2, nblk, st);
+  *z_out = Z;
+  return ssv_launch_gemm_nt_bf3(g, st);
+}
+extern "C" int ssv_conv1d_bwd_weight_multi(const ssv_wgrad_job* jobs_dev, int njobs, long dy_bs, long x_bs, int B, int Cin, int Cout, int L, int k, int max_shift,
+                                           int n2, int nblk, void* ws, size_t ws_bytes, ssv_stream_t stream) {
+  int Z = 0;
+  SSV_TRY(wgrad_multi_gemm(jobs_dev, njobs, dy_bs, x_bs, B, Cin, Cout, L, k, max_shift, n2, nblk, ws, ws_bytes, stream, &Z));
+  return ssv_launch_reduce_pair_multi(jobs_dev, njobs, (const float*)ws, Cout, Cin, k, Z, n2, nblk, (hipStream_t)stream);
+}
+extern "C" int ssv_conv1d_bwd_weight_multi_gemm(const ssv_wgrad_job* jobs_dev, int njobs, long dy_bs, long x_bs, int B, int Cin, int Cout, int L, int k, int max_shift,
+                                                int n2, int nblk, void* ws, size_t ws_bytes, ssv_stream_t stream) {
+  int Z = 0;
+  return wgrad_multi_gemm(jobs_dev, njobs, dy_bs, x_bs, B, Cin, Cout, L, k, max_shift, n2, nblk, ws, ws_bytes, stream, &Z);
 }
 
 static ConvWs deconv_fwd_ws(int Cin, int Cout) { return conv_ws(2 * split_bytes(Cout, Cin, 2)); }
diff --git a/spoofsv_amd/csrc/misc.hip b/spoofsv_amd/csrc/misc.hip
--- a/spoofsv_amd/csrc/misc.hip
+++ b/spoofsv_amd/csrc/misc.hip
@@ -96,6 +96,19 @@
   for (; k < nblk; k += 8) a[0] += part[(long)k * n2 + i];
   return (((a[0] + a[1]) + (a[2] + a[3])) + ((a[4] + a[5]) + (a[6] + a[7]))) + (((a[8] + a[9]) + (a[10] + a[11])) + ((a[12] + a[13]) + (a[14] + a[15])));
 }
+template <typename P>
+__device__ __forceinline__ void reduce_part_block(P part, float* __restrict__ pout, int n2, int nblk, int block, float (*red)[32] ) {
+  const int li = threadIdx.x & 31, rg = threadIdx.x >> 5;
+  const int i = block * 32 + li;
+  red[rg][li] = i < n2 ? ssv_fold_rows(part, n2, nblk, i, rg) : 0.f;
+  __syncthreads();
+  if (rg == 0 && i < n2) {
+    float t = 0.f;
+#pragma unroll
+    for (int r = 0; r < 8; ++r) t += red[r][li];
+    pout[i] = t;
+  }
+}
 __global__ __launch_bounds__(256) void reduce_pair_kernel(const float* __restrict__ s, float* __restrict__ out, int Nc, int KT, long n, int Z, int nA,
                                                           const float* __restrict__ part, float* __restrict__ pout, int n2, int nblk) {
   __shared__ float red[8][32];
@@ -104,16 +117,7 @@
     reduce_perm_block(s, out, Nc, KT, n, Z, (int)blockIdx.x, stage);
     return;
   }
-  const int li = threadIdx.x & 31, rg = threadIdx.x >> 5;
-  const int i = ((int)blockIdx.x - nA) * 32 + li;
-  red[rg][li] = i < n2 ? ssv_fold_rows(part, n2, nblk, i, rg) : 0.f;
-  __syncthreads();
-  if (rg == 0 && i < n2) {
-    float t = 0.f;
-#pragma unroll
-    for (int r = 0; r < 8; ++r) t += red[r][li];
-    pout[i] = t;
-  }
+  reduce_part_block(part, pout, n2, nblk, (int)blockIdx.x - nA, red);
 }
 int ssv_launch_reduce_pair(const float* slabs, float* out, int M, int Nc, int KT, int Z, const float* part, float* pout, int n2, int nblk, hipStream_t st) {
   const long n = (long)M * Nc * KT;
@@ -134,22 +138,39 @@
   }
   if (!jb.part) return;
   const __attribute__((address_space(1))) float* __restrict__ part = (const __attribute__((address_space(1))) float*)jb.part;
-  const int li = threadIdx.x & 31, rg = threadIdx.x >> 5;
-  const int i = ((int)blockIdx.x - nA) * 32 + li;
-  red[rg][li] = i < n2 ? ssv_fold_rows(part, n2, nblk, i, rg) : 0.f;
-  __syncthreads();
-  if (rg == 0 && i < n2) {
-    float t = 0.f;
-#pragma unroll
-    for (int r = 0; r < 8; ++r) t += red[r][li];
-    jb.pgrads[i] = t;
-  }
+  reduce_part_block(part, jb.pgrads, n2, nblk, (int)blockIdx.x - nA, red);
 }
 int ssv_launch_reduce_pair_multi(const ssv_wgrad_job* jobs, int njobs, const float* slabs, int M, int Nc, int KT, int Z, int n2, int nblk, hipStream_t st) {
   const long n = (long)M * Nc * KT;
   const int nA = ssv_cdiv((long)M * Nc, 256), nB = n2 > 0 ? ssv_cdiv(n2, 32) : 0;
   hipLaunchKernelGGL(reduce_pair_multi_kernel, dim3(nA + nB, njobs), dim3(256), 0, st, jobs, slabs, Nc, KT, n, Z, nA, n2, nblk);
   return ssv_check_launch("reduce_pair_multi");
+}
+
+__host__ __device__ static inline int reduce_job_nA(int M, int Nc) { return (int)(((long)M * Nc + 255) / 256); }
+__global__ __launch_bounds__(256) void reduce_jobs_kernel(const ssv_reduce_job* __restrict__ jobs, int njobs) {
+  __shared__ float red[8][32];
+  __shared__ __attribute__((aligned(16))) float stage[256 * 3];
+  int lo = 0, hi = njobs - 1;
+  while (lo < hi) {
+    const int mid = (lo + hi + 1) >> 1;
+    if (jobs[mid].first_block <= (int)blockIdx.x) lo = mid; else hi = mid - 1;
+  }
+  const ssv_reduce_job jb = jobs[lo];
+  const int block = (int)blockIdx.x - jb.first_block;
+  const int nA = reduce_job_nA(jb.M, jb.Nc);
+  if (block < nA) {
+    reduce_perm_block(ssv_global(jb.slabs), ssv_global(jb.dw), jb.Nc, jb.KT, (long)jb.M * jb.Nc * jb.KT, jb.Z, block, stage);
+    return;
+  }
+  if (!jb.part || (long)(block - nA) * 32 >= jb.n2) return;
+  const __attribute__((address_space(1))) float* __restrict__ part = (const __attribute__((address_space(1))) float*)jb.part;
+  reduce_part_block(part, ssv_global(jb.pgrads), jb.n2, jb.nblk, block - nA, red);
+}
+int ssv_reduce_job_blocks(const ssv_reduce_job& j) { return reduce_job_nA(j.M, j.Nc) + (j.part ? ssv_cdiv(j.n2, 32) : 0); }
+int ssv_launch_reduce_jobs(const ssv_reduce_job* jobs_dev, int njobs, int nblocks, hipStream_t st) {
+  hipLaunchKernelGGL(reduce_jobs_kernel, dim3(nblocks), dim3(256), 0, st, jobs_dev, njobs);
+  return ssv_check_launch("reduce_jobs");
 }
 
 __global__ __launch_bounds__(256) void pack_wt_kernel(const float* __restrict__ w, float* __restrict__ wt, int Cout, int Cin, int KT) {
@@ -688,16 +709,29 @@
   return ssv_check_launch("gatt_bwd_len");
 }
 
+template <int AMAX>
 __global__ __launch_bounds__(256) void adam_multi_kernel(const ssv_adam_chunk* __restrict__ chunks, float lr, float b1, float b2, float eps,
-                                                         int step_host, const int* __restrict__ step_dev) {
+                                                         int step_host, const int* __restrict__ step_dev, float* __restrict__ chunk_amax) {
+#pragma clang fp contract(off)
   const int step = step_dev ? step_dev[0] + 1 : step_host;
   const double bc1 = 1.0 - pow((double)b1, (double)step), bc2 = 1.0 - pow((double)b2, (double)step);
   const float step_size = (float)((double)lr / bc1), inv_sqrt_bc2 = (float)(1.0 / sqrt(bc2));
   const ssv_adam_chunk ch = chunks[blockIdx.x];
+  float amx = 0.f;
+  const float nb1 = 1.f - b1, nb2 = 1.f - b2;
+  auto step_p = [&](float& p, const float m, const float v) {
+    p = __builtin_fmaf(-step_size, m / __builtin_fmaf(sqrtf(v), inv_sqrt_bc2, eps), p);
+    if constexpr (AMAX) amx = fmaxf(amx, fabsf(p));
+  };
   auto upd = [&](float& p, float g, float& m, float& v) {
-    m = b1 * m + (1.f - b1) * g;
-    v = b2 * v + (1.f - b2) * g * g;
-    p -= step_size * (m / (sqrtf(v) * inv_sqrt_bc2 + eps));
+    m = __builtin_fmaf(b1, m, nb1 * g);
+    v = __builtin_fmaf(b2, v, (nb2 * g) * g);
+    step_p(p, m, v);
+  };
+  auto upd_tail = [&](float& p, float g, float& m, float& v) {
+    m = __builtin_fmaf(nb1, g, b1 * m);
+    v = b2 * v + (nb2 * g) * g;
+    step_p(p, m, v);
   };
   long i0 = 0;
   if ((((uintptr_t)ch.p | (uintptr_t)ch.g | (uintptr_t)ch.m | (uintptr_t)ch.v) & 15) == 0) {
@@ -733,19 +767,34 @@
   }
   for (long i = i0 + threadIdx.x; i < ch.n; i += 256) {
     float p = ch.p[i], m = ch.m[i], v = ch.v[i];
-    upd(p, ch.g[i], m, v);
+    upd_tail(p, ch.g[i], m, v);
     ch.p[i] = p; ch.m[i] = m; ch.v[i] = v;
   }
+  if constexpr (AMAX) {
+    __shared__ float amax_sm[4];
+    amx = ssv_wg_max<4>(amx, amax_sm);
+    if (threadIdx.x == 0) chunk_amax[blockIdx.x] = amx;
+  }
 }
 __global__ void step_inc_kernel(int* step_dev) { step_dev[0] += 1; }
+static int adam_multi_launch(const ssv_adam_chunk* chunks, int nchunks, float lr, float beta1, float beta2, float eps, int step, int* step_dev,
+                             float* chunk_amax, bool inc, hipStream_t st) {
+  if (chunk_amax) hipLaunchKernelGGL(adam_multi_kernel<1>, dim3(nchunks), dim3(256), 0, st, chunks, lr, beta1, beta2, eps, step, (const int*)step_dev, chunk_amax);
+  else hipLaunchKernelGGL(adam_multi_kernel<0>, dim3(nchunks), dim3(256), 0, st, chunks, lr, beta1, beta2, eps, step, (const int*)step_dev, (float*)nullptr);
+  SSV_TRY(ssv_check_launch("adam_multi"));
+  if (step_dev && inc) {
+    hipLaunchKernelGGL(step_inc_kernel, dim3(1), dim3(1), 0, st, step_dev);
+    return ssv_check_launch("step_inc");
+  }
+  return 0;
+}
 extern "C" int ssv_adam_multi(const ssv_adam_chunk* chunks, int nchunks, float lr, float beta1, float beta2, float eps,
                               int step, int* step_dev, ssv_stream_t stream) {
   SSV_CHECK(nchunks > 0 && (step_dev || step > 0), SSV_BAD_SHAPE, "adam_multi: nchunks=%d step=%d", nchunks, step);
-  hipLaunchKernelGGL(adam_multi_kernel, dim3(nchunks), dim3(256), 0, (hipStream_t)stream, chunks, lr, beta1, beta2, eps, step, (const int*)step_dev);
-  SSV_TRY(ssv_check_launch("adam_multi"));
-  if (step_dev) {
-    hipLaunchKernelGGL(step_inc_kernel, dim3(1), dim3(1), 0, (hipStream_t)stream, step_dev);
-    return ssv_check_launch("step_inc");
-  }
-  return 0;
-}
+  return adam_multi_launch(chunks, nchunks, lr, beta1, beta2, eps, step, step_dev, nullptr, true, (hipStream_t)stream);
+}
+extern "C" int ssv_adam_multi_amax(const ssv_adam_chunk* chunks, int nchunks, float lr, float beta1, float beta2, float eps,
+                                   int step, int* step_dev, float* chunk_amax, int defer_step_inc, ssv_stream_t stream) {
+  SSV_CHECK(nchunks > 0 && (step_dev || step > 0) && chunk_amax, SSV_BAD_SHAPE, "adam_multi_amax: nchunks=%d step=%d chunk_amax=%p", nchunks, step, (void*)chunk_amax);
+  return adam_multi_launch(chunks, nchunks, lr, beta1, beta2, eps, step, step_dev, chunk_amax, !defer_step_inc, (hipStream_t)stream);
+}
diff --git a/spoofsv_amd/csrc/pack.hip b/spoofsv_amd/csrc/pack.hip
--- a/spoofsv_amd/csrc/pack.hip
+++ b/spoofsv_amd/csrc/pack.hip
@@ -167,8 +167,10 @@
   }
 }
 template <int F16>
-__global__ __launch_bounds__(256) void pack_multi_kernel(const ssv_pack_job* __restrict__ jobs, int njobs, const float* __restrict__ amax) {
+__global__ __launch_bounds__(256) void pack_multi_kernel(const ssv_pack_job* __restrict__ jobs, int njobs, const float* __restrict__ amax,
+                                                         const int* __restrict__ ranges, int* __restrict__ step_inc) {
   __shared__ float smx[4];
+  if (step_inc && blockIdx.x == 0 && threadIdx.x == 0) step_inc[0] += 1;
   int lo = 0, hi = njobs - 1;
   while (lo < hi) {
     const int mid = (lo + hi + 1) >> 1;
@@ -177,7 +179,9 @@
   const ssv_pack_job j = jobs[lo];
   float sc = 1.f, inv = 1.f;
   if constexpr (F16) {
-    ssv_pow2_scale(ssv_list_max<4>(amax + (long)(lo >> 1) * SSV_PACK_AMAX_PER_WEIGHT, SSV_PACK_AMAX_PER_WEIGHT, smx), sc, inv);
+    const float mx = ranges ? ssv_list_max<4>(amax + ranges[2 * (lo >> 1)], ranges[2 * (lo >> 1) + 1], smx)
+                            : ssv_list_max<4>(amax + (long)(lo >> 1) * SSV_PACK_AMAX_PER_WEIGHT, SSV_PACK_AMAX_PER_WEIGHT, smx);
+    ssv_pow2_scale(mx, sc, inv);
     if ((int)blockIdx.x == j.first_block && threadIdx.x == 0 && j.inv_out) *j.inv_out = inv;
   }
   const long slots = (long)((j.M + 15) >> 4) * (j.Kpad >> 5) * 64;
@@ -195,9 +199,13 @@
   if (amax_ws) {
     hipLaunchKernelGGL(pack_amax_multi_kernel, dim3(SSV_PACK_AMAX_PER_WEIGHT, njobs / 2), dim3(256), 0, st, jobs_dev, amax_ws);
     SSV_TRY(ssv_check_launch("pack_amax_multi"));
-    hipLaunchKernelGGL(pack_multi_kernel<1>, dim3(nblocks), dim3(256), 0, st, jobs_dev, njobs, (const float*)amax_ws);
+    hipLaunchKernelGGL(pack_multi_kernel<1>, dim3(nblocks), dim3(256), 0, st, jobs_dev, njobs, (const float*)amax_ws, (const int*)nullptr, (int*)nullptr);
   } else {
-    hipLaunchKernelGGL(pack_multi_kernel<0>, dim3(nblocks), dim3(256), 0, st, jobs_dev, njobs, (const float*)nullptr);
+    hipLaunchKernelGGL(pack_multi_kernel<0>, dim3(nblocks), dim3(256), 0, st, jobs_dev, njobs, (const float*)nullptr, (const int*)nullptr, (int*)nullptr);
   }
   return ssv_check_launch("pack_multi");
 }
+int ssv_launch_pack_multi_from(const ssv_pack_job* jobs_dev, int njobs, int nblocks, const float* chunk_amax, const int* ranges_dev, int* step_inc, hipStream_t st) {
+  hipLaunchKernelGGL(pack_multi_kernel<1>, dim3(nblocks), dim3(256), 0, st, jobs_dev, njobs, chunk_amax, ranges_dev, step_inc);
+  return ssv_check_launch("pack_multi");
+}
diff --git a/spoofsv_amd/csrc/ssv_common.h b/spoofsv_amd/csrc/ssv_common.h
--- a/spoofsv_amd/csrc/ssv_common.h
+++ b/spoofsv_amd/csrc/ssv_common.h
@@ -90,16 +90,19 @@
 void ssv_nt_bf3_tile(int KT, int M, int Nc, int* wm, int* ntc);
 int ssv_nt_bf3_wg_per_cu(int KT, int wm, int ntc);
 int ssv_precision();
-enum { SSV_T_NT_FORCE, SSV_T_NNB_FORCE, SSV_T_LN_GROUPS, SSV_T_LN_PERSIST, SSV_T_LSTM_MERGE, SSV_T_PWLN_BWD, SSV_T_COUNT };
+enum { SSV_T_NT_FORCE, SSV_T_NNB_FORCE, SSV_T_LN_GROUPS, SSV_T_LN_PERSIST, SSV_T_LSTM_MERGE, SSV_T_PWLN_BWD, SSV_T_TAIL_LEGACY, SSV_T_COUNT };
 const char* ssv_tuning(int knob);
 int ssv_pack_job_blocks(const ssv_pack_job& j);
 int ssv_launch_pack_multi(const ssv_pack_job* jobs_dev, int njobs, int nblocks, float* amax_ws, hipStream_t st);
 #define SSV_PACK_AMAX_PER_WEIGHT 32
+int ssv_launch_pack_multi_from(const ssv_pack_job* jobs_dev, int njobs, int nblocks, const float* chunk_amax, const int* ranges_dev, int* step_inc, hipStream_t st);
 
 int ssv_launch_reduce_slabs(const float* slabs, float* out, long n, int Z, long slab_stride, hipStream_t st);
 int ssv_launch_reduce_slabs_perm(const float* slabs, float* out, int M, int Nc, int KT, int Z, hipStream_t st);
 int ssv_launch_reduce_pair(const float* slabs, float* out, int M, int Nc, int KT, int Z, const float* part, float* pout, int n2, int nblk, hipStream_t st);
 int ssv_launch_reduce_pair_multi(const ssv_wgrad_job* jobs, int njobs, const float* slabs, int M, int Nc, int KT, int Z, int n2, int nblk, hipStream_t st);
+int ssv_reduce_job_blocks(const ssv_reduce_job& j);
+int ssv_launch_reduce_jobs(const ssv_reduce_job* jobs_dev, int njobs, int nblocks, hipStream_t st);
 int ssv_launch_pack_wt(const float* w, float* wt, int Cout, int Cin, int KT, hipStream_t st);
 int ssv_launch_fill(float* p, float v, long n, hipStream_t st);
 int ssv_launch_linear_len1_fwd(const float* x, long x_bs, const float* w, const float* bias, const float* bias_b, long sbb, float* y, long y_bs,
diff --git a/spoofsv_amd/csrc/ssv_host.h b/spoofsv_amd/csrc/ssv_host.h
--- a/spoofsv_amd/csrc/ssv_host.h
+++ b/spoofsv_amd/csrc/ssv_host.h
@@ -61,7 +61,7 @@
 int dw_splits(int B, int M, int Nc, int k, int L);
 int conv1d_bwd_weight_impl(const float* dy, long dy_bs, const float* x, long x_bs, float* dw, int B, int Cin, int Cout, int L, int k, int dilation,
                            int causal, void* ws, size_t ws_bytes, ssv_stream_t stream, const float* part, float* pgrads, int n2, int nblk,
-                           const float* dy_amax, int dy_namax, const float* x_amax, int x_namax);
+                           const float* dy_amax, int dy_namax, const float* x_amax, int x_namax, int* left_z = nullptr);
 
 struct LstmWave { size_t xt, xp, out, c, bias, ih0, hh0, comb, comb_stride, aux, hp, hp_plane, l0c, x0p, total; int npad, xsplit0; };
 LstmWave lstm_wave_ws(int Bn, int T, int F, int H, int layers);
diff --git a/spoofsv_amd/ops.py b/spoofsv_amd/ops.py
--- a/spoofsv_amd/ops.py
+++ b/spoofsv_amd/ops.py
@@ -141,6 +141,9 @@
         self.captured_in_use = False
 
 
+_ReduceJob = collections.namedtuple("_ReduceJob", "slabs dw part pgrads M Nc KT Z n2 nblk keep")
+
+
 _WgradJob = collections.namedtuple("_WgradJob", "dy x part dw_ptr pg_ptr storages shift dy_amax x_amax")
 
 
@@ -148,6 +151,7 @@
 
     def __init__(self):
         self.jobs = {}
+        self.reduce = []
         self.slots = []
         self.cursor = 0
         self.pending = set()
@@ -179,11 +183,12 @@
             slot.upload_pending = False
             slot.captured_in_use = False
         self.jobs = {}
+        self.reduce = []
         self.pending.clear()
 
     @staticmethod
     def accepts(B, Cin, Cout, L, k, nblk, params=()):
-        if torch.is_grad_enabled() or any(p is not None and p.grad is not None for p in params):
+        if not DeferredWgrad._late_ok(params):
             return False
         ok = nblk <= 768 and bool(_lib.lib().ssv_conv1d_bwd_weight_multi_ok(B, Cin, Cout, L, k))
         if _DEFER is not None:
@@ -194,6 +199,37 @@
             if ok:
                 _DEFER.pending.update(owners)
         return ok
+
+    @staticmethod
+    def _late_ok(params):
+        return not (torch.is_grad_enabled() or any(p is not None and p.grad is not None for p in params))
+
+    @staticmethod
+    def queues(params):
+        if _DEFER is None or _lib.precision() < 1 or _lib.tail_legacy():
+            return False
+        if any(p is not None and not p.is_leaf for p in params) or not DeferredWgrad._late_ok(params):
+            return False
+        owners = [resident.param_of(p) for p in params if p is not None]
+        if any(q in _DEFER.pending for q in owners):
+            raise RuntimeError("DeferredWgrad: a parameter is used by two operators of one backward pass; deferred (batched) "
+                               "weight gradients cannot be summed by autograd -- build the step with defer_wgrad=False")
+        _DEFER.pending.update(owners)
+        return True
+
+    def queue_slabs(self, dy, dy_bs, dy_amax, x, x_bs, x_amax, dw, part, pg, n2, nblk, k, dilation, causal):
+        B, Cin, L = x.shape
+        Cout = dy.shape[1]
+        nb = _lib.query("ssv_conv1d_bwd_weight_workspace", B, Cin, Cout, L, k)
+        ws = _ws(nb, x.device)
+        z = _lib.lib().ssv_conv1d_bwd_weight_slabs(_p(dy), dy_bs, *_an(dy_amax), _p(x), x_bs, *_an(x_amax), _p(dw), _p(part), _p(pg), n2, nblk,
+                                                   B, Cin, Cout, L, k, dilation, int(causal), _p(ws), nb, _stream())
+        if z < 0:
+            raise RuntimeError("ssv_conv1d_bwd_weight_slabs failed (%d): %s" % (z, _lib.lib().ssv_last_error().decode()))
+        if z > 0:
+            keep = (ws, part, dw.untyped_storage(), None if pg is None else pg.untyped_storage())
+            self.reduce.append(_ReduceJob(ws.data_ptr(), dw.data_ptr(), 0 if part is None else part.data_ptr(), 0 if pg is None else pg.data_ptr(),
+                                          Cout, Cin, k, z, n2 if part is not None else 0, nblk if part is not None else 0, keep))
 
     def add(self, dy, dy_bs, x, x_bs, dw, part, pg, k, dilation, causal, n2, nblk, dy_amax=None, x_amax=None):
         B, Cin, L = x.shape
@@ -223,44 +259,84 @@
         self.cursor += 1
         return slot
 
-    def flush(self):
-        for key, jobs in self.jobs.items():
-            B, Cin, Cout, L, k, dy_bs, x_bs, n2, nblk, dev = key
-            n = len(jobs)
-            table = (_lib.WgradJob * n)()
-            f16 = _f16()
-            for t, j in zip(table, jobs):
-                t.dy, t.x, t.dw, t.part, t.pgrads = j.dy.data_ptr(), j.x.data_ptr(), j.dw_ptr, j.part.data_ptr(), j.pg_ptr
-                t.shift[0], t.shift[1], t.shift[2] = j.shift
-                if f16:
-                    if j.dy_amax is None or j.x_amax is None:
-                        raise RuntimeError("DeferredWgrad: a job was queued without operand scales in the split-fp16 mode")
-                    t.dy_amax, t.x_amax, t.dy_namax, t.x_namax = j.dy_amax.data_ptr(), j.x_amax.data_ptr(), j.dy_amax.numel(), j.x_amax.numel()
-            raw = bytes(table)
-            slot = self._slot(len(raw), dev)
-            slot.pinned[:len(raw)].copy_(torch.frombuffer(bytearray(raw), dtype=torch.uint8))
-            if torch.cuda.is_current_stream_capturing():
-                if slot.captured_in_use:
-                    raise RuntimeError("DeferredWgrad: this instance already serves a captured step (its frozen job tables are in use); "
-                                       "build a new step object for another capture")
-                slot.captured_in_use = True
-                dtable = slot.captured
-                if self._side is None:
-                    self._side = torch.cuda.Stream(device=dev)
-                with torch.cuda.stream(self._side):
-                    dtable.copy_(slot.pinned, non_blocking=True)
-                    slot.copied = torch.cuda.Event()
-                    slot.copied.record()
-            else:
-                dtable = slot.eager
+    def _upload(self, raw, dev):
+        slot = self._slot(len(raw), dev)
+        slot.pinned[:len(raw)].copy_(torch.frombuffer(bytearray(raw), dtype=torch.uint8))
+        if torch.cuda.is_current_stream_capturing():
+            if slot.captured_in_use:
+                raise RuntimeError("DeferredWgrad: this instance already serves a captured step (its frozen job tables are in use); "
+                                   "build a new step object for another capture")
+            slot.captured_in_use = True
+            dtable = slot.captured
+            if self._side is None:
+                self._side = torch.cuda.Stream(device=dev)
+            with torch.cuda.stream(self._side):
                 dtable.copy_(slot.pinned, non_blocking=True)
                 slot.copied = torch.cuda.Event()
                 slot.copied.record()
-            nb = _lib.query("ssv_conv1d_bwd_weight_multi_workspace", n, B, Cin, Cout, L, k)
-            ws = _ws(nb, dev)
-            max_shift = max(abs(v) for j in jobs for v in j.shift)
-            _lib.call("ssv_conv1d_bwd_weight_multi", _p(dtable), n, dy_bs, x_bs, B, Cin, Cout, L, k, max_shift, n2, nblk, _p(ws), nb, _stream())
+        else:
+            dtable = slot.eager
+            dtable.copy_(slot.pinned, non_blocking=True)
+            slot.copied = torch.cuda.Event()
+            slot.copied.record()
+        return dtable
+
+    def _wgrad_table(self, key, jobs):
+        n = len(jobs)
+        table = (_lib.WgradJob * n)()
+        f16 = _f16()
+        for t, j in zip(table, jobs):
+            t.dy, t.x, t.dw, t.part, t.pgrads = j.dy.data_ptr(), j.x.data_ptr(), j.dw_ptr, j.part.data_ptr(), j.pg_ptr
+            t.shift[0], t.shift[1], t.shift[2] = j.shift
+            if f16:
+                if j.dy_amax is None or j.x_amax is None:
+                    raise RuntimeError("DeferredWgrad: a job was queued without operand scales in the split-fp16 mode")
+                t.dy_amax, t.x_amax, t.dy_namax, t.x_namax = j.dy_amax.data_ptr(), j.x_amax.data_ptr(), j.dy_amax.numel(), j.x_amax.numel()
+        return self._upload(bytes(table), key[-1])
+
+    def flush(self):
+        if _lib.tail_legacy():
+            for key, jobs in self.jobs.items():
+                B, Cin, Cout, L, k, dy_bs, x_bs, n2, nblk, dev = key
+                n = len(jobs)
+                dtable = self._wgrad_table(key, jobs)
+                nb = _lib.query("ssv_conv1d_bwd_weight_multi_workspace", n, B, Cin, Cout, L, k)
+                ws = _ws(nb, dev)
+                max_shift = max(abs(v) for j in jobs for v in j.shift)
+                _lib.call("ssv_conv1d_bwd_weight_multi", _p(dtable), n, dy_bs, x_bs, B, Cin, Cout, L, k, max_shift, n2, nblk, _p(ws), nb, _stream())
+        elif self.jobs or self.reduce:
+            sizes = [_lib.query("ssv_conv1d_bwd_weight_multi_workspace", len(jobs), key[0], key[1], key[2], key[3], key[4]) for key, jobs in self.jobs.items()]
+            dev = next(iter(self.jobs))[-1] if self.jobs else None
+            ws = _ws(sum(sizes), dev) if self.jobs else None
+            reduce, off = list(self.reduce), 0
+            for (key, jobs), nb in zip(self.jobs.items(), sizes):
+                B, Cin, Cout, L, k, dy_bs, x_bs, n2, nblk, kdev = key
+                if kdev != dev:
+                    raise RuntimeError("DeferredWgrad: weight gradients of two devices in one flush")
+                n = len(jobs)
+                dtable = self._wgrad_table(key, jobs)
+                max_shift = max(abs(v) for j in jobs for v in j.shift)
+                base = ws.data_ptr() + off
+                _lib.call("ssv_conv1d_bwd_weight_multi_gemm", _p(dtable), n, dy_bs, x_bs, B, Cin, Cout, L, k, max_shift, n2, nblk,
+                          ctypes.c_void_p(base), nb, _stream())
+                Z = int(_lib.lib().ssv_conv1d_bwd_weight_multi_splits(n, B, Cin, Cout, L, k))
+                for i, j in enumerate(jobs):
+                    reduce.append(_ReduceJob(base + 4 * i * Z * Cout * Cin * k, j.dw_ptr, j.part.data_ptr() if n2 else 0, j.pg_ptr if n2 else 0,
+                                             Cout, Cin, k, Z, n2, nblk if n2 else 0, None))
+                off += nb
+            table = (_lib.ReduceJob * len(reduce))()
+            for t, r in zip(table, reduce):
+                t.slabs, t.dw, t.part, t.pgrads = r.slabs, r.dw, r.part or None, r.pgrads or None
+                t.M, t.Nc, t.KT, t.Z, t.n2, t.nblk = r.M, r.Nc, r.KT, r.Z, r.n2, r.nblk
+            nblocks = _lib.lib().ssv_wgrad_reduce_plan(table, len(reduce))
+            if nblocks < 0:
+                raise RuntimeError("ssv_wgrad_reduce_plan: " + _lib.lib().ssv_last_error().decode())
+            if dev is None:
+                dev = reduce[0].keep[0].device
+            dtable = self._upload(bytes(table), dev)
+            _lib.call("ssv_wgrad_reduce_jobs", _p(dtable), len(reduce), nblocks, _stream())
         self.jobs = {}
+        self.reduce = []
         self.pending.clear()
 
 
@@ -306,7 +382,9 @@
         bias = ctx.bias_ref
         pg = gradarena.grad_block((g1, b1, g2, b2, bias), 6, C, x.device) if bias is not None else torch.empty((6, C), dtype=_F32, device=x.device)
         nblk = _lib.query("ssv_ln_partial_rows", B, L)
-        if _DEFER is not None and _DEFER.accepts(B, C, 2 * C, L, k, nblk, (w, g1, b1, g2, b2, bias)):
+        params = (w, g1, b1, g2, b2, bias)
+        batched = _DEFER is not None and _DEFER.accepts(B, C, 2 * C, L, k, nblk, params)
+        if batched or DeferredWgrad.queues(params):
             dh = torch.empty((B, 2 * C, L), dtype=_F32, device=x.device)
             part = torch.empty((nblk, 6 * C), dtype=_F32, device=x.device)
             f16 = _f16()
@@ -317,7 +395,10 @@
             ws = _ws(nb, x.device)
             _lib.call("ssv_highway_conv1d_bwd_data", _p(dy), dybs, _p(x), xbs, _p(w), resident.lookup(w), _p(g1), _p(b1), _p(g2), _p(b2),
                       _p(h), _p(stats), _p(dx), C * L, _p(dh), _p(dh_amax), _p(part), B, C, L, k, dilation, causal, _p(ws), nb, _stream())
-            _DEFER.add(dh, 2 * C * L, x, xbs, dw, part, pg, k, dilation, causal, 6 * C, rows, dh_amax, x_amax)
+            if batched:
+                _DEFER.add(dh, 2 * C * L, x, xbs, dw, part, pg, k, dilation, causal, 6 * C, rows, dh_amax, x_amax)
+            else:
+                _DEFER.queue_slabs(dh, 2 * C * L, dh_amax, x, xbs, x_amax, dw, part, pg, 6 * C, rows, k, dilation, causal)
             return (dx, dw, pg[4:6].reshape(2 * C), pg[0], pg[1], pg[2], pg[3]) + (None,) * 6
         nb = _lib.query("ssv_highway_conv1d_bwd_workspace", B, C, L, k)
         ws = _ws(nb, x.device)
@@ -345,10 +426,13 @@
     return dx
 
 
-def _conv_bwd_weight(dy, dybs, x, xbs, wshape, k=1, dilation=1, causal=0, out=None, dy_amax=None, x_amax=None):
+def _conv_bwd_weight(dy, dybs, x, xbs, wshape, k=1, dilation=1, causal=0, out=None, dy_amax=None, x_amax=None, late=None):
     B, Cin, L = x.shape
     Cout = wshape[0]
     dw = out if out is not None else torch.empty(wshape, dtype=_F32, device=x.device)
+    if late is not None and DeferredWgrad.queues(late):
+        _DEFER.queue_slabs(dy, dybs, dy_amax, x, xbs, x_amax, dw, None, None, 0, 0, k, dilation, causal)
+        return dw
     nb = _lib.query("ssv_conv1d_bwd_weight_workspace", B, Cin, Cout, L, k)
     ws = _ws(nb, x.device)
     _lib.call("ssv_conv1d_bwd_weight", _p(dy), dybs, *_an(dy_amax), _p(x), xbs, *_an(x_amax), _p(dw), B, Cin, Cout, L, k, dilation, int(causal),
@@ -408,7 +492,9 @@
         dw = gradarena.grad_like(w)
         ds = torch.empty((B, Cout, 1), dtype=_F32, device=x.device) if ctx.has_s else None
         nblk = _lib.query("ssv_ln_partial_rows", B, L)
-        if _DEFER is not None and _DEFER.accepts(B, Cin, Cout, L, 1, nblk, (w, gamma, beta, ctx.bias_ref)):
+        params = (w, gamma, beta, ctx.bias_ref)
+        batched = _DEFER is not None and _DEFER.accepts(B, Cin, Cout, L, 1, nblk, params)
+        if batched or DeferredWgrad.queues(params):
             dpre = torch.empty((B, Cout, L), dtype=_F32, device=x.device)
             part = torch.empty((nblk, 3 * Cout), dtype=_F32, device=x.device)
             f16 = _f16()
@@ -419,7 +505,10 @@
             ws = _ws(nb, x.device)
             _lib.call("ssv_pointwise_conv_ln_act_bwd_data", _p(dy), dybs, _p(w), resident.lookup(w), _p(gamma), _p(beta), _p(pre), _p(stats),
                       _p(dx), Cin * L, _p(ds), _p(dpre), _p(dpre_amax), _p(part), B, Cin, Cout, L, ctx.act, _p(ws), nb, _stream())
-            _DEFER.add(dpre, Cout * L, x, xbs, dw, part, pg, 1, 1, 0, 3 * Cout, rows, dpre_amax, x_amax)
+            if batched:
+                _DEFER.add(dpre, Cout * L, x, xbs, dw, part, pg, 1, 1, 0, 3 * Cout, rows, dpre_amax, x_amax)
+            else:
+                _DEFER.queue_slabs(dpre, Cout * L, dpre_amax, x, xbs, x_amax, dw, part, pg, 3 * Cout, rows, 1, 1, 0)
             return dx, dw, pg[2], pg[0], pg[1], ds, None, None, None, None
         nb = _lib.query("ssv_pointwise_conv_ln_act_bwd_workspace", B, Cin, Cout, L)
         ws = _ws(nb, x.device)
@@ -456,7 +545,7 @@
         Cout = w.shape[0]
         dy_amax = amax_of(dy) if (_f16() and _bf3_shape(dy)) else None
         dx = _conv_bwd_data(dy, dybs, w, Cin, L, k, dilation, causal, dy_amax) if need_dx else None
-        dw = _conv_bwd_weight(dy, dybs, x, xbs, tuple(w.shape), k, dilation, causal, out=gradarena.view(w), dy_amax=dy_amax, x_amax=ctx.x_amax)
+        dw = _conv_bwd_weight(dy, dybs, x, xbs, tuple(w.shape), k, dilation, causal, out=gradarena.view(w), dy_amax=dy_amax, x_amax=ctx.x_amax, late=(w,))
         db = None
         if has_bias:
             db = gradarena.view(ctx.bias_ref)
@@ -1085,7 +1174,7 @@
             w2 = w.view(Cin, 2 * Cout, 1)
             _conv_fwd(du, 2 * Cout * L, w2, None, None, dx, Cin * L, 1, 1, 0, du_am)
             x_am = (ctx.x_amax if ctx.x_amax is not None else amax_of(x)) if f16 else None
-            _conv_bwd_weight(x, xbs, du, 2 * Cout * L, (Cin, 2 * Cout, 1), 1, 1, 0, dw.view(Cin, 2 * Cout, 1), x_am, du_am)
+            _conv_bwd_weight(x, xbs, du, 2 * Cout * L, (Cin, 2 * Cout, 1), 1, 1, 0, dw.view(Cin, 2 * Cout, 1), x_am, du_am, late=(w,))
             _lib.call("ssv_bias_grad", _p(dy), dybs, _p(db), B, Cout, 2 * L, _stream())
             return dx, dw, db, None, None, None
         _lib.call("ssv_deconv1d_k2s2_bwd", _p(dy), dybs, None, 0, _p(x), xbs, _p(w), _p(dx), Cin * L, _p(dw), _p(db),
diff --git a/spoofsv_amd/resident.py b/spoofsv_amd/resident.py
--- a/spoofsv_amd/resident.py
+++ b/spoofsv_amd/resident.py
@@ -100,9 +100,22 @@
         self._build()
         _lib.call("ssv_conv_pack_multi", ctypes.c_void_p(self._jobs.data_ptr()), self._njobs, self._nblocks,
                   ctypes.c_void_p(self._ws.data_ptr()), self._ws_bytes, stream)
+        self._mark_current()
+
+    def _mark_current(self):
         for p in self.params:
             if _owner(p) is self:
                 p._ssv_planes.version, p._ssv_planes.addr = p._version, p.data_ptr()
+
+    def owns_all(self):
+        return all(_owner(p) is self for p in self.params)
+
+    def refresh_from(self, stream, chunk_amax, ranges, step_inc=None):
+        self._build()
+        assert ranges.dtype == torch.int32 and ranges.numel() == 2 * len(self.params)
+        _lib.call("ssv_conv_pack_multi_from", ctypes.c_void_p(self._jobs.data_ptr()), self._njobs, self._nblocks,
+                  ctypes.c_void_p(chunk_amax.data_ptr()), ctypes.c_void_p(ranges.data_ptr()), step_inc, stream)
+        self._mark_current()
 
 
 def ensure(module, stream):
diff --git a/spoofsv_amd/train.py b/spoofsv_amd/train.py
--- a/spoofsv_amd/train.py
+++ b/spoofsv_amd/train.py
@@ -60,6 +60,11 @@
         self._steps = 0
         self._resident = None
         self.resident = resident
+        self._chunk_amax = None
+        self._chunk_range = {}
+        self._ranges = None
+        self._ranges_upload = None
+        self._ranges_key = None
 
     def refresh_resident_weights(self):
         if not self.resident:
@@ -87,16 +92,47 @@
         _lib.call("ssv_adam_multi", _p(self._table), self._nchunks, float(group["lr"]), float(b1), float(b2),
                   float(group["eps"]), self._steps, step_dev, _stream())
 
+    def _launch_amax(self, group, step_dev):
+        b1, b2 = group["betas"]
+        _lib.call("ssv_adam_multi_amax", _p(self._table), self._nchunks, float(group["lr"]), float(b1), float(b2),
+                  float(group["eps"]), self._steps, step_dev, _p(self._chunk_amax), 1, _stream())
+
+    def _pair_ranges(self):
+        if (not self.resident or type(self)._launch is not FusedAdam._launch or _lib.precision() != 2 or _lib.lib().ssv_tail_legacy()):
+            return None
+        if self._resident is None:
+            self._resident = _resident.ResidentWeights([p for g in self.param_groups for p in g["params"]])
+        rw = self._resident
+        if not rw.params or any(id(p) not in self._chunk_range for p in rw.params):
+            return None
+        rw._build()
+        if not rw.owns_all():
+            return None
+        rows = [self._chunk_range[id(p)] for p in rw.params]
+        key = (rw._key, tuple(rows))
+        if key != self._ranges_key:
+            for p, (first, count) in zip(rw.params, rows):
+                assert count == (p.numel() + _CHUNK - 1) // _CHUNK and 0 <= first and first + count <= self._nchunks
+            if self._ranges_upload is None:
+                self._ranges = torch.empty((len(rows), 2), dtype=torch.int32, device=rw.params[0].device)
+                self._ranges_upload = StagedUpload(self._ranges)
+            self._ranges_upload.host().copy_(torch.tensor(rows, dtype=torch.int32))
+            self._ranges_upload.send()
+            self._ranges_key = key
+        return self._ranges
+
     def _build(self, plist):
         key = tuple((p.data_ptr(), p.grad.data_ptr()) for p in plist)
         if key == self._key:
             return
         rows = []
+        self._chunk_range = {}
         for p in plist:
             moments = self._moments(p)
             if not (p.is_contiguous() and p.grad.is_contiguous() and p.dtype == torch.float32 and p.grad.dtype == torch.float32):
                 raise RuntimeError("FusedAdam needs dense float32 parameters and gradients")
             n = p.numel()
+            self._chunk_range[id(p)] = (len(rows), (n + _CHUNK - 1) // _CHUNK)
             for off in range(0, n, _CHUNK):
                 m = min(_CHUNK, n - off)
                 rows.append((p.data_ptr() + 4 * off, p.grad.data_ptr() + 4 * off) + tuple(0 if t is None else t.data_ptr() + 4 * off for t in moments) + (m,))
@@ -107,6 +143,7 @@
         if self._upload is None:
             cap = sum((p.numel() + _CHUNK - 1) // _CHUNK for g in self.param_groups for p in g["params"])
             self._table = torch.empty((cap, cols), dtype=torch.int64, device=plist[0].device)
+            self._chunk_amax = torch.zeros(cap, dtype=torch.float32, device=plist[0].device)
             self._upload = StagedUpload(self._table)
         self._upload.host()[:len(rows)].copy_(torch.from_numpy(arr))
         self._upload.send()
@@ -118,6 +155,7 @@
         loss = closure() if closure is not None else None
         if len(self.param_groups) != 1:
             raise RuntimeError("FusedAdam keeps one device-side step counter: use one parameter group")
+        paired = False
         for group in self.param_groups:
             plist = [p for p in group["params"] if p.grad is not None]
             if not plist:
@@ -130,8 +168,15 @@
                 if self._step_dev is None:
                     self._step_dev = torch.full((1,), self._steps - 1, dtype=torch.int32, device=plist[0].device)
                 step_dev = _p(self._step_dev)
-            self._launch(group, step_dev)
-        self.refresh_resident_weights()
+            ranges = self._pair_ranges()
+            if ranges is not None:
+                self._launch_amax(group, step_dev)
+                self._resident.refresh_from(_stream(), self._chunk_amax, ranges, step_dev)
+                paired = True
+            else:
+                self._launch(group, step_dev)
+        if not paired:
+            self.refresh_resident_weights()
         return loss
 
     def state_dict(self):
```

After: 896,400 mel-frames/s (median of 6 runs). About the same (+0.7%).
